# uber-research/UPSNet

Hardware: AMD Instinct MI355X
Metric: images/sec (whole node), UPSNet-50 1024x2048 (higher is better)
Workload: dtype f32

## Files before the change

include/upsnet_hip.h:

```cpp
#ifndef UPSNET_HIP_H
#define UPSNET_HIP_H

#include <stddef.h>
#include <stdint.h>

#ifdef __cplusplus
extern "C" {
#endif

const char *upsnet_last_error(void);
const char *upsnet_last_kernel_form(void);
int upsnet_abi_version(void);

int upsnet_zero_fill(void *stream, void *ptr, size_t bytes);


int upsnet_roi_align_forward(void *stream, const float *bottom_data, float spatial_scale, int num_rois,
                             int height, int width, int channels, int pooled_height, int pooled_width,
                             int sampling_ratio, const float *bottom_rois, float *top_data);

int upsnet_roi_align_forward_nhwc(void *stream, const float *feat_nhwc, int batch, int height, int width,
                                  int channels, float spatial_scale, const float *rois, int num_rois,
                                  int pooled_height, int pooled_width, int sampling_ratio, float *out_nhwc);

int upsnet_fpn_roi_align_forward(void *stream, const float *const feat_nhwc[4], const int feat_h[4],
                                 const int feat_w[4], const float spatial_scale[4], int channels,
                                 const float *rois, int num_rois, const int *num_rois_dev, int pooled_height,
                                 int pooled_width, int sampling_ratio, float *out_nhwc, int *levels_out);

int upsnet_fpn_roi_order(void *stream, const float *rois, int num_rois, const int *num_rois_dev, int image_height, int image_width,
                         int *order_out);
int upsnet_fpn_roi_align_forward_ordered(void *stream, const float *const feat_nhwc[4], const int feat_h[4], const int feat_w[4],
                                         const float spatial_scale[4], int channels, const float *rois, int num_rois, const int *num_rois_dev,
                                         int pooled_height, int pooled_width, int sampling_ratio, float *out_nhwc, int *levels_out,
                                         const int *order);

void upsnet_roi_tuning(int variant);
void upsnet_roi_geometry(int target_workgroups, int min_bins);


int upsnet_deform_im2col(void *stream, const float *data_im, const float *data_offset, int channels,
                         int height, int width, int ksize_h, int ksize_w, int pad_h, int pad_w, int stride_h,
                         int stride_w, int dilation_h, int dilation_w, int parallel_imgs, int deformable_group,
                         float *data_col);

int upsnet_mod_deform_im2col(void *stream, const float *data_im, const float *data_offset,
                             const float *data_mask, int batch_size, int channels, int height_im, int width_im,
                             int height_col, int width_col, int kernel_h, int kernel_w, int pad_h, int pad_w,
                             int stride_h, int stride_w, int dilation_h, int dilation_w, int deformable_group,
                             float *data_col);


int upsnet_roi_align_backward(void *stream, const float *top_diff, float spatial_scale, int batch_size, int num_rois,
                              int height, int width, int channels, int pooled_height, int pooled_width,
                              int sampling_ratio, const float *bottom_rois, float *bottom_diff);

int upsnet_deform_col2im(void *stream, const float *data_col, const float *data_offset, int channels, int height,
                         int width, int ksize_h, int ksize_w, int pad_h, int pad_w, int stride_h, int stride_w,
                         int dilation_h, int dilation_w, int parallel_imgs, int deformable_group, float *grad_im);

int upsnet_deform_col2im_coord(void *stream, const float *data_col, const float *data_im, const float *data_offset,
                               int channels, int height, int width, int ksize_h, int ksize_w, int pad_h, int pad_w,
                               int stride_h, int stride_w, int dilation_h, int dilation_w, int parallel_imgs,
                               int deformable_group, float *grad_offset);

int upsnet_mod_deform_col2im(void *stream, const float *data_col, const float *data_offset, const float *data_mask,
                             int batch_size, int channels, int height_im, int width_im, int height_col, int width_col,
                             int kernel_h, int kernel_w, int pad_h, int pad_w, int stride_h, int stride_w,
                             int dilation_h, int dilation_w, int deformable_group, float *grad_im);

int upsnet_mod_deform_col2im_coord(void *stream, const float *data_col, const float *data_im, const float *data_offset,
                                   const float *data_mask, int batch_size, int channels, int height_im, int width_im,
                                   int height_col, int width_col, int kernel_h, int kernel_w, int pad_h, int pad_w,
                                   int stride_h, int stride_w, int dilation_h, int dilation_w, int deformable_group,
                                   float *grad_offset, float *grad_mask);

int upsnet_deform_conv_forward_nhwc(void *stream, int nlev, const float *const x[], const float *const offset[],
                                    const float *const mask[], float *const out[], const int height[],
                                    const int width[], int cin, int cout, int kh, int kw, int pad_h, int pad_w,
                                    int stride_h, int stride_w, int dil_h, int dil_w, int deformable_group,
                                    const float *wpack, int ldw, const float *bias, int relu);

size_t upsnet_dcn_packed_weight_floats(int cout, int cin, int kh, int kw);
int upsnet_dcn_pack_weight(void *stream, const float *weight, int cout, int cin, int kh, int kw, float *wpack);
int upsnet_deform_conv_fused_nhwc(void *stream, int nlev, const float *const x[], const float *const offset[],
                                  const float *const mask[], float *const out[], const int height[], const int width[],
                                  int cin, int cout, int kh, int kw, int pad, int stride, int dil, const float *wpack,
                                  const float *bias, int relu);
size_t upsnet_deform_conv_fused_splitk_workspace_bytes(int height, int width, int cout, int kh, int kw, int pad, int stride, int dil,
                                                       int ksplit);
int upsnet_deform_conv_fused_nhwc_splitk(void *stream, const float *x, const float *offset, const float *mask, float *out, int height,
                                         int width, int cin, int cout, int kh, int kw, int pad, int stride, int dil,
                                         const float *wpack, const float *bias, int relu, int ksplit, void *workspace);
void upsnet_dcn_tuning(int variant);

size_t upsnet_dcn_packed_weight_bf16_elems(int cout, int cin, int kh, int kw);
int upsnet_dcn_pack_weight_bf16(void *stream, const float *weight, int cout, int cin, int kh, int kw, void *wpack);
int upsnet_deform_conv_fused_nhwc_bf16(void *stream, int nlev, const float *const x[], const float *const offset[],
                                       const float *const mask[], float *const out[], const int height[], const int width[], int cin,
                                       int cout, int kh, int kw, int pad, int stride, int dil, const void *wpack, const float *bias,
                                       int relu);


int upsnet_prep_image_u8(void *stream, const unsigned char *image_hwc, int height, int width, const double pixel_means[3],
                         double im_scale, int resized_h, int resized_w, int padded_h, int padded_w, int nhwc4, float *blob);

int upsnet_image_to_nhwc4(void *stream, const float *nchw, int batch, int channels, int height, int width, float *nhwc4);


int upsnet_conv2d_nhwc_f32_multiw(void *stream, int nseg, const float *const x[], float *const out[], const int batch[],
                                  const int height[], const int width[], int Cin, const float *const wpack[], int ldw, int Cout,
                                  int KH, int KW, int stride, int pad, int relu);

int upsnet_conv2d_nhwc_f32(void *stream, int nseg, const float *const x[], const float *const residual[],
                           float *const out[], const int batch[], const int height[], const int width[], int Cin,
                           const float *wpack, int ldw, const float *bias, int Cout, int KH, int KW, int stride, int pad,
                           int relu, int residual_up);

size_t upsnet_conv2d_splitk_workspace_bytes(int batch, int height, int width, int Cout, int KH, int KW, int stride, int pad, int ksplit);
int upsnet_conv2d_nhwc_f32_splitk(void *stream, const float *x, const float *residual, float *out, int batch, int height, int width,
                                  int Cin, const float *wpack, int ldw, const float *bias, int Cout, int KH, int KW, int stride,
                                  int pad, int relu, int ksplit, void *workspace);

int upsnet_conv2d_winograd_nhwc_f32(void *stream, int nseg, const float *const x[], const float *const residual[],
                                    float *const out[], const int batch[], const int height[], const int width[], int Cin,
                                    const float *wpack, int ldw, const float *bias, int Cout, int relu);

int upsnet_conv2d_winograd_nhwc_f32_splitk(void *stream, const float *x, const float *residual, float *out, int batch, int height,
                                           int width, int Cin, const float *wpack, int ldw, const float *bias, int Cout, int relu,
                                           int ksplit, void *workspace);
int upsnet_conv_pack_weight_winograd(void *stream, const float *weight, int cout, int cin, int ldw, float *wpack);

int upsnet_conv2d_winograd_nhwc_f32_tn32(void *stream, int nseg, const float *const x[], const float *const residual[],
                                         float *const out[], const int batch[], const int height[], const int width[], int Cin,
                                         const float *wpack, int ldw, const float *bias, int Cout, int relu);
int upsnet_conv_pack_weight_winograd_tn32(void *stream, const float *weight, int cout, int cin, int ldw, float *wpack);
int upsnet_conv2d_winograd_nhwc_f32_tail(void *stream, const float *x, float *out, int batch, int n_main, int height, int width, int Cin,
                                         const float *wpack, int ldw, const float *wpack32, int ldw32, const float *bias, int Cout, int relu);

int upsnet_conv2d_nhwc_bf16(void *stream, int nseg, const float *const x[], const float *const residual[], float *const out[],
                            const int batch[], const int height[], const int width[], int Cin, const void *wpack_hi,
                            const void *wpack_lo, int ldw, const float *bias, int Cout, int KH, int KW, int stride, int pad,
                            int relu);
int upsnet_conv_pack_weight_bf16(void *stream, const float *weight, int cout, int cin, int kh, int kw, int ldw, void *wpack_hi,
                                 void *wpack_lo);
int upsnet_bottleneck_proj_bf16(void *stream, const void *x, void *out, int batch, int height_in, int width_in, int cin, int cmid, int stride,
                                const void *w1, const void *w2, const void *w3d, const float *b1, const float *b2, const float *b3d);
int upsnet_conv_bf16_tuning(int enable, int tile_rows);
int upsnet_conv1x1_bf16_tuning(int enable);
int upsnet_stem_pool_pack_weight_f32(void *stream, const float *weight, int cin, float *wpack);
int upsnet_stem_pool_f32(void *stream, const float *x4, int batch, int height, int width, const float *wpack, const float *bias, float *out);
int upsnet_stem_pool_pack_weight_bf16(void *stream, const float *weight, int cin, void *wpack);
int upsnet_stem_pool_bf16(void *stream, const float *x4, int batch, int height, int width, const void *wpack, const float *bias, void *out);
int upsnet_deconv2x2_nhwc_bf16(void *stream, const void *x, int batch, int height, int width, int Cin, const void *wpack_hi, int ldw,
                               const float *bias, int Cout, int relu, void *out, int out_bf16);

int upsnet_bottleneck_bf16(void *stream, const void *x, void *out, int batch, int height, int width, int cmid, const void *w1,
                           const void *w2, const void *w3, const float *b1, const float *b2, const float *b3);

int upsnet_conv2d_stem_nhwc4_f32(void *stream, const float *x, int batch, int height, int width, const float *wpack,
                                 int ldw, const float *bias, int Cout, int KH, int KW, int stride, int pad, int relu,
                                 float *out);
int upsnet_conv_pack_weight_stem(void *stream, const float *weight, int cout, int cin, int kh, int kw, int ldw, float *wpack);

int upsnet_deconv2x2_nhwc_f32(void *stream, const float *x, int batch, int height, int width, int Cin, const float *wpack,
                              int ldw, const float *bias, int Cout, int relu, float *out);
int upsnet_deconv2x2_pack_weight(void *stream, const float *weight, int cin, int cout, int ldw, float *wpack);

int upsnet_deconv2x2_frag_nhwc_f32(void *stream, const float *x, float *out, int batch, int height, int width, int Cin,
                                   const float *wpack, const float *bias4, int Cout, int relu);

void upsnet_conv_tuning(int winograd_tiles, int force_tile);

int upsnet_conv_pack_weight(void *stream, const float *weight, int cout, int cin, int kh, int kw, int ldw, float *wpack);

int upsnet_conv1x1_frag_nhwc_f32(void *stream, const float *x, const float *residual, float *out, int batch, int height, int width,
                                 int Cin, const float *wpack, const float *bias, int Cout, int stride, int relu, int residual_up);
void upsnet_conv1x1_tuning(int bn);
int upsnet_conv1x1_siblings_nhwc_f32(void *stream, const float *x, float *out_a, float *out_b, int batch, int height, int width, int Cin,
                                     const float *wpack, const float *bias, int cout_a, int cout_b, int stride, int relu_a, int relu_b);
void upsnet_conv1x1_pair32_tuning(int waves);

int upsnet_conv2d_winograd36_nhwc_f32(void *stream, int nseg, const float *const x[], float *const out[], const int batch[],
                                      const int height[], const int width[], int Cin, const float *wpack, int ldw, const float *bias,
                                      int Cout, int relu);
int upsnet_conv_pack_weight_winograd36(void *stream, const float *weight, int cout, int cin, int ldw, float *wpack);
size_t upsnet_conv2d_winograd36_splitk_workspace_bytes(int batch, int height, int width, int Cout, int ksplit);
int upsnet_conv2d_winograd36_nhwc_f32_splitk(void *stream, const float *x, float *out, int batch, int height, int width, int Cin,
                                             const float *wpack, int ldw, const float *bias, int Cout, int relu, int ksplit, void *workspace);

size_t upsnet_conv1x1_ksw_packed_weight_floats(int cout, int cin);
int upsnet_conv1x1_ksw_pack_weight(void *stream, const float *weight, int cout, int cin, float *wpack);
int upsnet_conv1x1_ksw_nhwc_f32(void *stream, const float *x, const float *residual, float *out, int batch, int height, int width, int Cin,
                                const float *wpack, const float *bias, int Cout, int stride, int relu, int tile_pixels, int tile_channels,
                                int split_n);
void upsnet_conv1x1_ksw_tuning(int tile);

size_t upsnet_conv3x3_ksw_packed_weight_floats(int cin);
int upsnet_conv3x3_ksw_pack_weight(void *stream, const float *weight, int cout, int cin, float *wpack);
int upsnet_conv3x3_ksw_nhwc_f32(void *stream, const float *x, float *out, int batch, int height, int width, int Cin, const float *wpack,
                                const float *bias, int Cout, int relu);

size_t upsnet_conv1x1_splitk_workspace_bytes(int batch, int out_height, int out_width, int Cout, int ksplit);
int upsnet_conv1x1_frag_nhwc_f32_splitk(void *stream, const float *x, const float *residual, float *out, int batch, int height, int width,
                                        int Cin, const float *wpack, const float *bias, int Cout, int stride, int relu, int ksplit,
                                        void *workspace);

int upsnet_conv1x1_pair_nhwc_f32(void *stream, const float *x, const float *residual, float *out1, float *out2, long pixels, int C0,
                                 const float *w3pack, const float *bias3, int C1, const float *w1pack, const float *bias1, int C2);


int upsnet_nms_host(int *keep_out_host, int *num_out_host, const float *boxes_host, int boxes_num,
                    int boxes_dim, float nms_overlap_thresh, int device_id);

size_t upsnet_nms_workspace_bytes(int num_problems, int nmax);
int upsnet_nms_batched(void *stream, const float *boxes, const float *scores, const int *counts,
                       const uint8_t *pre_removed, int num_problems, int nmax, float thresh, int *keep_idx,
                       int *keep_cnt, void *workspace);

void upsnet_nms_tuning(int lds_staging);

int upsnet_cpu_nms_batched(void *stream, const float *boxes, const float *scores, const int *counts, int num_problems,
                           int nmax, double thresh, int *keep_idx, int *keep_cnt, void *workspace);

size_t upsnet_soft_nms_batched_workspace_bytes(int num_problems, int nmax);
int upsnet_soft_nms_batched(void *stream, float *boxes, int64_t *inds, const int *counts, int num_problems, int nmax,
                            float sigma, float Nt, float threshold, int method, int *n_out, void *workspace);

size_t upsnet_soft_nms_workspace_bytes(int n);
int upsnet_soft_nms(void *stream, float *boxes, int64_t *inds, int n, float sigma, float Nt, float threshold,
                    int method, int *n_out, void *workspace);


size_t upsnet_proposal_workspace_bytes(int nlev, const int *heights_host, const int *widths_host, int num_anchors,
                                       int pre_nms_top_n, int post_nms_top_n);
int upsnet_pyramid_proposals(void *stream, int nlev, const float *const cls_prob[], const float *const bbox_pred[],
                             const int *heights_host, const int *widths_host, const int *strides_host,
                             const float *anchors_host, int num_anchors, const float *im_info, int pre_nms_top_n,
                             int post_nms_top_n, float nms_thresh, float min_size, float *rois_out,
                             float *scores_out, int *num_out, void *workspace);

int upsnet_pyramid_proposals_strided(void *stream, int nlev, const float *const cls_prob[], const float *const bbox_pred[],
                                     const long *cls_chan_stride, const long *cls_pix_stride, const long *box_chan_stride,
                                     const long *box_pix_stride, const int *heights_host, const int *widths_host,
                                     const int *strides_host, const float *anchors_host, int num_anchors, const float *im_info,
                                     int pre_nms_top_n, int post_nms_top_n, float nms_thresh, float min_size, float *rois_out,
                                     float *scores_out, int *num_out, void *workspace);
int upsnet_pyramid_proposals_strided_ordered(void *stream, int nlev, const float *const cls_prob[], const float *const bbox_pred[],
                                     const long *cls_chan_stride, const long *cls_pix_stride, const long *box_chan_stride,
                                     const long *box_pix_stride, const int *heights_host, const int *widths_host,
                                     const int *strides_host, const float *anchors_host, int num_anchors, const float *im_info,
                                     int pre_nms_top_n, int post_nms_top_n, float nms_thresh, float min_size, float *rois_out,
                                     float *scores_out, int *num_out, void *workspace, int *roi_order_out);

int upsnet_pyramid_proposals_joint_strided(void *stream, int nlev, const float *const cls_prob[], const float *const bbox_pred[],
                                           const long *cls_chan_stride, const long *cls_pix_stride, const long *box_chan_stride,
                                           const long *box_pix_stride, const int *heights_host, const int *widths_host,
                                           const int *strides_host, const float *anchors_host, int num_anchors, const float *im_info,
                                           int pre_nms_top_n, int post_nms_top_n, float nms_thresh, float min_size, float *rois_out,
                                           float *scores_out, int *num_out, void *workspace);


int upsnet_mask_roi_capacity(int num_rois, int num_classes, int class_agnostic);
size_t upsnet_mask_roi_workspace_bytes(int num_rois, int num_classes, int class_agnostic);
int upsnet_mask_roi(void *stream, const float *rois, const float *bbox_delta, const float *cls_prob, int num_rois,
                    const int *num_rois_dev, int num_classes, const float *im_info, int class_agnostic,
                    float score_thresh, float nms_thresh, int max_det, const float reg_weights_host[4],
                    float *boxes_out, float *scores_out, int64_t *cls_out, int *src_out, int *num_out,
                    void *workspace);
int upsnet_mask_roi_ex(void *stream, const float *rois, const float *bbox_delta, const float *cls_prob, int num_rois,
                       const int *num_rois_dev, int num_classes, const float *im_info, int class_agnostic, int clip_boxes,
                       float score_thresh, float nms_thresh, int max_det, const float reg_weights_host[4],
                       float *boxes_out, float *scores_out, int64_t *cls_out, int *src_out, int *num_out,
                       void *workspace);

int upsnet_mask_roi_dedup(void *stream, const int *a_src, const int64_t *a_cls, const int *num_a, int cap_a, const int *b_src,
                          const int64_t *b_cls, const float *b_boxes, const int *num_b, int cap_b, int *map_out,
                          float *extra_boxes, int *num_extra);

int upsnet_mask_logit_gather(void *stream, const float *mask_logit, int n_rows, int num_classes, int hw, long stride_n,
                             long stride_c, long stride_e, const int *row, const int64_t *cls, int K, float *out);


size_t upsnet_mask_removal_workspace_bytes(int m, int num_thing_classes, int height, int width);
int upsnet_mask_removal(void *stream, const float *mask_rois, const float *cls_prob, const float *mask_logit,
                        const int64_t *cls_idx, int m, const int *m_dev, int mask_size, int num_thing_classes, int height, int width,
                        double fraction_threshold, int64_t *keep_inds, int *num_keep, int *real_keep,
                        void *workspace);

int upsnet_panoptic_tail_pack(void *stream, const int64_t *keep, const int *num_keep, int K, const int64_t *cls, const float *scores,
                              const int *det_num, const int *pan_num, const int *extra_num, int64_t *kept_cls, float *kept_scores,
                              int *counters);

int upsnet_mask_paste(void *stream, const float *mask_rois, const float *mask_logit, const int64_t *keep_inds,
                      const int *num_keep, const int *real_keep, int kmax, int mask_size, int height, int width,
                      float *mask_energy);

int upsnet_seg_term(void *stream, const float *fcn_output, int num_seg, int height, int width, const float *boxes,
                    const int64_t *cls, const int64_t *class_map, int k, float *seg_inst);

int upsnet_panoptic_fuse(void *stream, const float *fcn_output, int num_seg, int height, int width, int num_stuff,
                         const float *mask_rois, const float *mask_logit, const int64_t *cls_idx,
                         const int64_t *keep_inds, const int *num_keep, const int *real_keep, int kmax,
                         int mask_size, const int64_t *class_map, int enable_void, int64_t *pan_out,
                         int64_t *sem_out);

int upsnet_fcn_score_combine(void *stream, int nlev, const float *const part[], int num_seg, int height, int width,
                             const float *bias, float *score);

int upsnet_panoptic_fuse_up(void *stream, const float *fcn_score, int score_nhwc, int num_seg, int score_h, int score_w,
                            int scale, int num_stuff, const float *mask_rois, const float *mask_logit,
                            const int64_t *cls_idx, const int64_t *keep_inds, const int *num_keep, const int *real_keep,
                            int kmax, int mask_size, const int64_t *class_map, int64_t *pan_out, int64_t *sem_out);

int upsnet_panoptic_argmax(void *stream, const float *fcn_output, int num_seg, int height, int width, int num_stuff,
                           const float *seg_inst, const float *mask_energy, int k, int enable_void,
                           int64_t *pan_out);


size_t upsnet_unified_pan_workspace_bytes(void);
int upsnet_unified_pan_result(void *stream, const int64_t *pan, const int64_t *seg, const int64_t *cls_inds, int num_inst,
                              int height, int width, int id_last_stuff, int num_seg_classes, int stuff_area_limit,
                              void *workspace, unsigned char *pan_2ch);

size_t upsnet_combined_pan_workspace_bytes(int num_images, long total_pixels);
int upsnet_combined_pan_result(void *stream, int num_images, const int64_t *images, int max_height, int max_width, long total_pixels,
                               const int *cand, const int *segments, int id_last_stuff, int num_classes, int stuff_area_limit,
                               double fraction_threshold, void *workspace);

int upsnet_im_post_rle(void *stream, const float *pred_boxes, const float *mask_prob, const int64_t *cls_inds, int num_det,
                       int num_mask_channels, int mask_size, int im_height, int im_width, int cap, unsigned *transitions,
                       int *transition_count);

int upsnet_restore_label_maps(void *stream, const int64_t *sseg, const int64_t *pano, long src_stride, int src_height, int src_width,
                              const int *y_ofs, int out_height, const int *x_ofs, int out_width, unsigned char *out_sseg,
                              unsigned char *out_pano);


size_t upsnet_pq_workspace_bytes(int max_gt);
int upsnet_pq_accumulate(void *stream, const unsigned char *pred_2ch, const unsigned char *gt_rgb, int height, int width,
                         const int64_t *segments, int num_segments, const unsigned char *cat_known, int image_index, int max_gt,
                         void *workspace, int64_t *tp, int64_t *fp, int64_t *fn, double *iou, uint64_t *status);

int upsnet_confusion_accumulate(void *stream, const unsigned char *gt_label, const unsigned char *pred_label, long npix,
                                int class_num, int ignore_label, int64_t *confusion);


size_t upsnet_det_eval_image_workspace_bytes(int num_det, int num_rows, int num_gt, int height, int width, int segm);
int upsnet_det_eval_image(void *stream, int segm, int height, int width, int num_rows, int num_det, const double *det_xyxy,
                          const double *det_score, const int64_t *det_cls, const int *class_to_row, int num_classes,
                          const float *det_box_f32, const float *mask_prob, int num_mask_channels, int mask_size,
                          const int *det_trans, const int64_t *det_trans_off, int num_gt, const int *gt_row_off,
                          const double *gt_box, const double *gt_area, const int *gt_crowd, const int *gt_trans,
                          const int64_t *gt_trans_off, const int *gt_trans_dst, int num_gt_rle, const unsigned char *const *gt_u8,
                          const int *gt_u8_dst, int num_gt_u8, const int *rows_with_gt, int num_rows_with_gt,
                          const double *params, int image_index, void *workspace, double *rec_score, int *rec_img, int *rec_rk,
                          uint64_t *rec_match, uint64_t *rec_ign, int64_t *npig);

size_t upsnet_det_eval_accumulate_workspace_bytes(long num_records, int num_rows);
int upsnet_det_eval_accumulate(void *stream, long num_records, const double *rec_score, const int *rec_img, const int *rec_rk,
                               const uint64_t *rec_match, const uint64_t *rec_ign, const int *img_ord, int num_rows,
                               const int64_t *npig, const double *rec_thrs, void *workspace, double *precision, double *recall,
                               double *scores);

size_t upsnet_det_eval_boundary_image_workspace_bytes(int num_det, int num_rows, int num_gt, int height, int width);
int upsnet_det_eval_boundary_image(void *stream, int dilation, int height, int width, int num_rows, int num_det,
                                   const double *det_score, const int64_t *det_cls, const int *class_to_row, int num_classes,
                                   const float *det_box_f32, const float *mask_prob, int num_mask_channels, int mask_size,
                                   const int *det_trans, const int64_t *det_trans_off, int num_gt, const int *gt_row_off,
                                   const double *gt_area, const int *gt_crowd, const int *gt_trans,
                                   const int64_t *gt_trans_off, const int *gt_trans_dst, int num_gt_rle,
                                   const unsigned char *const *gt_u8, const int *gt_u8_dst, int num_gt_u8, const int *rows_with_gt,
                                   int num_rows_with_gt, const double *params, int image_index, void *workspace, double *rec_score,
                                   int *rec_img, int *rec_rk, uint64_t *rec_match, uint64_t *rec_ign, int64_t *npig);
int upsnet_boundary_dilation_fits(int height, int width, int dilation);

size_t upsnet_boundary_masks_workspace_bytes(int num_masks, int height, int width);
int upsnet_boundary_masks(void *stream, int dilation, int height, int width, int num_masks, const unsigned char *masks_u8,
                          const int *trans, const int64_t *trans_off, void *workspace, unsigned char *boundary_u8, int *boundary_area);

size_t upsnet_poly_raster_workspace_bytes(long total_vertices, long total_points);
int upsnet_poly_raster(void *stream, const double *vertices, const int *poly_off, const int *obj_off, const int *poly_off_dev,
                       const int *obj_off_dev, int num_poly, int num_obj, long total_points, int height, int width, void *workspace,
                       int *trans, int64_t *trans_off);


size_t upsnet_proposal_recall_workspace_bytes(int num_problems, long total_proposals);
int upsnet_proposal_recall(void *stream, int num_problems, const int64_t *problems, const float *proposals, const float *gt_boxes,
                           int max_gt, long total_proposals, void *workspace, float *out);


size_t upsnet_cs_inst_counts_ints(int num_preds);
size_t upsnet_cs_inst_workspace_bytes(int num_preds);
int upsnet_cs_inst_state_words(void);
int upsnet_cs_inst_image(void *stream, const uint16_t *gt_ids, int height, int width, int num_preds, const int *pred_cls,
                         const float *pred_scores, const int *trans, const int *trans_off, const unsigned char *masks, int walk_strided,
                         uint16_t *gt_t, const double *thresholds, int num_thr, int *counts, void *workspace, float *rec_score,
                         unsigned char *rec_cls, unsigned char *rec_code, int64_t *state);


size_t upsnet_cs_pixel_inst_ints(void);
int upsnet_cs_pixel_image(void *stream, const unsigned char *gt_labels, const uint16_t *gt_ids, const unsigned char *pred,
                          const unsigned char *lut, int height, int width, const double *avg_class_size, int64_t *conf, int *inst,
                          double *wsum, int *bad);


size_t upsnet_pan_format_workspace_bytes(void);
size_t upsnet_pan_format_table_ints(void);
int upsnet_pan_format(void *stream, const unsigned char *pred_2ch, int height, int width, const int *cat_table, void *workspace,
                      unsigned char *rgb, int *table);

int upsnet_pan_relabel(void *stream, const unsigned char *rgb, int height, int width, const int *table, int num_segments,
                       int image_index, unsigned char *out_2ch, int *counts, uint64_t *status);


size_t upsnet_gt_prepare_workspace_bytes(int seg_capacity);
int upsnet_gt_prepare(void *stream, const int *ids, const unsigned char *label_ids, int height, int width, const int *train_id,
                      const int *has_instances, const int *thing_row, int seg_capacity, int trans_capacity, void *workspace,
                      unsigned char *train_map, unsigned char *rgb, int *table, int *trans_off, int *trans, int *status);


int upsnet_vis_max_detections(void);
int upsnet_vis_max_label(void);
size_t upsnet_vis_workspace_bytes(int num_dets, int height, int width);
int upsnet_vis_font(unsigned char *cells);
int upsnet_vis_render(void *stream, const unsigned char *image, int height, int width, int num_dets, const float *boxes,
                      const unsigned char *colours, const unsigned char *labels, const int *label_len, const int *trans,
                      const int *trans_off, int num_trans, void *workspace, unsigned char *out);


int upsnet_group_norm_chunk_pixels(void);
size_t upsnet_group_norm_workspace_bytes(int nseg, const int batch[], const int height[], const int width[]);
int upsnet_group_norm_nhwc_f32(void *stream, int nseg, const float *const x[], float *const out[], const int batch[],
                               const int height[], const int width[], int C, const float *gamma, const float *beta, float eps,
                               int relu, const float *const residual[], const int res_height[], const int res_width[],
                               int residual_up, void *workspace);
int upsnet_group_norm_small_nhwc_f32(void *stream, const float *x, float *out, int batch, int height, int width, int C,
                                     const float *gamma, const float *beta, float eps, int relu);


int upsnet_cs_inst_expand(void *stream, const int *trans, const int *trans_off, int num_masks, int height, int width, int bits,
                          unsigned char *out);


int upsnet_tta_seg_merge(void *stream, int num_aug, const float *const maps[], const int map_h[], const int map_w[], const float q[],
                         const float resized_w[], const int flip[], int cell, int num_seg, int height, int width, float *out);

int upsnet_tta_roi_union(void *stream, int num_aug, const float *const rois[], const float *const delta[], const float *const prob[],
                         const int *const num_rois_dev[], const float r[], const float resized_w[], const int flip[], int capacity,
                         int delta_dim, int num_classes, float *rois_out, float *delta_out, float *prob_out, int *num_out);

int upsnet_tta_boxes_to_aug(void *stream, int num_aug, const float q[], const float resized_w[], const int flip[], const float *boxes,
                            int num_boxes, float *boxes_out);

int upsnet_tta_mask_merge(void *stream, int num_aug, const float *const logits[], const int flip[], int num_rois, int num_classes,
                          int mask_size, int nhwc, float *out);

#ifdef __cplusplus
}
#endif
#endif
```

upsnet_amd/_lib.py:

```python
import ctypes
import os

import torch

_HERE = os.path.dirname(os.path.abspath(__file__))
LIB_PATH = os.environ.get("UPSNET_LIB_PATH") or os.path.join(_HERE, "csrc", "libupsnet_hip.so")

c_int, c_float, c_double, c_void_p, c_size_t, c_long = ctypes.c_int, ctypes.c_float, ctypes.c_double, ctypes.c_void_p, ctypes.c_size_t, ctypes.c_long
P = c_void_p

_SIGNATURES = {
    "upsnet_last_error": (ctypes.c_char_p, []),
    "upsnet_last_kernel_form": (ctypes.c_char_p, []),
    "upsnet_abi_version": (c_int, []),
    "upsnet_zero_fill": (c_int, [P, P, c_size_t]),
    "upsnet_roi_align_forward": (c_int, [P, P, c_float, c_int, c_int, c_int, c_int, c_int, c_int, c_int, P, P]),
    "upsnet_roi_align_forward_nhwc": (c_int, [P, P, c_int, c_int, c_int, c_int, c_float, P, c_int, c_int, c_int, c_int, P]),
    "upsnet_fpn_roi_align_forward": (c_int, [P, P, P, P, P, c_int, P, c_int, P, c_int, c_int, c_int, P, P]),
    "upsnet_fpn_roi_order": (c_int, [P, P, c_int, P, c_int, c_int, P]),
    "upsnet_fpn_roi_align_forward_ordered": (c_int, [P, P, P, P, P, c_int, P, c_int, P, c_int, c_int, c_int, P, P, P]),
    "upsnet_roi_tuning": (None, [c_int]),
    "upsnet_roi_geometry": (None, [c_int, c_int]),
    "upsnet_deform_im2col": (c_int, [P, P, P] + [c_int] * 13 + [P]),
    "upsnet_mod_deform_im2col": (c_int, [P, P, P, P] + [c_int] * 15 + [P]),
    "upsnet_roi_align_backward": (c_int, [P, P, c_float] + [c_int] * 8 + [P, P]),
    "upsnet_deform_col2im": (c_int, [P, P, P] + [c_int] * 13 + [P]),
    "upsnet_deform_col2im_coord": (c_int, [P, P, P, P] + [c_int] * 13 + [P]),
    "upsnet_mod_deform_col2im": (c_int, [P, P, P, P] + [c_int] * 15 + [P]),
    "upsnet_mod_deform_col2im_coord": (c_int, [P, P, P, P, P] + [c_int] * 15 + [P, P]),
    "upsnet_deform_conv_forward_nhwc": (c_int, [P, c_int, P, P, P, P, P, P] + [c_int] * 11 + [P, c_int, P, c_int]),
    "upsnet_dcn_packed_weight_floats": (c_size_t, [c_int, c_int, c_int, c_int]),
    "upsnet_dcn_pack_weight": (c_int, [P, P, c_int, c_int, c_int, c_int, P]),
    "upsnet_deform_conv_fused_nhwc": (c_int, [P, c_int, P, P, P, P, P, P] + [c_int] * 7 + [P, P, c_int]),
    "upsnet_deform_conv_fused_splitk_workspace_bytes": (c_size_t, [c_int] * 9),
    "upsnet_deform_conv_fused_nhwc_splitk": (c_int, [P, P, P, P, P] + [c_int] * 9 + [P, P, c_int, c_int, P]),
    "upsnet_dcn_tuning": (None, [c_int]),
    "upsnet_dcn_packed_weight_bf16_elems": (c_size_t, [c_int, c_int, c_int, c_int]),
    "upsnet_dcn_pack_weight_bf16": (c_int, [P, P, c_int, c_int, c_int, c_int, P]),
    "upsnet_deform_conv_fused_nhwc_bf16": (c_int, [P, c_int, P, P, P, P, P, P] + [c_int] * 7 + [P, P, c_int]),
    "upsnet_conv1x1_frag_nhwc_f32": (c_int, [P, P, P, P, c_int, c_int, c_int, c_int, P, P, c_int, c_int, c_int, c_int]),
    "upsnet_conv1x1_tuning": (None, [c_int]),
    "upsnet_conv1x1_siblings_nhwc_f32": (c_int, [P, P, P, P, c_int, c_int, c_int, c_int, P, P, c_int, c_int, c_int, c_int, c_int]),
    "upsnet_conv1x1_pair32_tuning": (None, [c_int]),
    "upsnet_conv1x1_splitk_workspace_bytes": (ctypes.c_size_t, [c_int, c_int, c_int, c_int, c_int]),
    "upsnet_conv1x1_frag_nhwc_f32_splitk": (c_int, [P, P, P, P, c_int, c_int, c_int, c_int, P, P, c_int, c_int, c_int, c_int, P]),
    "upsnet_conv1x1_ksw_packed_weight_floats": (ctypes.c_size_t, [c_int, c_int]),
    "upsnet_conv1x1_ksw_pack_weight": (c_int, [P, P, c_int, c_int, P]),
    "upsnet_conv1x1_ksw_nhwc_f32": (c_int, [P, P, P, P, c_int, c_int, c_int, c_int, P, P, c_int, c_int, c_int, c_int, c_int, c_int]),
    "upsnet_conv1x1_ksw_tuning": (None, [c_int]),
    "upsnet_conv3x3_ksw_packed_weight_floats": (ctypes.c_size_t, [c_int]),
    "upsnet_conv3x3_ksw_pack_weight": (c_int, [P, P, c_int, c_int, P]),
    "upsnet_conv3x3_ksw_nhwc_f32": (c_int, [P, P, P, c_int, c_int, c_int, c_int, P, P, c_int, c_int]),
    "upsnet_conv2d_winograd36_splitk_workspace_bytes": (ctypes.c_size_t, [c_int, c_int, c_int, c_int, c_int]),
    "upsnet_conv2d_winograd36_nhwc_f32_splitk": (c_int, [P, P, P, c_int, c_int, c_int, c_int, P, c_int, P, c_int, c_int, c_int, P]),
    "upsnet_conv1x1_pair_nhwc_f32": (c_int, [P, P, P, P, P, c_long, c_int, P, P, c_int, P, P, c_int]),
    "upsnet_conv2d_nhwc_f32": (c_int, [P, c_int, P, P, P, P, P, P, c_int, P, c_int, P, c_int, c_int, c_int, c_int, c_int, c_int, c_int]),
    "upsnet_conv2d_nhwc_f32_multiw": (c_int, [P, c_int, P, P, P, P, P, c_int, P, c_int, c_int, c_int, c_int, c_int, c_int, c_int]),
    "upsnet_conv_tuning": (None, [c_int, c_int]),
    "upsnet_conv_pack_weight": (c_int, [P, P, c_int, c_int, c_int, c_int, c_int, P]),
    "upsnet_nms_host": (c_int, [P, P, P, c_int, c_int, c_float, c_int]),
    "upsnet_nms_workspace_bytes": (c_size_t, [c_int, c_int]),
    "upsnet_nms_batched": (c_int, [P, P, P, P, P, c_int, c_int, c_float, P, P, P]),
    "upsnet_nms_tuning": (None, [c_int]),
    "upsnet_cpu_nms_batched": (c_int, [P, P, P, P, c_int, c_int, c_double, P, P, P]),
    "upsnet_soft_nms_batched_workspace_bytes": (c_size_t, [c_int, c_int]),
    "upsnet_soft_nms_batched": (c_int, [P, P, P, P, c_int, c_int, c_float, c_float, c_float, c_int, P, P]),
    "upsnet_soft_nms_workspace_bytes": (c_size_t, [c_int]),
    "upsnet_soft_nms": (c_int, [P, P, P, c_int, c_float, c_float, c_float, c_int, P, P]),
    "upsnet_proposal_workspace_bytes": (c_size_t, [c_int, P, P, c_int, c_int, c_int]),
    "upsnet_pyramid_proposals_strided": (c_int, [P, c_int, P, P, P, P, P, P, P, P, P, P, c_int, P, c_int, c_int, c_float, c_float, P, P, P, P]),
    "upsnet_pyramid_proposals_strided_ordered": (c_int, [P, c_int, P, P, P, P, P, P, P, P, P, P, c_int, P, c_int, c_int, c_float, c_float, P, P, P, P, P]),
    "upsnet_pyramid_proposals_joint_strided": (c_int, [P, c_int, P, P, P, P, P, P, P, P, P, P, c_int, P, c_int, c_int, c_float, c_float, P, P, P, P]),
    "upsnet_pyramid_proposals": (c_int, [P, c_int, P, P, P, P, P, P, c_int, P, c_int, c_int, c_float, c_float, P, P, P, P]),
    "upsnet_mask_roi_capacity": (c_int, [c_int, c_int, c_int]),
    "upsnet_mask_roi_workspace_bytes": (c_size_t, [c_int, c_int, c_int]),
    "upsnet_mask_roi": (c_int, [P, P, P, P, c_int, P, c_int, P, c_int, c_float, c_float, c_int, P, P, P, P, P, P, P]),
    "upsnet_mask_roi_ex": (c_int, [P, P, P, P, c_int, P, c_int, P, c_int, c_int, c_float, c_float, c_int, P, P, P, P, P, P, P]),
    "upsnet_mask_logit_gather": (c_int, [P, P, c_int, c_int, c_int, c_long, c_long, c_long, P, P, c_int, P]),
    "upsnet_mask_removal_workspace_bytes": (c_size_t, [c_int, c_int, c_int, c_int]),
    "upsnet_mask_removal": (c_int, [P, P, P, P, P, c_int, P, c_int, c_int, c_int, c_int, c_double, P, P, P, P]),
    "upsnet_panoptic_tail_pack": (c_int, [P, P, P, c_int, P, P, P, P, P, P, P, P]),
    "upsnet_mask_paste": (c_int, [P, P, P, P, P, P, c_int, c_int, c_int, c_int, P]),
    "upsnet_seg_term": (c_int, [P, P, c_int, c_int, c_int, P, P, P, c_int, P]),
    "upsnet_panoptic_fuse": (c_int, [P, P, c_int, c_int, c_int, c_int, P, P, P, P, P, P, c_int, c_int, P, c_int, P, P]),
    "upsnet_panoptic_fuse_up": (c_int, [P, P, c_int, c_int, c_int, c_int, c_int, c_int, P, P, P, P, P, P, c_int, c_int, P, P, P]),
    "upsnet_conv2d_stem_nhwc4_f32": (c_int, [P, P, c_int, c_int, c_int, P, c_int, P, c_int, c_int, c_int, c_int, c_int, c_int, P]),
    "upsnet_conv_pack_weight_stem": (c_int, [P, P, c_int, c_int, c_int, c_int, c_int, P]),
    "upsnet_deconv2x2_nhwc_f32": (c_int, [P, P, c_int, c_int, c_int, c_int, P, c_int, P, c_int, c_int, P]),
    "upsnet_deconv2x2_pack_weight": (c_int, [P, P, c_int, c_int, c_int, P]),
    "upsnet_deconv2x2_frag_nhwc_f32": (c_int, [P, P, P, c_int, c_int, c_int, c_int, P, P, c_int, c_int]),
    "upsnet_prep_image_u8": (c_int, [P, P, c_int, c_int, P, c_double, c_int, c_int, c_int, c_int, c_int, P]),
    "upsnet_image_to_nhwc4": (c_int, [P, P, c_int, c_int, c_int, c_int, P]),
    "upsnet_unified_pan_workspace_bytes": (c_size_t, []),
    "upsnet_unified_pan_result": (c_int, [P, P, P, P, c_int, c_int, c_int, c_int, c_int, c_int, P, P]),
    "upsnet_combined_pan_workspace_bytes": (c_size_t, [c_int, c_long]),
    "upsnet_combined_pan_result": (c_int, [P, c_int, P, c_int, c_int, c_long, P, P, c_int, c_int, c_int, c_double, P]),
    "upsnet_mask_roi_dedup": (c_int, [P, P, P, P, c_int, P, P, P, P, c_int, P, P, P]),
    "upsnet_conv2d_winograd_nhwc_f32": (c_int, [P, c_int, P, P, P, P, P, P, c_int, P, c_int, P, c_int, c_int]),
    "upsnet_conv2d_winograd_nhwc_f32_splitk": (c_int, [P, P, P, P, c_int, c_int, c_int, c_int, P, c_int, P, c_int, c_int, c_int, P]),
    "upsnet_conv_pack_weight_winograd": (c_int, [P, P, c_int, c_int, c_int, P]),
    "upsnet_conv_pack_weight_winograd_tn32": (c_int, [P, P, c_int, c_int, c_int, P]),
    "upsnet_conv2d_winograd_nhwc_f32_tn32": (c_int, [P, c_int, P, P, P, P, P, P, c_int, P, c_int, P, c_int, c_int]),
    "upsnet_conv2d_winograd_nhwc_f32_tail": (c_int, [P, P, P, c_int, c_int, c_int, c_int, c_int, P, c_int, P, c_int, P, c_int, c_int]),
    "upsnet_conv2d_winograd36_nhwc_f32": (c_int, [P, c_int, P, P, P, P, P, c_int, P, c_int, P, c_int, c_int]),
    "upsnet_conv_pack_weight_winograd36": (c_int, [P, P, c_int, c_int, c_int, P]),
    "upsnet_conv2d_nhwc_bf16": (c_int, [P, c_int, P, P, P, P, P, P, c_int, P, P, c_int, P, c_int, c_int, c_int, c_int, c_int, c_int]),
    "upsnet_bottleneck_proj_bf16": (c_int, [P, P, P, c_int, c_int, c_int, c_int, c_int, c_int, P, P, P, P, P, P]),
    "upsnet_conv_bf16_tuning": (c_int, [c_int, c_int]),
    "upsnet_conv1x1_bf16_tuning": (c_int, [c_int]),
    "upsnet_stem_pool_pack_weight_f32": (c_int, [P, P, c_int, P]),
    "upsnet_stem_pool_f32": (c_int, [P, P, c_int, c_int, c_int, P, P, P]),
    "upsnet_stem_pool_pack_weight_bf16": (c_int, [P, P, c_int, P]),
    "upsnet_stem_pool_bf16": (c_int, [P, P, c_int, c_int, c_int, P, P, P]),
    "upsnet_deconv2x2_nhwc_bf16": (c_int, [P, P, c_int, c_int, c_int, c_int, P, c_int, P, c_int, c_int, P, c_int]),
    "upsnet_bottleneck_bf16": (c_int, [P, P, P, c_int, c_int, c_int, c_int, P, P, P, P, P, P]),
    "upsnet_conv_pack_weight_bf16": (c_int, [P, P, c_int, c_int, c_int, c_int, c_int, P, P]),
    "upsnet_conv2d_splitk_workspace_bytes": (c_size_t, [c_int, c_int, c_int, c_int, c_int, c_int, c_int, c_int, c_int]),
    "upsnet_conv2d_nhwc_f32_splitk": (c_int, [P, P, P, P, c_int, c_int, c_int, c_int, P, c_int, P, c_int, c_int, c_int, c_int, c_int, c_int, c_int, P]),
    "upsnet_im_post_rle": (c_int, [P, P, P, P, c_int, c_int, c_int, c_int, c_int, c_int, P, P]),
    "upsnet_fcn_score_combine": (c_int, [P, c_int, P, c_int, c_int, c_int, P, P]),
    "upsnet_panoptic_argmax": (c_int, [P, P, c_int, c_int, c_int, c_int, P, P, c_int, c_int, P]),
    "upsnet_pq_workspace_bytes": (c_size_t, [c_int]),
    "upsnet_pq_accumulate": (c_int, [P, P, P, c_int, c_int, P, c_int, P, c_int, c_int, P, P, P, P, P, P]),
    "upsnet_restore_label_maps": (c_int, [P, P, P, c_long, c_int, c_int, P, c_int, P, c_int, P, P]),
    "upsnet_confusion_accumulate": (c_int, [P, P, P, c_long, c_int, c_int, P]),
    "upsnet_det_eval_image_workspace_bytes": (c_size_t, [c_int] * 6),
    "upsnet_det_eval_image": (c_int, [P, c_int, c_int, c_int, c_int, c_int, P, P, P, P, c_int, P, P, c_int, c_int, P, P, c_int, P, P, P, P,
                                      P, P, P, c_int, P, P, c_int, P, c_int, P, c_int, P, P, P, P, P, P, P]),
    "upsnet_det_eval_accumulate_workspace_bytes": (c_size_t, [c_long, c_int]),
    "upsnet_det_eval_accumulate": (c_int, [P, c_long, P, P, P, P, P, P, c_int, P, P, P, P, P, P]),
    "upsnet_det_eval_boundary_image_workspace_bytes": (c_size_t, [c_int] * 5),
    "upsnet_det_eval_boundary_image": (c_int, [P, c_int, c_int, c_int, c_int, c_int, P, P, P, c_int, P, P, c_int, c_int, P, P, c_int, P, P, P,
                                               P, P, P, c_int, P, P, c_int, P, c_int, P, c_int, P, P, P, P, P, P, P]),
    "upsnet_boundary_dilation_fits": (c_int, [c_int, c_int, c_int]),
    "upsnet_boundary_masks_workspace_bytes": (c_size_t, [c_int, c_int, c_int]),
    "upsnet_boundary_masks": (c_int, [P, c_int, c_int, c_int, c_int, P, P, P, P, P, P]),
    "upsnet_poly_raster_workspace_bytes": (c_size_t, [c_long, c_long]),
    "upsnet_poly_raster": (c_int, [P, P, P, P, P, P, c_int, c_int, c_long, c_int, c_int, P, P, P]),
    "upsnet_proposal_recall_workspace_bytes": (c_size_t, [c_int, c_long]),
    "upsnet_proposal_recall": (c_int, [P, c_int, P, P, P, c_int, c_long, P, P]),
    "upsnet_cs_inst_counts_ints": (c_size_t, [c_int]),
    "upsnet_cs_inst_workspace_bytes": (c_size_t, [c_int]),
    "upsnet_cs_inst_state_words": (c_int, []),
    "upsnet_cs_inst_image": (c_int, [P, P, c_int, c_int, c_int, P, P, P, P, P, c_int, P, P, c_int, P, P, P, P, P, P]),
    "upsnet_cs_pixel_inst_ints": (c_size_t, []),
    "upsnet_cs_pixel_image": (c_int, [P, P, P, P, P, c_int, c_int, P, P, P, P, P]),
    "upsnet_pan_format_workspace_bytes": (c_size_t, []),
    "upsnet_pan_format_table_ints": (c_size_t, []),
    "upsnet_pan_format": (c_int, [P, P, c_int, c_int, P, P, P, P]),
    "upsnet_pan_relabel": (c_int, [P, P, c_int, c_int, P, c_int, c_int, P, P, P]),
    "upsnet_gt_prepare_workspace_bytes": (c_size_t, [c_int]),
    "upsnet_gt_prepare": (c_int, [P, P, P, c_int, c_int, P, P, P, c_int, c_int, P, P, P, P, P, P, P]),
    "upsnet_vis_max_detections": (c_int, []),
    "upsnet_vis_max_label": (c_int, []),
    "upsnet_vis_workspace_bytes": (c_size_t, [c_int, c_int, c_int]),
    "upsnet_vis_font": (c_int, [P]),
    "upsnet_vis_render": (c_int, [P, P, c_int, c_int, c_int, P, P, P, P, P, P, c_int, P, P]),
    "upsnet_group_norm_chunk_pixels": (c_int, []),
    "upsnet_group_norm_workspace_bytes": (c_size_t, [c_int, P, P, P]),
    "upsnet_group_norm_nhwc_f32": (c_int, [P, c_int, P, P, P, P, P, c_int, P, P, c_float, c_int, P, P, P, c_int, P]),
    "upsnet_group_norm_small_nhwc_f32": (c_int, [P, P, P, c_int, c_int, c_int, c_int, P, P, c_float, c_int]),
    "upsnet_cs_inst_expand": (c_int, [P, P, P, c_int, c_int, c_int, c_int, P]),
    "upsnet_tta_seg_merge": (c_int, [P, c_int, P, P, P, P, P, P, c_int, c_int, c_int, c_int, P]),
    "upsnet_tta_roi_union": (c_int, [P, c_int, P, P, P, P, P, P, P, c_int, c_int, c_int, P, P, P, P]),
    "upsnet_tta_boxes_to_aug": (c_int, [P, c_int, P, P, P, P, c_int, P]),
    "upsnet_tta_mask_merge": (c_int, [P, c_int, P, P, c_int, c_int, c_int, c_int, P]),
}

_lib = None


def exported_symbols():
    return sorted(_SIGNATURES)


def lib():
    global _lib
    if _lib is None:
        if not os.path.exists(LIB_PATH):
            raise RuntimeError("upsnet_amd: %s is missing -- build it with `python -m upsnet_amd.build` "
                               "(there is no CPU fallback)" % LIB_PATH)
        l = ctypes.CDLL(LIB_PATH)
        for name, (res, args) in _SIGNATURES.items():
            fn = getattr(l, name)
            fn.restype = res
            fn.argtypes = args
        _lib = l
    return _lib


def check(rc, what):
    if rc != 0:
        raise RuntimeError("upsnet_amd.%s failed: %s" % (what, lib().upsnet_last_error().decode()))


def ptr(t):
    return None if t is None else c_void_p(t.data_ptr())


def stream():
    return c_void_p(torch.cuda.current_stream().cuda_stream)


def require_cuda(*tensors):
    for t in tensors:
        if t is not None and not t.is_cuda:
            raise Exception("not implemented")


def f32c(t):
    if t.dtype != torch.float32:
        t = t.float()
    return t.contiguous()


def nhwc(t):
    return t.contiguous(memory_format=torch.channels_last)


def int_array(vals):
    return (c_int * len(vals))(*[int(v) for v in vals])


def float_array(vals):
    return (c_float * len(vals))(*[float(v) for v in vals])


def ptr_array(tensors):
    return (c_void_p * len(tensors))(*[None if t is None else t.data_ptr() for t in tensors])
```

upsnet_amd/csrc/conv_params.h:

```cpp
#pragma once
#include "common.h"

#define CV_BM 128
#define CV_BK 32
#define CV_LDA (CV_BM + 1)
#define CV_MAXSEG 5

typedef float floatx16 __attribute__((ext_vector_type(16)));

struct ConvSeg {
    const float *x, *res, *off, *mask;
    const float *w;
    float *out;
    int N, H, W, Ho, Wo;
    int OH, OW;
    int tile_start;
    long M;
};

struct ConvParams {
    ConvSeg seg[CV_MAXSEG];
    const float *w, *bias;
    int nseg, Cin, Cout, ldw, KH, KW, stride, pad, dil, relu;
    int res_up;
    int m_tiles, n_tiles;
    int ksplit;
    float *partial;
    long m_total;
    int io;
    int sib_split, sib_relu;
    float *sib_out;
};

static inline int conv_fill(ConvParams &p, const char *who, int nseg, const float *const x[], const float *const res[],
                     const float *const off[], const float *const mask[], float *const out[], const int batch[],
                     const int height[], const int width[], int Cin, int Cout, const float *wpack, int ldw, const float *bias,
                     int KH, int KW, int stride, int pad, int dil, int relu)
{
    UPS_REQUIRE(nseg >= 1 && nseg <= CV_MAXSEG, "%s: 1..%d feature maps per launch (got %d)", who, CV_MAXSEG, nseg);
    UPS_REQUIRE(x && out && height && width && wpack, "%s: null pointer", who);
    UPS_REQUIRE(Cin > 0 && Cin % CV_BK == 0, "%s: Cin must be a multiple of 32 (got %d)", who, Cin);
    UPS_REQUIRE(Cout > 0 && ldw % 32 == 0 && ldw >= Cout, "%s: ldw must be Cout rounded up to 32 (got %d for Cout=%d)", who, ldw, Cout);
    UPS_REQUIRE(KH >= 1 && KW >= 1 && KH * KW <= 49 && stride >= 1 && pad >= 0 && dil >= 1, "%s: bad kernel/stride/pad/dilation", who);
    UPS_REQUIRE((long)KH * KW * Cin * ldw < (1L << 30), "%s: packed weight exceeds 4 GiB", who);
    p.w = wpack; p.bias = bias; p.nseg = nseg; p.Cin = Cin; p.Cout = Cout; p.ldw = ldw; p.KH = KH; p.KW = KW;
    p.stride = stride; p.pad = pad; p.dil = dil; p.relu = relu; p.res_up = 0;
    p.ksplit = 1; p.partial = nullptr; p.m_total = 0; p.io = 0; p.sib_split = 0; p.sib_relu = 0; p.sib_out = nullptr;
    int tiles = 0;
    for (int i = 0; i < CV_MAXSEG; ++i) {
        ConvSeg &s = p.seg[i];
        if (i < nseg) {
            const int nb = batch ? batch[i] : 1;
            UPS_REQUIRE(x[i] && out[i] && nb > 0 && height[i] > 0 && width[i] > 0, "%s: bad feature map %d", who, i);
            s.x = x[i]; s.out = out[i]; s.res = res ? res[i] : nullptr; s.off = off ? off[i] : nullptr; s.mask = mask ? mask[i] : nullptr;
            s.w = nullptr;
            s.N = nb; s.H = height[i]; s.W = width[i];
            s.OH = s.OW = 0;
            s.Ho = (height[i] + 2 * pad - (dil * (KH - 1) + 1)) / stride + 1;
            s.Wo = (width[i] + 2 * pad - (dil * (KW - 1) + 1)) / stride + 1;
            UPS_REQUIRE(s.Ho > 0 && s.Wo > 0, "%s: empty output for feature map %d", who, i);
            UPS_REQUIRE((long)nb * height[i] * width[i] * Cin < (1L << 30), "%s: feature map %d exceeds 4 GiB (32-bit byte offsets); split the batch", who, i);
            s.M = (long)nb * s.Ho * s.Wo;
            UPS_REQUIRE(s.M * Cout < (1L << 29), "%s: output %d exceeds 2 GiB (32-bit byte offsets in the epilogue); split the batch", who, i);
            s.tile_start = tiles;
            tiles += (int)((s.M + 127) / 128);
        } else {
            s.x = s.res = s.off = s.mask = nullptr; s.w = nullptr; s.out = nullptr;
            s.N = s.H = s.W = s.Ho = s.Wo = s.OH = s.OW = 0; s.M = 0; s.tile_start = 0x7fffffff;
        }
    }
    p.m_tiles = tiles;
    return 0;
}


int conv_splitk_reduce(hipStream_t st, const float *partial, int ksplit, long m_total, long M, int Cout, const float *bias, const float *res,
                       int relu, float *out);
```

upsnet_amd/csrc/conv_wino36.hip:

```cpp
#include <cstdlib>
#include <type_traits>
#include "conv_params.h"
#include "upsnet_hip.h"

#define W36_TM 32
#define W36_TN 64
#define W36_PTS 36
#define W36_VBUF (W36_PTS * 4 * W36_TM * 16)
#define W36_BSTEP (2 * W36_TN * 16)
#define W36_STEPS (2 * W36_PTS)
#define W36_XCH (16 * W36_PTS * 64 * 4)
#define W36_RING 3

typedef unsigned w36_uintx4 __attribute__((ext_vector_type(4)));

#define W36_BT(D0, D1, D2, D3, D4, D5)                                                                               \
    {                                                                                                                \
        const float a0_ = D0, a1_ = D1, a2_ = D2, a3_ = D3, a4_ = D4, a5_ = D5;                                       \
        const float e1_ = __builtin_fmaf(-2.25f, a2_, a4_), o1_ = __builtin_fmaf(-2.25f, a1_, a3_);                   \
        const float e3_ = __builtin_fmaf(-0.5625f, a2_, a4_), o3_ = __builtin_fmaf(-0.5625f, a1_, a3_);               \
        D0 = __builtin_fmaf(1.265625f, a0_, __builtin_fmaf(-2.8125f, a2_, a4_));                                     \
        D1 = __builtin_fmaf(0.75f, o1_, e1_);                                                                        \
        D2 = __builtin_fmaf(-0.75f, o1_, e1_);                                                                       \
        D3 = __builtin_fmaf(1.5f, o3_, e3_);                                                                         \
        D4 = __builtin_fmaf(-1.5f, o3_, e3_);                                                                        \
        D5 = __builtin_fmaf(1.265625f, a1_, __builtin_fmaf(-2.8125f, a3_, a5_));                                     \
    }
#define W36_AT(M0, M1, M2, M3, M4, M5, Y0, Y1, Y2, Y3)                                                               \
    {                                                                                                                \
        const float s1_ = (M1) + (M2), d1_ = (M1) - (M2), s2_ = (M3) + (M4), d2_ = (M3) - (M4);                      \
        Y0 = ((M0) + s1_) + s2_;                                                                                     \
        Y1 = __builtin_fmaf(1.5f, d2_, 0.75f * d1_);                                                                 \
        Y2 = __builtin_fmaf(2.25f, s2_, 0.5625f * s1_);                                                              \
        Y3 = __builtin_fmaf(3.375f, d2_, __builtin_fmaf(0.421875f, d1_, (M5)));                                      \
    }

template <bool SK>
__global__ void __launch_bounds__(512, 1) conv_wino36_f32_kernel(const ConvParams p)
{
    extern __shared__ __attribute__((aligned(16))) unsigned char smem_raw[];
    const int tid = threadIdx.x, lane = tid & 63;
    const int wave = __builtin_amdgcn_readfirstlane(tid >> 6);
    const int cb = wave >> 2, pg = wave & 3;
    const int lhalf = lane >> 5, l32 = lane & 31;
    int m_t, n_t, kz = 0;
    {
        const int nt = p.n_tiles;
        const int per = (p.m_tiles + 7) >> 3;
        int bid = (int)blockIdx.x;
        if constexpr (SK) { const int base_grid = 8 * per * nt; kz = bid / base_grid; bid -= kz * base_grid; }
        const int q = bid >> 3;
        n_t = q % nt;
        const int local = q / nt;
        m_t = (bid & 7) * per + local;
        if (local >= per || m_t >= p.m_tiles) return;
    }
    int si = 0;
#pragma unroll
    for (int q = 1; q < CV_MAXSEG; ++q) if (q < p.nseg && m_t >= p.seg[q].tile_start) si = q;
    const ConvSeg sg = p.seg[si];
    const long p0 = (long)(m_t - sg.tile_start) * W36_TM;
    const int nslabs_all = p.Cin >> 4;
    const int s_first = SK ? (kz * nslabs_all) / p.ksplit : 0;
    const int nslabs = SK ? ((kz + 1) * nslabs_all) / p.ksplit - s_first : nslabs_all;
    const long HoWo = (long)sg.Ho * sg.Wo;

    const int ltile = tid >> 4, lch = tid & 15;
    int hrow0, wcol0;
    int hlo, hhi;
    unsigned tbase, nrmask = 0, ncmask = 0;
    bool lane_fix;
    {
        const long pp = p0 + ltile;
        const bool tile_ok = pp < sg.M;
        const long ppc = tile_ok ? pp : sg.M - 1;
        const int n = (int)(ppc / HoWo);
        const int rem = (int)(ppc - (long)n * HoWo);
        const int ty = rem / sg.Wo, tx = rem - ty * sg.Wo;
        const int h0 = 4 * ty - 1;
        hlo = n * sg.H; hhi = tile_ok ? hlo + sg.H : hlo;
        hrow0 = hlo + h0;
        wcol0 = 4 * tx - 1;
#pragma unroll
        for (int r = 0; r < 6; ++r) nrmask |= (h0 + r >= 0 && h0 + r < sg.H) ? 0u : (1u << r);
#pragma unroll
        for (int c = 0; c < 6; ++c) ncmask |= (wcol0 + c >= 0 && wcol0 + c < sg.W) ? 0u : (1u << c);
        lane_fix = tile_ok && (nrmask | ncmask) != 0;
        tbase = (unsigned)(hrow0 * sg.W + wcol0) * (4u * (unsigned)p.Cin) + 4u * (unsigned)lch;
    }
    const bool fix = __builtin_amdgcn_ballot_w64(lane_fix) != 0ull;
    bool risky;
    {
        const long plast = min(p0 + (long)W36_TM, sg.M) - 1;
        const long nl = plast / HoWo;
        const long tyl = (plast - nl * HoWo) / sg.Wo;
        risky = (nl * sg.H + 4 * tyl + 4) * (long)sg.W + 4L * sg.Wo >= (long)sg.N * sg.H * sg.W;
    }
    const unsigned cin4 = 4u * (unsigned)p.Cin;
    const unsigned rowpitch = (unsigned)sg.W * cin4;
    const unsigned cin4_s = __builtin_amdgcn_readfirstlane(cin4);
    const unsigned rowpitch_s = __builtin_amdgcn_readfirstlane((unsigned)sg.W) * cin4_s;
    const unsigned cbase = (unsigned)wcol0 * cin4 + 4u * (unsigned)lch;
#define W36_ROWOFF(R) (((unsigned)min(max(hrow0 + (R), hlo), max(hhi - 1, hlo)) * rowpitch) | ((hrow0 + (R) >= hlo && hrow0 + (R) < hhi) ? 0u : 0x80000000u))
    const size_t xaddr = reinterpret_cast<size_t>(sg.x);
    const unsigned xlo = __builtin_amdgcn_readfirstlane((unsigned)xaddr), xhi = __builtin_amdgcn_readfirstlane((unsigned)(xaddr >> 32));
    const unsigned xbytes = __builtin_amdgcn_readfirstlane((unsigned)(sg.N * sg.H * sg.W) * 4u * (unsigned)p.Cin - (SK ? (unsigned)s_first * 64u : 0u));
    const char *xbase = reinterpret_cast<const char *>(((size_t)xhi << 32) | xlo) + (SK ? (size_t)s_first * 64 : 0);
#define W36_SWZ(Q) ((((Q) & 1) << 2) | (((Q) >> 1) << 1))
    const unsigned st_base = (unsigned)((((lch >> 2) * W36_TM + (ltile ^ W36_SWZ(lch >> 2))) * 16) + (lch & 3) * 4);
    constexpr unsigned XI_PITCH = 4 * W36_TM * 16;
    const unsigned fr_base0 = (unsigned)((lhalf * W36_TM + (l32 ^ W36_SWZ(lhalf))) * 16) + (unsigned)pg * 9u * XI_PITCH;
    const unsigned fr_base1 = (unsigned)(((2 + lhalf) * W36_TM + (l32 ^ W36_SWZ(2 + lhalf))) * 16) + (unsigned)pg * 9u * XI_PITCH;
    const size_t waddr = reinterpret_cast<size_t>(p.w) + ((size_t)n_t * (size_t)nslabs_all + (size_t)s_first) * (W36_STEPS * W36_BSTEP);
    const unsigned wlo = __builtin_amdgcn_readfirstlane((unsigned)waddr), whi = __builtin_amdgcn_readfirstlane((unsigned)(waddr >> 32));
    const __amdgpu_buffer_rsrc_t wrsrc = __builtin_amdgcn_make_buffer_rsrc(reinterpret_cast<void *>(((size_t)whi << 32) | wlo), 0,
                                                                            nslabs * (int)(W36_STEPS * W36_BSTEP), 0x00020000);
    const unsigned b_lane = (unsigned)(lhalf * (W36_TN * 16) + (32 * cb + l32) * 16);
    const int gmax = nslabs * W36_STEPS - 1;

    floatx16 acc[9];
#pragma unroll
    for (int i = 0; i < 9; ++i)
#pragma unroll
        for (int r = 0; r < 16; ++r) acc[i][r] = 0.f;

    float ld[36];
    float4 breg[W36_RING];

#define W36_LOADROW_FAST(R, RS) { unsigned so_ = (unsigned)((R) ? (R) - 1 : 0) * rowpitch_s; asm volatile("" : "+s"(so_));              \
        ld[6 * (R)] = __uint_as_float(__builtin_amdgcn_raw_buffer_load_b32(RS, (R) ? tbase + rowpitch_s : tbase, so_, 0));               \
        _Pragma("unroll") for (int c_ = 1; c_ < 6; ++c_) ld[6 * (R) + c_] = __uint_as_float(__builtin_amdgcn_raw_buffer_load_b32(       \
            RS, ((R) ? tbase + rowpitch_s : tbase) + cin4_s, so_ + (unsigned)(c_ - 1) * cin4_s, 0)); }
#define W36_LOADROW_SAFE(R, RS) { unsigned cb_ = cbase; asm volatile("" : "+v"(cb_)); const unsigned rb_ = W36_ROWOFF(R) + cb_; _Pragma("unroll") for (int c_ = 0; c_ < 6; ++c_) \
        ld[6 * (R) + c_] = __uint_as_float(__builtin_amdgcn_raw_buffer_load_b32(RS, (rb_ + (unsigned)c_ * cin4) | ((ncmask << (30 - c_)) & 0x40000000u), 0, 0)); }
#define W36_FIXROW(R) if (fix) { asm volatile("" ::: "memory"); const unsigned bad_ = ((nrmask >> (R)) & 1u) ? 0x3fu : ncmask;           \
        _Pragma("unroll") for (int c_ = 0; c_ < 6; ++c_) ld[6 * (R) + c_] = ((bad_ >> c_) & 1u) ? 0.f : ld[6 * (R) + c_]; }
#define W36_ROWPASS(R) W36_BT(ld[6 * (R) + 0], ld[6 * (R) + 1], ld[6 * (R) + 2], ld[6 * (R) + 3], ld[6 * (R) + 4], ld[6 * (R) + 5])
#define W36_COLSTASH(J, SB)                                                                                           \
    {                                                                                                                 \
        float c0_ = ld[0 + (J)], c1_ = ld[6 + (J)], c2_ = ld[12 + (J)], c3_ = ld[18 + (J)], c4_ = ld[24 + (J)], c5_ = ld[30 + (J)]; \
        W36_BT(c0_, c1_, c2_, c3_, c4_, c5_)                                                                          \
        *reinterpret_cast<float *>(smem_raw + (SB) + (0 * 6 + (J)) * XI_PITCH) = c0_;                                 \
        *reinterpret_cast<float *>(smem_raw + (SB) + (1 * 6 + (J)) * XI_PITCH) = c1_;                                 \
        *reinterpret_cast<float *>(smem_raw + (SB) + (2 * 6 + (J)) * XI_PITCH) = c2_;                                 \
        *reinterpret_cast<float *>(smem_raw + (SB) + (3 * 6 + (J)) * XI_PITCH) = c3_;                                 \
        *reinterpret_cast<float *>(smem_raw + (SB) + (4 * 6 + (J)) * XI_PITCH) = c4_;                                 \
        *reinterpret_cast<float *>(smem_raw + (SB) + (5 * 6 + (J)) * XI_PITCH) = c5_;                                 \
    }
#define W36_BLOAD(SLOT, G) { const w36_uintx4 v_ = __builtin_amdgcn_raw_buffer_load_b128(wrsrc, b_lane, (unsigned)min((G), gmax) * W36_BSTEP, 0); \
        breg[SLOT] = make_float4(__uint_as_float(v_.x), __uint_as_float(v_.y), __uint_as_float(v_.z), __uint_as_float(v_.w)); }

#pragma unroll
    for (int u = 0; u < W36_RING; ++u) W36_BLOAD(u, 18 * pg + u)
    {
        const __amdgpu_buffer_rsrc_t xr = __builtin_amdgcn_make_buffer_rsrc(const_cast<char *>(xbase), 0, xbytes, 0x00020000);
#pragma unroll
        for (int r = 0; r < 6; ++r) { W36_LOADROW_SAFE(r, xr) }
#pragma unroll
        for (int r = 0; r < 6; ++r) { W36_ROWPASS(r) }
#pragma unroll
        for (int j = 0; j < 6; ++j) { W36_COLSTASH(j, st_base) }
    }
    __syncthreads();
    float4 afr = *reinterpret_cast<const float4 *>(smem_raw + fr_base0);

    auto slab_loop = [&](auto fast_tag) __attribute__((always_inline)) {
    constexpr bool FAST = decltype(fast_tag)::value;
    for (int s = 0; s < nslabs; ++s) {
        const int sn = min(s + 1, nslabs - 1);
        const __amdgpu_buffer_rsrc_t xr = __builtin_amdgcn_make_buffer_rsrc(const_cast<char *>(xbase) + (size_t)sn * 64, 0, xbytes - (unsigned)sn * 64u, 0x00020000);
        const unsigned cur = (s & 1) ? W36_VBUF : 0u, nxt = W36_VBUF - cur;
        const unsigned sb = nxt + st_base;
        const int g0 = s * W36_STEPS + 18 * pg;
#pragma unroll
        for (int u = 0; u < 18; ++u) {
            if (u < 6) { if constexpr (FAST) { W36_LOADROW_FAST(u, xr) } else { W36_LOADROW_SAFE(u, xr) } }
            float4 afn;
            if (u < 17) afn = *reinterpret_cast<const float4 *>(smem_raw + cur + (((u + 1) & 1) ? fr_base1 : fr_base0) + (unsigned)((u + 1) >> 1) * XI_PITCH);
            else afn = *reinterpret_cast<const float4 *>(smem_raw + nxt + fr_base0);
            if (u == 6) { if constexpr (FAST) { W36_FIXROW(0) } W36_ROWPASS(0) }
            if (u == 7) { if constexpr (FAST) { W36_FIXROW(1) } W36_ROWPASS(1) }
            if (u == 8) { if constexpr (FAST) { W36_FIXROW(2) } W36_ROWPASS(2) }
            if (u == 9) { if constexpr (FAST) { W36_FIXROW(3) } W36_ROWPASS(3) }
            if (u == 10) { if constexpr (FAST) { W36_FIXROW(4) } W36_ROWPASS(4) }
            if (u == 11) { if constexpr (FAST) { W36_FIXROW(5) } W36_ROWPASS(5) W36_COLSTASH(0, sb) }
            if (u == 12) { W36_COLSTASH(1, sb) }
            if (u == 13) { W36_COLSTASH(2, sb) }
            if (u == 14) { W36_COLSTASH(3, sb) }
            if (u == 15) { W36_COLSTASH(4, sb) }
            if (u == 16) { W36_COLSTASH(5, sb) }
            const float4 bf = breg[u % W36_RING];
            acc[u >> 1] = __builtin_amdgcn_mfma_f32_32x32x2f32(afr.x, bf.x, acc[u >> 1], 0, 0, 0);
            acc[u >> 1] = __builtin_amdgcn_mfma_f32_32x32x2f32(afr.y, bf.y, acc[u >> 1], 0, 0, 0);
            acc[u >> 1] = __builtin_amdgcn_mfma_f32_32x32x2f32(afr.z, bf.z, acc[u >> 1], 0, 0, 0);
            acc[u >> 1] = __builtin_amdgcn_mfma_f32_32x32x2f32(afr.w, bf.w, acc[u >> 1], 0, 0, 0);
            W36_BLOAD(u % W36_RING, (u + W36_RING < 18 ? g0 : g0 + W36_STEPS - 18) + u + W36_RING)
            if (u == 16) __syncthreads();
            afr = afn;
            __builtin_amdgcn_sched_barrier(0);
        }
    }
    };
    if (risky) slab_loop(std::false_type{}); else slab_loop(std::true_type{});
#undef W36_LOADROW_FAST
#undef W36_LOADROW_SAFE
#undef W36_ROWOFF
#undef W36_FIXROW
#undef W36_ROWPASS
#undef W36_COLSTASH
#undef W36_BLOAD

    const unsigned crow = (unsigned)p.Cout * 4u;
    const size_t oaddr_ = reinterpret_cast<size_t>(SK ? p.partial + (size_t)kz * (size_t)p.m_total * (size_t)p.Cout : sg.out);
    const unsigned obytes_ = __builtin_amdgcn_readfirstlane((unsigned)((long)sg.N * sg.OH * sg.OW) * crow);
    const __amdgpu_buffer_rsrc_t orsrc = __builtin_amdgcn_make_buffer_rsrc(
        reinterpret_cast<void *>(((size_t)(unsigned)__builtin_amdgcn_readfirstlane((unsigned)(oaddr_ >> 32)) << 32) | (unsigned)__builtin_amdgcn_readfirstlane((unsigned)oaddr_)),
        0, (int)obytes_, 0x00020000);
    float *xch = reinterpret_cast<float *>(smem_raw);
#pragma unroll 1
    for (int bb = 0; bb < 2; ++bb) {
        __syncthreads();
        if (cb == bb) {
#pragma unroll
            for (int u = 0; u < 9; ++u)
#pragma unroll
                for (int r = 0; r < 16; ++r) xch[(r * W36_PTS + 9 * pg + u) * 64 + lane] = acc[u][r];
        }
        __syncthreads();
        const int co_ch = n_t * W36_TN + 32 * bb + l32;
        const bool co_ok = co_ch < p.Cout;
        const float bv = (p.bias != nullptr && co_ok) ? p.bias[co_ch] : 0.f;
#pragma unroll 1
        for (int rr = 0; rr < 2; ++rr) {
            const int r = 2 * wave + rr;
            const long pp = p0 + 8 * (r >> 2) + 4 * lhalf + (r & 3);
            float m[36];
#pragma unroll
            for (int x = 0; x < 36; ++x) m[x] = xch[(r * W36_PTS + x) * 64 + lane];
            if (!(co_ok && pp < sg.M)) continue;
            const int n = (int)(pp / HoWo);
            const int rem = (int)(pp - (long)n * HoWo);
            const int ty = rem / sg.Wo, tx = rem - ty * sg.Wo;
            float t[6][4];
#pragma unroll
            for (int i = 0; i < 6; ++i) W36_AT(m[6 * i + 0], m[6 * i + 1], m[6 * i + 2], m[6 * i + 3], m[6 * i + 4], m[6 * i + 5], t[i][0], t[i][1], t[i][2], t[i][3])
#pragma unroll
            for (int c = 0; c < 4; ++c) {
                float y[4];
                W36_AT(t[0][c], t[1][c], t[2][c], t[3][c], t[4][c], t[5][c], y[0], y[1], y[2], y[3])
                const int ox = 4 * tx + c;
#pragma unroll
                for (int a = 0; a < 4; ++a) {
                    const int oy = 4 * ty + a;
                    float v = y[a];
                    if constexpr (!SK) { v = v + bv; if (p.relu) v = fmaxf(v, 0.f); }
                    const unsigned off = (oy < sg.OH && ox < sg.OW) ? (unsigned)((n * sg.OH + oy) * sg.OW + ox) * crow + 4u * (unsigned)co_ch : 0x80000000u;
                    __builtin_amdgcn_raw_buffer_store_b32(__float_as_uint(v), orsrc, off, 0, 0);
                }
            }
        }
    }
}

static int w36_fill(ConvParams &p, const char *who, int nseg, const float *const x[], float *const out[], const int batch[], const int height[],
                    const int width[], int Cin, int Cout, const float *wpack, int ldw, const float *bias, int relu)
{
    UPS_REQUIRE(Cin > 0 && Cin % 32 == 0 && ldw % W36_TN == 0, "%s: Cin %% 32 == 0 and ldw %% 64 == 0 (got %d, %d)", who, Cin, ldw);
    int rc = conv_fill(p, who, nseg, x, nullptr, nullptr, nullptr, out, batch, height, width, Cin, Cout, wpack, ldw, bias, 3, 3, 1, 1, 1, relu);
    if (rc) return rc;
    UPS_REQUIRE((long)W36_PTS * Cin * ldw < (1L << 29), "%s: packed weight exceeds 2 GiB", who);
    int tiles = 0;
    for (int i = 0; i < nseg; ++i) {
        ConvSeg &s = p.seg[i];
        s.OH = s.Ho; s.OW = s.Wo;
        s.Ho = (s.OH + 3) / 4; s.Wo = (s.OW + 3) / 4;
        s.M = (long)s.N * s.Ho * s.Wo;
        UPS_REQUIRE((long)s.N * s.H * s.W * Cin < (1L << 28), "%s: feature map %d exceeds 1 GiB; split the batch", who, i);
        UPS_REQUIRE((long)s.N * s.OH * s.OW * Cout < (1L << 29), "%s: output %d exceeds 2 GiB; split the batch", who, i);
        s.tile_start = tiles;
        tiles += (int)((s.M + W36_TM - 1) / W36_TM);
    }
    p.m_tiles = tiles;
    p.n_tiles = ldw / W36_TN;
    return 0;
}

extern "C" int upsnet_conv2d_winograd36_nhwc_f32(void *stream, int nseg, const float *const x[], float *const out[], const int batch[],
                                                 const int height[], const int width[], int Cin, const float *wpack, int ldw, const float *bias,
                                                 int Cout, int relu)
{
    ConvParams p;
    int rc = w36_fill(p, "conv2d_winograd36_nhwc_f32", nseg, x, out, batch, height, width, Cin, Cout, wpack, ldw, bias, relu);
    if (rc) return rc;
    static std::atomic<unsigned long long> attr_dev{0};
    UPS_ONCE_PER_DEVICE(attr_dev, UPS_CHECK_HIP(hipFuncSetAttribute(reinterpret_cast<const void *>(&conv_wino36_f32_kernel<false>), hipFuncAttributeMaxDynamicSharedMemorySize, W36_XCH)));
    const int grid = 8 * ((p.m_tiles + 7) / 8) * p.n_tiles;
    hipLaunchKernelGGL(conv_wino36_f32_kernel<false>, dim3(grid), dim3(512), W36_XCH, (hipStream_t)stream, p);
    UPS_CHECK_LAUNCH("conv_wino36_f32_kernel");
    ups_set_form("wino36<%d,%d>", W36_TM, W36_TN);
    return 0;
}

extern "C" size_t upsnet_conv2d_winograd36_splitk_workspace_bytes(int batch, int height, int width, int Cout, int ksplit)
{
    return (size_t)ksplit * (size_t)batch * height * width * Cout * sizeof(float);
}

extern "C" int upsnet_conv2d_winograd36_nhwc_f32_splitk(void *stream, const float *x, float *out, int batch, int height, int width, int Cin,
                                                        const float *wpack, int ldw, const float *bias, int Cout, int relu, int ksplit,
                                                        void *workspace)
{
    const float *xs[1] = {x};
    float *os[1] = {out};
    const int nb[1] = {batch}, hh[1] = {height}, ww[1] = {width};
    ConvParams p;
    int rc = w36_fill(p, "conv2d_winograd36_nhwc_f32_splitk", 1, xs, os, nb, hh, ww, Cin, Cout, wpack, ldw, bias, relu);
    if (rc) return rc;
    UPS_REQUIRE(workspace && ksplit >= 2 && ksplit <= 8 && Cin / 16 >= ksplit, "conv2d_winograd36_nhwc_f32_splitk: ksplit 2..8, <= Cin / 16, and a workspace");
    p.ksplit = ksplit;
    p.partial = (float *)workspace;
    p.m_total = (long)batch * height * width;
    UPS_REQUIRE(p.m_total * Cout < (1L << 29), "conv2d_winograd36_nhwc_f32_splitk: output exceeds 2 GiB; split the batch");
    static std::atomic<unsigned long long> attr_dev{0};
    UPS_ONCE_PER_DEVICE(attr_dev, UPS_CHECK_HIP(hipFuncSetAttribute(reinterpret_cast<const void *>(&conv_wino36_f32_kernel<true>), hipFuncAttributeMaxDynamicSharedMemorySize, W36_XCH)));
    const int grid = 8 * ((p.m_tiles + 7) / 8) * p.n_tiles * ksplit;
    hipLaunchKernelGGL(conv_wino36_f32_kernel<true>, dim3(grid), dim3(512), W36_XCH, (hipStream_t)stream, p);
    UPS_CHECK_LAUNCH("conv_wino36_f32_kernel<splitk>");
    ups_set_form("wino36<%d,%d> splitk%d", W36_TM, W36_TN, ksplit);
    return conv_splitk_reduce((hipStream_t)stream, p.partial, ksplit, p.m_total, p.m_total, Cout, bias, nullptr, relu, out);
}

__global__ void conv_pack_weight_wino36_kernel(const float *__restrict__ w, int cout, int cin, int ldw, float *__restrict__ wp)
{
    const long total = (long)ldw * cin;
    const int nslabs = cin >> 4;
    const double G[6][3] = {{64.0 / 81, 0.0, 0.0}, {-128.0 / 243, -32.0 / 81, -8.0 / 27}, {-128.0 / 243, 32.0 / 81, -8.0 / 27},
                            {32.0 / 243, 16.0 / 81, 8.0 / 27}, {32.0 / 243, -16.0 / 81, 8.0 / 27}, {0.0, 0.0, 1.0}};
    for (long idx = (long)blockIdx.x * blockDim.x + threadIdx.x; idx < total; idx += (long)blockDim.x * gridDim.x) {
        const int co = idx % ldw, c = idx / ldw;
        double g[3][3], t[6][3];
#pragma unroll
        for (int a = 0; a < 3; ++a)
#pragma unroll
            for (int b = 0; b < 3; ++b) g[a][b] = co < cout ? (double)w[(((long)co * cin + c) * 3 + a) * 3 + b] : 0.0;
#pragma unroll
        for (int i = 0; i < 6; ++i)
#pragma unroll
            for (int b = 0; b < 3; ++b) t[i][b] = G[i][0] * g[0][b] + G[i][1] * g[1][b] + G[i][2] * g[2][b];
        const long blk = ((long)(co / W36_TN) * nslabs + (c >> 4)) * W36_PTS;
        const int q = (c & 15) >> 2, ci = c & 3, cl = co % W36_TN;
#pragma unroll
        for (int i = 0; i < 6; ++i)
#pragma unroll
            for (int j = 0; j < 6; ++j) {
                const double u = t[i][0] * G[j][0] + t[i][1] * G[j][1] + t[i][2] * G[j][2];
                wp[(((blk + i * 6 + j) * 4 + q) * W36_TN + cl) * 4 + ci] = (float)u;
            }
    }
}

extern "C" int upsnet_conv_pack_weight_winograd36(void *stream, const float *weight, int cout, int cin, int ldw, float *wpack)
{
    UPS_REQUIRE(weight && wpack && cout > 0 && cin > 0 && ldw >= cout, "conv_pack_weight_winograd36: bad args");
    UPS_REQUIRE(cin % 16 == 0 && ldw % W36_TN == 0, "conv_pack_weight_winograd36: Cin %% 16 must be 0 and ldw a multiple of 64");
    const long total = (long)ldw * cin;
    int blocks = (int)((total + 255) / 256);
    if (blocks > 65535) blocks = 65535;
    hipLaunchKernelGGL(conv_pack_weight_wino36_kernel, dim3(blocks), dim3(256), 0, (hipStream_t)stream, weight, cout, cin, ldw, wpack);
    UPS_CHECK_LAUNCH("conv_pack_weight_wino36_kernel");
    return 0;
}
```

upsnet_amd/knobs.py:

```python
import os
import re

_ROOT = os.path.dirname(os.path.abspath(__file__))
_NAME = re.compile(r'UPSNET_[A-Z0-9_]+')

REGISTRY = {
    'UPSNET_ALLOW_LIBRARY_CONV': ('0', 'models/hipconv.py', 'a convolution no hand-written kernel covers runs on the library instead of raising'),
    'UPSNET_BF16_ACT': ('1', 'models/hipconv.py', 'bf16 mode: bf16 activations between the layers (0: fp32 activations)'),
    'UPSNET_BF16_BLOCK': ('1', 'models/hipconv.py', 'bf16 mode: one-launch bottlenecks (0: three launches)'),
    'UPSNET_BF16_BLOCK_MIN_TILES': ('128', 'models/hipconv.py', 'bf16 mode: fewest tiles for the one-launch bottleneck'),
    'UPSNET_BF16_HALO': ('1', 'csrc/conv_bf16.hip', 'bf16 3x3 layers on the haloed-patch kernel (0: general kernel)'),
    'UPSNET_BF16_MIN_WG': ('192', 'models/hipconv.py', 'bf16 mode: fewest workgroups for a bf16 layer'),
    'UPSNET_BF16_MIN_WG_WREG': ('16', 'models/hipconv.py', 'bf16 mode: fewest workgroups for the weights-from-L2 3x3 kernel'),
    'UPSNET_BF16_NARROW_BELOW': ('384', 'csrc/conv_bf16.hip', 'bf16 general kernel: 128 x 64 tiles below this many workgroups'),
    'UPSNET_BF16_PROJ': ('1', 'models/hipconv.py', 'bf16 mode: projection bottlenecks as one launch'),
    'UPSNET_BF16_STEM': ('1', 'models/hipconv.py', 'bf16 mode: fused stem + pool kernel'),
    'UPSNET_BF16_WREG': ('1', 'csrc/conv3x3_wreg_bf16.hip', 'bf16 3x3 layers on the weights-from-L2 kernel'),
    'UPSNET_BF16_WREG1': ('1', 'csrc/conv1x1_wreg_bf16.hip', 'bf16 1x1 layers on the no-LDS kernel where it wins'),
    'UPSNET_BF16_WREG_TH': ('auto', 'csrc/conv3x3_wreg_bf16.hip', 'tile rows of the weights-from-L2 3x3 kernel'),
    'UPSNET_CONV1X1': ('1', 'models/hipconv.py', '1x1 layers on the lean GEMM kernel (0: implicit-GEMM kernel)'),
    'UPSNET_CONV1X1_BALANCE': ('0', 'models/hipconv.py', 'split-K tail for unevenly tiled 1x1 layers'),
    'UPSNET_CONV1X1_MIN_WG': ('256', 'models/hipconv.py', 'fewest workgroups for the lean 1x1 kernel'),
    'UPSNET_CONV1X1_KSW': ('1', 'models/hipconv.py', 'small-tile (16x16x4 fragment) 1x1 kernel for maps the 64-pixel tiles do not fill evenly'),
    'UPSNET_CONV1X1_KSW_MAX_FILL': ('0.75', 'models/hipconv.py', 'use it when the last round of 64-pixel workgroups is less than this full'),
    'UPSNET_CONV3X3_KSW': ('1', 'models/hipconv.py', 'small-tile 3x3 kernel for <= 32-channel layers (offset predictors) on small maps'),
    'UPSNET_CONV1X1_PAIR': ('1', 'models/hipconv.py', 'conv3 + next conv1 in one launch'),
    'UPSNET_CONV1X1_PAIR32_WAVES': ('8', 'ops.py', 'waves per workgroup of the res4 pair kernel'),
    'UPSNET_CONV1X1_PAIR_MIN_TILES': ('1024', 'models/hipconv.py', 'fewest tiles for the res2 pair kernel'),
    'UPSNET_CONV1X1_PAIR_RES3': ('1', 'models/hipconv.py', 'pair kernel on res3'),
    'UPSNET_CONV1X1_PAIR_RES4': ('1', 'models/hipconv.py', 'pair kernel on res4'),
    'UPSNET_CONV1X1_SIBLINGS': ('1', 'models/hipconv.py', 'conv1 + projection shortcut in one launch'),
    'UPSNET_CONV_PRECISION': ('fp32', 'models/hipconv.py', 'fp32 | bf16 | bf16x3 (bench.py --conv-precision)'),
    'UPSNET_DCN_BF16': ('1', 'ops.py', 'bf16 mode: fused deformable convolution on the bf16 cores'),
    'UPSNET_DCN_KERNEL': ('frag', 'ops.py', 'generation of the fused deformable kernel'),
    'UPSNET_DCN_SMALL_GRID': ('0', 'csrc/deform_fused.hip', 'small-grid variant threshold of the fused deformable kernel'),
    'UPSNET_DCN_SPLITK': ('1', 'ops.py', 'split-K for the offset predictors of small maps'),
    'UPSNET_DCN_VARIANT': ('5', 'csrc/deform_fused.hip', 'schedule variant of the fused deformable kernel'),
    'UPSNET_DECONV_FRAG': ('1', 'models/hipconv.py', 'transposed convolution on the lean GEMM kernel'),
    'UPSNET_DIST_BACKEND': ('nccl', 'upsnet_end2end_test.py', 'torch.distributed backend of the harness (gloo when ranks share a GPU)'),
    'UPSNET_EARLY_MASK': ('1', 'models/resnet_upsnet.py', 'mask head on the side stream as soon as the detections exist'),
    'UPSNET_FC_RELU': ('1', 'models/rcnn.py', 'ReLU of fc6 / fc7 in the library GEMM epilogue (0: separate elementwise launch)'),
    'UPSNET_GRAPH': ('1', 'models/resnet_upsnet.py', 'whole forward as one HIP graph'),
    'UPSNET_GRAPH_ALIAS': ('1', 'models/resnet_upsnet.py', 'outputs are views into the graph buffers (0: copies)'),
    'UPSNET_GRAPH_OWN_STREAM': ('0', 'models/resnet_upsnet.py', 'capture / replay on an own stream with one instance'),
    'UPSNET_GRAPH_SLOTS': ('2', 'models/resnet_upsnet.py', 'graph instances per input shape'),
    'UPSNET_HIP_MEMSET': ('0', 'csrc/fill.hip', 'zero scratch with hipMemsetAsync instead of a kernel'),
    'UPSNET_LIB_PATH': ('', '_lib.py', 'path of libupsnet_hip.so (same-box A/B of two builds)'),
    'UPSNET_NMS_LDS': ('0', 'csrc/nms.hip', 'stage the suppression mask in LDS'),
    'UPSNET_NMS_SCAN16': ('1', 'csrc/nms.hip', 'unrolled scan for <= 1024 boxes'),
    'UPSNET_OVERLAP': ('1', 'models/resnet_upsnet.py', 'semantic branch on a side stream'),
    'UPSNET_PIN': ('1', 'upsnet_end2end_test.py', 'pin each rank to its CPU slice'),
    'UPSNET_ROI_KERNEL': ('auto', 'csrc/roi_align.hip', 'ROIAlign kernel variant 0..4; auto = 3 (corner-sharing) for >= 100 bins per ROI, else 0 -- so '
                                                        '"0" is NOT the default; upsnet_roi_tuning(v >= 0) overrides the variable, (v < 0) returns to it'),
    'UPSNET_ROI_XCD_ORDER': ('1', 'ops.py', 'deal the ROIs of the box head\'s ROIAlign launch to the XCDs by image neighbourhood (table written by prop_merge_kernel)'),
    'UPSNET_ROI_XCD_ORDER_MIN': ('512', 'ops.py', 'only for launches with at least this many ROIs'),
    'UPSNET_ROI_XCD_ORDER_STANDALONE': ('0', 'ops.py', 'build the table with a launch of its own for ROI sets that do not come from pyramid_proposals'),
    'UPSNET_ROI_PER_BIN': ('0', 'csrc/roi_align.hip', 'one wave per (roi, bin) (older decomposition)'),
    'UPSNET_SHARE_GPU': ('0', 'upsnet_end2end_test.py', 'let N ranks share one GPU (functional runs of the N > 1 path)'),
    'UPSNET_SPLITK': ('1', 'models/hipconv.py', 'split-K forms for small maps'),
    'UPSNET_STEM_POOL': ('1', 'models/hipconv.py', 'fused stem + pool kernel (0: stem kernel + library pool)'),
    'UPSNET_WINO36': ('1', 'models/hipconv.py', 'largest 3x3 / stride 1 layers on the Winograd F(4x4,3x3) kernel'),
    'UPSNET_WINO36_SPLITK': ('0', 'models/hipconv.py', 'res3 / res4 conv2 and FPN P4 on the split-K F(4x4) form (3-5 us per launch; more rounding error)'),
    'UPSNET_WINO36_PREFIX': ('0', 'models/hipconv.py', 'multi-map F(4x4) launches keep only the leading maps that fill whole rounds of workgroups (measured: no gain)'),
    'UPSNET_WINO36_ROI': ('1', 'models/hipconv.py', 'mask head (ROI batches) on the Winograd F(4x4,3x3) kernel (0: F(2x2) with the half-size tail)'),
    'UPSNET_WINO36_MIN_FILL': ('0.65', 'models/hipconv.py', 'F(4x4,3x3) only if its last round of workgroups is at least this full'),
    'UPSNET_WINOGRAD': ('1', 'models/hipconv.py', '3x3 / stride 1 layers on the Winograd kernel'),
    'UPSNET_WINOGRAD_MIN_WG': ('128', 'models/hipconv.py', 'fewest workgroups for the Winograd kernel'),
    'UPSNET_WINO_TAIL_FUSED': ('1', 'models/hipconv.py', 'mask-head tail inside the main launch (0: two launches)'),
    'UPSNET_WINO_TAIL_SPLIT': ('1', 'models/hipconv.py', 'mask-head tail on half-size workgroups'),
    'UPSNET_WINO_TM64_MIN': ('768', 'models/hipconv.py', '64-tile Winograd workgroups above this many'),
}


def known():
    return set(REGISTRY)


def scan_sources():
    names = set()
    files = [os.path.join(os.path.dirname(_ROOT), 'bench.py')]
    for d, _, fs in os.walk(_ROOT):
        files += [os.path.join(d, f) for f in fs if f.endswith(('.py', '.hip', '.cpp', '.h')) and f != 'knobs.py']
    for f in files:
        try:
            with open(f, errors='ignore') as fh:
                names.update(_NAME.findall(fh.read()))
        except OSError:
            pass
    return names


def active(env=None):
    env = os.environ if env is None else env
    return {k: env[k] for k in sorted(env) if k.startswith('UPSNET_')}


def check(env=None):
    act = active(env)
    unknown = sorted(set(act) - known())
    if unknown:
        raise ValueError('unknown UPSNET_* environment variable(s) %s -- no source file reads them (typo?)' % ', '.join(unknown))
    return act
```

upsnet_amd/models/hipconv.py:

```python
import os

import torch
import torch.nn as nn
import torch.nn.functional as F

from .. import group_norm, ops

ENABLED = True
ALLOW_LIBRARY = os.environ.get('UPSNET_ALLOW_LIBRARY_CONV', '0') == '1'
FALLBACKS = []
TRACE = None


def _library(m, x, why):
    if x.is_cuda:
        FALLBACKS.append((repr(m), why))
        if not ALLOW_LIBRARY:
            raise RuntimeError('upsnet_amd.hipconv: %r on a CUDA tensor %s is not covered by the hand-written kernels (%s); set '
                               'UPSNET_ALLOW_LIBRARY_CONV=1 to run it on the library convolution' % (m, tuple(x.shape), why))


def _trace(kind, **kw):
    if TRACE is not None:
        kw['kind'] = kind
# ... 24 lines not shown

def _plan(m):
    return _pack(m, 'direct', ops.pack_conv_weight)


def _conv1x1_plan(m):
    return _pack(m, 'c1x1', ops.pack_conv1x1_weight)


def _use_conv1x1(m, x, always=False):
    if not (CONV1X1 and tuple(m.kernel_size) == (1, 1) and tuple(m.padding) == (0, 0) and m.stride[0] in (1, 2) and
            m.in_channels % 32 == 0 and m.out_channels >= 32):
        return False
    if always:
        return True
    st = m.stride[0]
    pix = x.shape[0] * ((x.shape[2] - 1) // st + 1) * ((x.shape[3] - 1) // st + 1)
    return -(-pix // 64) * -(-m.out_channels // 64) >= CONV1X1_MIN_WG


BALANCE = os.environ.get('UPSNET_CONV1X1_BALANCE', '0') == '1'
_BAL_OVERHEAD_US = 6.0
_BAL_STEP_US = 0.49
_CUS = {}


def _cus(device):
    if device.index not in _CUS:
        _CUS[device.index] = torch.cuda.get_device_properties(device).multi_processor_count
    return _CUS[device.index]


def _c1_bn(m_tiles, cout):
    return 128 if (cout > 64 and m_tiles * -(-cout // 128) >= 512) else 64


def _c1_walk_us(m_tiles, cin, cout):
    bn = _c1_bn(m_tiles, cout)
    return m_tiles * -(-cout // bn), (cin // 32) * (2 if bn == 128 else 1) * _BAL_STEP_US


def _c1_best_split(wgs, walk_us, nsl, cus):
    best, best_t = 1, -(-wgs // cus) * walk_us
    for ks in range(2, min(16, nsl // 2) + 1):
        if -(-nsl // ks) * (ks - 1) >= nsl:
            continue
        t = -(-wgs * ks // cus) * (walk_us / ks) + _BAL_OVERHEAD_US
        if t < best_t - 1.0:
            best, best_t = ks, t
    return best, best_t


def _c1_balance(m, x, cus=None):
    st = m.stride[0]
    M = x.shape[0] * ((x.shape[2] - 1) // st + 1) * ((x.shape[3] - 1) // st + 1)
    if not BALANCE or st != 1:
        return M, 1
    cus = cus or _cus(x.device)
    cin, cout, nsl = m.in_channels, m.out_channels, m.in_channels // 32
    m_tiles = -(-M // 64)
    wgs, walk = _c1_walk_us(m_tiles, cin, cout)
    plain = -(-wgs // cus) * walk
    if wgs % cus == 0 or wgs >= 8 * cus:
        return M, 1
    nt = wgs // m_tiles
    main_tiles = (wgs // cus) * cus // nt
    main_t = 0.0
    if main_tiles > 0:
        mw, mwalk = _c1_walk_us(main_tiles, cin, cout)
        main_t = -(-mw // cus) * mwalk
    tw, twalk = _c1_walk_us(m_tiles - main_tiles, cin, cout)
    ks, tail_t = _c1_best_split(tw, twalk, nsl, cus)
    if ks == 1 or main_t + tail_t + (_BAL_OVERHEAD_US if main_tiles else 0.0) >= plain - 1.0:
        return M, 1
    return main_tiles * 64, ks


def _conv1x1_balanced(m, x, relu, residual):
    rows_main, ks = _c1_balance(m, x)
    wp = _conv1x1_plan(m)
    if ks == 1:
        return ops.conv1x1_frag(x, wp, m.bias, m.out_channels, 1, relu=relu, residual=residual), 'conv1x1'
    x = ops.nhwc(x.float())
    N, C, H, W = x.shape
    M, co = N * H * W, m.out_channels
    out = ops._nhwc_out(N, co, H, W, x.device)
    slab = lambda t, c: t.permute(0, 2, 3, 1).reshape(M, c)
    img = lambda rows, c: rows.view(1, 1, rows.shape[0], c).permute(0, 3, 1, 2)
    xr, orow = slab(x, C), slab(out, co)
    rr = None if residual is None else slab(ops.nhwc(residual.float()), co)
    if rows_main:
        ops.conv1x1_frag(img(xr[:rows_main], C), wp, m.bias, co, 1, relu=relu, residual=None if rr is None else img(rr[:rows_main], co),
                         out=img(orow[:rows_main], co))
    ops.conv1x1_frag(img(xr[rows_main:], C), wp, m.bias, co, 1, relu=relu, residual=None if rr is None else img(rr[rows_main:], co),
                     out=img(orow[rows_main:], co), ksplit=ks)
    return out, 'conv1x1 %s splitk%d' % ('main + tail' if rows_main else 'all', ks)


KSW = os.environ.get('UPSNET_CONV1X1_KSW', '1') != '0'
KSW_MAX_FILL = float(os.environ.get('UPSNET_CONV1X1_KSW_MAX_FILL', '0.75'))
KSW_TILE = (16, 64)


def _ksw_plan(m):
    return _pack(m, 'ksw', ops.pack_conv1x1_ksw_weight)


def _use_ksw(m, x, cus=None):
    if not (KSW and PRECISION == 'fp32' and x.dtype == torch.float32 and tuple(m.kernel_size) == (1, 1) and tuple(m.padding) == (0, 0) and
            m.stride[0] in (1, 2) and m.in_channels % 16 == 0 and m.out_channels % 4 == 0 and m.in_channels >= 256 and
            m.in_channels >= 2 * m.out_channels):
        return False
    st = m.stride[0]
    pix = x.shape[0] * ((x.shape[2] - 1) // st + 1) * ((x.shape[3] - 1) // st + 1)
    m_tiles = -(-pix // 64)
    wgs = m_tiles * -(-m.out_channels // _c1_bn(m_tiles, m.out_channels))
    cus = cus or _cus(x.device)
    return wgs < KSW_MAX_FILL * -(-wgs // cus) * cus


KSW3 = os.environ.get('UPSNET_CONV3X3_KSW', '1') != '0'


def _ksw3_plan(m):
    return _pack(m, 'ksw3', ops.pack_conv3x3_ksw_weight)


def _use_ksw3(m, x):
    return (KSW3 and PRECISION == 'fp32' and x.dtype == torch.float32 and tuple(m.kernel_size) == (3, 3) and tuple(m.stride) == (1, 1) and
            tuple(m.padding) == (1, 1) and tuple(m.dilation) == (1, 1) and m.out_channels <= 32 and m.in_channels % 16 == 0)


PAIR = os.environ.get('UPSNET_CONV1X1_PAIR', '1') != '0'
PAIR_MIN_TILES = int(os.environ.get('UPSNET_CONV1X1_PAIR_MIN_TILES', '1024'))


PAIR_RES3 = os.environ.get('UPSNET_CONV1X1_PAIR_RES3', '1') != '0'
PAIR_RES4 = os.environ.get('UPSNET_CONV1X1_PAIR_RES4', '1') != '0'


def use_pair(m3, m1, x, residual):
    if not (PAIR and CONV1X1 and PRECISION == 'fp32' and supported(m3, x) and residual is not None and isinstance(m1, nn.Conv2d)):
        return False
    ok = lambda m: (tuple(m.kernel_size) == (1, 1) and tuple(m.stride) == (1, 1) and tuple(m.padding) == (0, 0) and m.groups == 1)
    if not (ok(m3) and ok(m1) and m3.out_channels % 128 == 0 and m1.in_channels == m3.out_channels):
        return False
    tiles = x.shape[0] * x.shape[2] * x.shape[3] // 64
    if m3.in_channels == 64 and m1.out_channels == 64:
        return tiles >= PAIR_MIN_TILES
    if PAIR_RES3 and m3.in_channels == 128 and m1.out_channels == 128:
        return tiles >= PAIR_MIN_TILES // 2
    if PAIR_RES4 and m3.in_channels == 256 and m1.out_channels == 256:
        return 2 * tiles >= PAIR_MIN_TILES // 4
    return False


def conv_pair(m3, m1, x, residual):
    out1, out2 = ops.conv1x1_pair(x, residual, _conv1x1_plan(m3), m3.bias, m3.out_channels, _conv1x1_plan(m1), m1.bias, m1.out_channels)
    _trace('conv', module=m3, x=x, out=out1, relu=True, residual=residual, residual_up=False, form='pair(conv3)')
    _trace('conv', module=m1, x=out1, out=out2, relu=True, residual=None, residual_up=False, form='pair(conv1)')
    return out1, out2


SIBLINGS = os.environ.get('UPSNET_CONV1X1_SIBLINGS', '1') != '0'


def use_siblings(ma, mb, x):
    if not (SIBLINGS and CONV1X1 and PRECISION == 'fp32' and isinstance(ma, nn.Conv2d) and isinstance(mb, nn.Conv2d) and supported(ma, x) and
            supported(mb, x) and x.dtype == torch.float32):
        return False
    ok = lambda m: tuple(m.kernel_size) == (1, 1) and tuple(m.padding) == (0, 0) and m.groups == 1 and m.stride[0] in (1, 2)
    if not (_use_conv1x1(ma, x) and _use_conv1x1(mb, x)):
        return False
    return (ok(ma) and ok(mb) and ma.stride == mb.stride and ma.in_channels == mb.in_channels and ma.in_channels % 32 == 0 and
            ma.out_channels % 32 == 0 and (ma.bias is None) == (mb.bias is None))


def conv_siblings(ma, mb, x, relu_a=True, relu_b=False):
    wp, b = ops.cached_pack(ma, 'siblings', (ma.weight, ma.bias, mb.weight, mb.bias), lambda: (
        ops.pack_conv1x1_weight(torch.cat([ma.weight.detach(), mb.weight.detach()], 0)),
        None if ma.bias is None else torch.cat([ma.bias.detach(), mb.bias.detach()], 0).contiguous()))
    ya, yb = ops.conv1x1_siblings(x, wp, b, ma.out_channels, mb.out_channels, ma.stride[0], relu_a=relu_a, relu_b=relu_b)
    _trace('conv', module=ma, x=x, out=ya, relu=relu_a, residual=None, residual_up=False, form='conv1x1 siblings(a)')
    _trace('conv', module=mb, x=x, out=yb, relu=relu_b, residual=None, residual_up=False, form='conv1x1 siblings(b)')
    return ya, yb


def supported(m, x):
    return (ENABLED and isinstance(m, nn.Conv2d) and x.is_cuda and
            (x.dtype == torch.float32 or (x.dtype == torch.bfloat16 and PRECISION == 'bf16')) and
            ops.conv_supported(m.in_channels, m.kernel_size[0], m.kernel_size[1], m.groups, m.dilation) and
            m.stride[0] == m.stride[1] and m.padding[0] == m.padding[1] and m.padding_mode == 'zeros')


BF16_MIN_WG = int(os.environ.get('UPSNET_BF16_MIN_WG', '192'))
BF16_MIN_WG_WREG = int(os.environ.get('UPSNET_BF16_MIN_WG_WREG', '16'))


def _use_bf16(m, xs, always=False):
    if PRECISION == 'fp32' or m.kernel_size[0] * m.kernel_size[1] > 9 or m.out_channels < 64:
        return False
    if always or xs[0].dtype == torch.bfloat16:
        return True
    k, st, pd, dl = m.kernel_size[0], m.stride[0], m.padding[0], m.dilation[0]
    wgs = 0
    for x in xs:
        ho, wo = (x.shape[2] + 2 * pd - (dl * (k - 1) + 1)) // st + 1, (x.shape[3] + 2 * pd - (dl * (k - 1) + 1)) // st + 1
        wgs += -(-(x.shape[0] * ho * wo) // 128)
    small_ok = PRECISION == 'bf16' and k == 3 and st == 1 and dl == 1 and m.out_channels % 256 == 0
    return wgs * -(-m.out_channels // 128) >= (BF16_MIN_WG_WREG if small_ok else BF16_MIN_WG)


def _bf16_form():
    return PRECISION if TRACE is None else '%s %s' % (PRECISION, ops.last_kernel_form())


def _bf16_plan(m):
    return _pack(m, 'bf16', lambda w: ops.pack_conv_weight_bf16(w, split=(PRECISION == 'bf16x3')), PRECISION)


BF16_BLOCK = os.environ.get('UPSNET_BF16_BLOCK', '1') != '0'
BF16_BLOCK_MIN_TILES = int(os.environ.get('UPSNET_BF16_BLOCK_MIN_TILES', '128'))
BF16_PROJ = os.environ.get('UPSNET_BF16_PROJ', '1') != '0'


def use_block(blk, x):
    if not (ENABLED and BF16_BLOCK and PRECISION == 'bf16' and BF16_ACT and x.is_cuda and x.dtype == torch.bfloat16 and not blk.deformable):
        return False
    c1, c2, c3 = blk.conv1, blk.conv2, blk.conv3
    cm, cin, st = c1.out_channels, c1.in_channels, c1.stride[0]
    plain = lambda m, k, p, s=1: (tuple(m.kernel_size) == (k, k) and tuple(m.stride) == (s, s) and tuple(m.padding) == (p, p) and
                                  tuple(m.dilation) == (1, 1) and m.groups == 1)
    if not (plain(c2, 3, 1) and plain(c3, 1, 0) and c2.in_channels == cm and c2.out_channels == cm and c3.in_channels == cm and
            c3.out_channels == 4 * cm):
        return False
    ho, wo = (x.shape[2] - 1) // st + 1, (x.shape[3] - 1) // st + 1
    th, tw = {64: (8, 16), 128: (8, 8)}.get(cm, (4, 8))
    if x.shape[0] * -(-ho // th) * -(-wo // tw) < BF16_BLOCK_MIN_TILES or x.shape[0] * ho * wo * 4 * cm >= (1 << 30):
        return False
    if blk.downsample is None:
        return cm in (64, 128, 256, 512) and plain(c1, 1, 0) and cin == 4 * cm
    pr = blk.downsample[0]
    return (BF16_PROJ and isinstance(pr, nn.Conv2d) and len(blk.downsample) == 2 and isinstance(blk.downsample[1], nn.Identity) and
            st in (1, 2) and plain(c1, 1, 0, st) and plain(pr, 1, 0, st) and pr.in_channels == cin and pr.out_channels == 4 * cm and
            (cm, cin) in ((64, 64), (128, 256), (256, 512)))


def block(blk, x):
    ms = (blk.conv1, blk.conv2, blk.conv3) + (() if blk.downsample is None else (blk.downsample[0],))
    pack = ops.pack_bottleneck_bf16 if blk.downsample is None else ops.pack_bottleneck_proj_bf16
    p = ops.cached_pack(blk.conv1, 'block16', [t for m in ms for t in (m.weight, m.bias)], lambda: pack(*(m.weight for m in ms), *(m.bias for m in ms)))
    if blk.downsample is None:
        y = ops.bottleneck_bf16(x, p)
    else:
        y = ops.bottleneck_proj_bf16(x, p, blk.conv1.stride[0])
    _trace('block', module=blk, x=x, out=y, form='bottleneck_bf16' if blk.downsample is None else 'bottleneck_proj_bf16')
    return y


def _winograd_plan(m, tn32=False):
    return _pack(m, 'wino32' if tn32 else 'wino', lambda w: ops.pack_winograd_weight(w, tn32=tn32))


WINO_TAIL_SPLIT = os.environ.get('UPSNET_WINO_TAIL_SPLIT', '1') != '0'


def _wino_tail_split(m, x):
    if not WINO_TAIL_SPLIT or x.shape[0] < 2 or m.out_channels % 64:
        return 0
    cus = _cus(x.device)
    n, tiles, nt = x.shape[0], ((x.shape[2] + 1) // 2) * ((x.shape[3] + 1) // 2), m.out_channels // 64
    slots = 2 * cus
    wgs = -(-(n * tiles) // 32) * nt
    if wgs <= slots or _wino_tm(m, [x]) != 32:
        return 0
    n_main = ((wgs // slots) * slots // nt) * 32 // tiles
    fit = (cus // (m.out_channels // 32)) * 32 // tiles
    n_main = min(n_main, n - fit) if n - fit > 0 else n_main
    tail = n - n_main
    if n_main <= 0 or tail <= 0 or -(-(tail * tiles) // 32) * (m.out_channels // 32) > cus:
        return 0
    return n_main


WINO_TAIL_FUSED = os.environ.get('UPSNET_WINO_TAIL_FUSED', '1') != '0'


def _wino_split_launch(m, x, n_main, relu):
    wp, ldw = _winograd_plan(m)
    if WINO_TAIL_FUSED:
        wp32, ldw32 = _winograd_plan(m, tn32=True)
        return ops.conv2d_winograd_tail(x, wp, ldw, wp32, ldw32, m.bias, m.out_channels, n_main, relu=relu)
    out = ops._nhwc_out(x.shape[0], m.out_channels, x.shape[2], x.shape[3], x.device)
    ops.conv2d_winograd_multi([x[:n_main]], wp, ldw, m.bias, m.out_channels, relu=relu, outs=[out[:n_main]])
    wp32, ldw32 = _winograd_plan(m, tn32=True)
    ops.conv2d_winograd_multi([x[n_main:]], wp32, ldw32, m.bias, m.out_channels, relu=relu, outs=[out[n_main:]], tn32=True)
    return out


def _winograd36_plan(m):
    return _pack(m, 'wino36', ops.pack_winograd36_weight)


def _winograd36_shape_ok(m):
    return (tuple(m.kernel_size) == (3, 3) and tuple(m.stride) == (1, 1) and tuple(m.padding) == (1, 1) and tuple(m.dilation) == (1, 1) and
            m.in_channels % 32 == 0 and m.out_channels % 64 == 0)


def _use_winograd36(m, xs):
    if not (WINO36 and WINOGRAD and _winograd36_shape_ok(m) and all(x.dtype == torch.float32 for x in xs)):
        return False
    cus = _cus(xs[0].device)
    wgs = sum(-(-(x.shape[0] * ((x.shape[2] + 3) // 4) * ((x.shape[3] + 3) // 4)) // 32) for x in xs) * (m.out_channels // 64)
    if cus // 2 <= wgs < cus and m.in_channels >= 256:
        return True
    return wgs >= cus and wgs >= WINO36_MIN_FILL * (-(-wgs // cus)) * cus


WINO36_PREFIX = os.environ.get('UPSNET_WINO36_PREFIX', '0') != '0'


def _wino36_round_prefix(m, xs):
    n = len(xs)
    if not WINO36_PREFIX or n < 2:
        return n
    cus = _cus(xs[0].device)
    per = [-(-(x.shape[0] * ((x.shape[2] + 3) // 4) * ((x.shape[3] + 3) // 4)) // 32) * (m.out_channels // 64) for x in xs]
    fill = lambda w: w / float(-(-w // cus) * cus)
    last = sum(per) % cus
    if last == 0 or last >= cus // 2:
        return n
    for k in range(n - 1, 0, -1):
        w = sum(per[:k])
        if w >= cus and fill(w) >= 0.95:
            return k
    return n


def _wino36_ksplit(m, x):
    if not (WINO36 and WINOGRAD and _winograd36_shape_ok(m) and x.dtype == torch.float32):
        return 1
    cus = _cus(x.device)
    wgs = -(-(x.shape[0] * ((x.shape[2] + 3) // 4) * ((x.shape[3] + 3) // 4)) // 32) * (m.out_channels // 64)
    if wgs >= cus or wgs < cus // 4 or (wgs >= cus // 2 and m.in_channels >= 256):
        return 1
    ks = min(cus // wgs, (m.in_channels // 16) // 4, 8)
    return ks if ks >= 2 else 1


def _use_winograd(m, xs, always=False):
    if not (WINOGRAD and tuple(m.kernel_size) == (3, 3) and tuple(m.stride) == (1, 1) and tuple(m.padding) == (1, 1) and
            tuple(m.dilation) == (1, 1) and m.in_channels % 16 == 0):
        return False
    if always:
        return True
    return _wino_workgroups(m, xs, _wino_tm(m, xs)) * _wino_ksplit(m, xs) >= WINOGRAD_MIN_WORKGROUPS


def _wino_workgroups(m, xs, tm=64):
    tiles = sum(-(-(x.shape[0] * ((x.shape[2] + 1) // 2) * ((x.shape[3] + 1) // 2)) // tm) for x in xs)
    return tiles * (1 if m.out_channels <= 32 else -(-m.out_channels // 64))


def _wino_tm(m, xs):
    return 64 if m.out_channels > 32 and _wino_workgroups(m, xs, 64) > WINO_TM64_MIN else 32


def _wino_ksplit(m, xs):
    if not SPLITK or len(xs) != 1 or m.out_channels % 4 or _wino_tm(m, xs) == 64:
        return 1
    wgs, slabs = _wino_workgroups(m, xs, 32), m.in_channels // 16
    if wgs >= 256:
        return 1
    k = 1
    while k < 8 and wgs * (k + 1) <= 512 and slabs // (k + 1) >= 4:
        k += 1
    return k


def _ksplit(m, x, ldw):
    if not SPLITK:
        return 1
    k, st, pd = m.kernel_size[0], m.stride[0], m.padding[0]
    pix = x.shape[0] * ((x.shape[2] + 2 * pd - k) // st + 1) * ((x.shape[3] + 2 * pd - k) // st + 1)
    slabs = k * k * m.in_channels // 32
    if ldw == 32:
        blocks, ks = -(-pix // 128), 1
        while ks < 8 and blocks * (ks + 1) <= 384 and slabs // (ks + 1) >= 6:
            ks += 1
        while ks > 1 and -(-slabs // ks) * (ks - 1) >= slabs:
            ks -= 1
        return ks
    if ldw % 64 or m.out_channels % 4:
        return 1
    blocks = -(-pix // 64) * (ldw // 64)
    if blocks <= 128 and slabs >= 32:
        return 4
    if blocks <= 256 and slabs >= 128:
        return 3
    return 1


def conv(m, x, relu=False, residual=None, residual_up=False, winograd=True, pin=False, out_dtype=None):
    if x.dtype == torch.bfloat16 and not (supported(m, x) and _use_bf16(m, [x])):
        x = x.float()
    if residual is not None and residual.dtype == torch.bfloat16 and not (supported(m, x) and _use_bf16(m, [x], always=pin or winograd == 'always')):
        residual = residual.float()
    y, form = _conv(m, x, relu, residual, residual_up, winograd, pin or winograd == 'always', out_dtype)
    _trace('conv', module=m, x=x, out=y, relu=relu, residual=residual, residual_up=residual_up, form=form)
    return y


def _conv(m, x, relu=False, residual=None, residual_up=False, winograd=True, pin=False, out_dtype=None):
    if supported(m, x):
        if (not residual_up or tuple(m.kernel_size) == (1, 1)) and _use_bf16(m, [x], always=pin):
            hi, lo, ldw = _bf16_plan(m)
            od = out_dtype if (out_dtype == torch.bfloat16 and lo is None) else torch.float32
            return ops.conv2d_nhwc_bf16_multi([x], hi, lo, ldw, m.bias, m.out_channels, m.kernel_size[0], m.stride[0], m.padding[0],
                                              relu=relu, residuals=None if residual is None else [residual],
                                              residual_up=residual_up, out_dtype=od)[0], _bf16_form()
        if winograd is True and not pin and residual is None and WINO36_SPLITK and _wino36_ksplit(m, x) > 1:
            wp, ldw = _winograd36_plan(m)
            ks = _wino36_ksplit(m, x)
            return ops.conv2d_winograd36_splitk(x, wp, ldw, m.bias, m.out_channels, ks, relu=relu), 'winograd36 splitk%d' % ks
        if winograd is True and not pin and residual is None and _use_winograd36(m, [x]):
            wp, ldw = _winograd36_plan(m)
            return ops.conv2d_winograd36_multi([x], wp, ldw, m.bias, m.out_channels, relu=relu)[0], 'winograd36'
        if (winograd == 'always' and WINO36 and WINO36_ROI and residual is None and x.dtype == torch.float32 and _winograd36_shape_ok(m) and
                x.shape[2] * x.shape[3] <= 1024):
            wp, ldw = _winograd36_plan(m)
            return ops.conv2d_winograd36_multi([x], wp, ldw, m.bias, m.out_channels, relu=relu)[0], 'winograd36 roi'
        if winograd and not residual_up and _use_winograd(m, [x], always=(winograd == 'always')):
            wp, ldw = _winograd_plan(m)
            ks = 1 if winograd == 'always' else _wino_ksplit(m, [x])
            if ks > 1:
                return ops.conv2d_winograd_splitk(x, wp, ldw, m.bias, m.out_channels, ks, relu=relu, residual=residual), 'winograd splitk%d' % ks
            n_main = _wino_tail_split(m, x) if (residual is None and x.dtype == torch.float32) else 0
            if n_main:
                return _wino_split_launch(m, x, n_main, relu), 'winograd tm32 + tail tn32'
            return ops.conv2d_winograd_multi([x], wp, ldw, m.bias, m.out_channels, relu=relu,
                                             residuals=None if residual is None else [residual])[0], 'winograd tm%d' % _wino_tm(m, [x])
        if not pin and residual is None and _use_ksw3(m, x):
            return ops.conv3x3_ksw(x, _ksw3_plan(m), m.bias, m.out_channels, relu=relu), 'conv3x3 ksw 16x32'
        if not pin and not residual_up and _use_ksw(m, x):
            return ops.conv1x1_ksw(x, _ksw_plan(m), m.bias, m.out_channels, KSW_TILE, stride=m.stride[0], relu=relu,
                                   residual=residual), 'conv1x1 ksw %dx%d' % KSW_TILE
        if _use_conv1x1(m, x, always=pin):
            if not pin and not residual_up and m.stride[0] == 1:
                return _conv1x1_balanced(m, x, relu, residual)
            return ops.conv1x1_frag(x, _conv1x1_plan(m), m.bias, m.out_channels, m.stride[0], relu=relu, residual=residual,
                                    residual_up=residual_up), 'conv1x1'
        wp, ldw = _plan(m)
        ks = 1 if (residual_up or pin) else _ksplit(m, x, ldw)
        if ks > 1:
            return ops.conv2d_nhwc_splitk(x, wp, ldw, m.bias, m.out_channels, m.kernel_size[0], m.stride[0], m.padding[0], ks,
                                          relu=relu, residual=residual), 'igemm splitk%d' % ks
        return ops.conv2d_nhwc(x, wp, ldw, m.bias, m.out_channels, m.kernel_size[0], m.stride[0], m.padding[0],
                               relu=relu, residual=residual, residual_up=residual_up), 'igemm'
    _library(m, x, 'hipconv.supported() is false')
    y = m(x)
    if residual is not None:
        y = y + (F.interpolate(residual, scale_factor=2, mode='nearest') if residual_up else residual)
    return (F.relu(y, inplace=True) if relu else y), 'library'


def conv_multi(m, xs, relu=False):
    xs = list(xs)
    if len(xs) <= 5 and all(supported(m, x) for x in xs):
        if _use_bf16(m, xs):
            hi, lo, ldw = _bf16_plan(m)
            ys, form = ops.conv2d_nhwc_bf16_multi(xs, hi, lo, ldw, m.bias, m.out_channels, m.kernel_size[0], m.stride[0], m.padding[0], relu=relu), _bf16_form()
        elif _use_winograd36(m, xs):
            wp, ldw = _winograd36_plan(m)
            k = _wino36_round_prefix(m, xs)
            if k < len(xs):
                ys = ops.conv2d_winograd36_multi(xs[:k], wp, ldw, m.bias, m.out_channels, relu=relu)
                for x, y in zip(xs[:k], ys):
                    _trace('conv', module=m, x=x, out=y, relu=relu, residual=None, residual_up=False, form='winograd36 multi')
                return ys + conv_multi(m, xs[k:], relu=relu)
            ys, form = ops.conv2d_winograd36_multi(xs, wp, ldw, m.bias, m.out_channels, relu=relu), 'winograd36 multi'
        elif _use_winograd(m, xs):
            wp, ldw = _winograd_plan(m)
            ys, form = ops.conv2d_winograd_multi(xs, wp, ldw, m.bias, m.out_channels, relu=relu), 'winograd tm%d multi' % _wino_tm(m, xs)
        else:
            wp, ldw = _plan(m)
            ys, form = ops.conv2d_nhwc_multi(xs, wp, ldw, m.bias, m.out_channels, m.kernel_size[0], m.stride[0], m.padding[0], relu=relu), 'igemm multi'
        for x, y in zip(xs, ys):
            _trace('conv', module=m, x=x, out=y, relu=relu, residual=None, residual_up=False, form=form)
        return ys
    return [conv(m, x, relu=relu) for x in xs]


def stem_supported(m, x):
    return (ENABLED and isinstance(m, nn.Conv2d) and x.is_cuda and x.dtype == torch.float32 and m.in_channels <= 4 and
            m.kernel_size[1] <= 8 and m.groups == 1 and tuple(m.dilation) == (1, 1) and m.stride[0] == m.stride[1] and
            m.padding[0] == m.padding[1] and m.padding_mode == 'zeros')


def conv_stem(m, x, relu=False):
    if not stem_supported(m, x):
        _library(m, x, 'hipconv.stem_supported() is false')
        y = m(x[:, :m.in_channels] if x.shape[1] != m.in_channels else x)
        return F.relu(y, inplace=True) if relu else y
    wp, ldw = _pack(m, 'stem', ops.pack_stem_weight)
    is_nhwc4 = x.shape[1] == 4 and x.is_contiguous(memory_format=torch.channels_last)
    x4 = x if is_nhwc4 else ops.image_to_nhwc4(x)
    y = ops.conv2d_stem(x4, wp, ldw, m.bias, m.out_channels, m.kernel_size[0], m.kernel_size[1], m.stride[0], m.padding[0], relu=relu)
    _trace('conv', module=m, x=x4[:, :m.in_channels], out=y, relu=relu, residual=None, residual_up=False, form='stem')
    return y


STEM_POOL = os.environ.get('UPSNET_STEM_POOL', '1') != '0'
BF16_STEM = os.environ.get('UPSNET_BF16_STEM', '1') != '0'


def _stem_geometry(m, x):
    return (ENABLED and stem_supported(m, x) and m.out_channels == 64 and m.in_channels <= 3 and tuple(m.kernel_size) == (7, 7) and
            tuple(m.stride) == (2, 2) and tuple(m.padding) == (3, 3))


def use_stem_pool(m, x):
    if not _stem_geometry(m, x):
        return None
    if PRECISION == 'bf16' and BF16_ACT and BF16_STEM:
        return 'bf16'
    return 'f32' if STEM_POOL else None


def stem_pool(m, x):
    kind = use_stem_pool(m, x)
    wp = _pack(m, 'stem_pool_' + kind, ops.pack_stem_pool_weight_bf16 if kind == 'bf16' else ops.pack_stem_pool_weight_f32)
    is_nhwc4 = x.shape[1] == 4 and x.is_contiguous(memory_format=torch.channels_last)
    x4 = x if is_nhwc4 else ops.image_to_nhwc4(x)
    y = ops.stem_pool_bf16(x4, wp, m.bias) if kind == 'bf16' else ops.stem_pool_f32(x4, wp, m.bias)
    _trace('stem_pool', module=m, x=x4[:, :m.in_channels], out=y, form='stem + pool bf16' if kind == 'bf16' else 'stem + pool')
    return y


DECONV_FRAG = os.environ.get('UPSNET_DECONV_FRAG', '1') != '0'


def deconv2x2(m, x, relu=False):
    geom = (ENABLED and isinstance(m, nn.ConvTranspose2d) and x.is_cuda and tuple(m.kernel_size) == (2, 2) and
            tuple(m.stride) == (2, 2) and tuple(m.padding) == (0, 0) and tuple(m.output_padding) == (0, 0) and m.groups == 1 and
            tuple(m.dilation) == (1, 1) and m.in_channels % 32 == 0)
    if geom and x.dtype == torch.bfloat16 and PRECISION == 'bf16' and m.in_channels % 64 == 0 and m.out_channels % 32 == 0:
        whi, ldw = _pack(m, 'deconv16', ops.pack_deconv2x2_weight_bf16)
        y = ops.deconv2x2_bf16(x, whi, ldw, m.bias, m.out_channels, relu=relu)
        _trace('deconv', module=m, x=x, out=y, relu=relu, form='deconv2x2 bf16')
        return y
    if x.dtype == torch.bfloat16:
        x = x.float()
    ok = geom and x.dtype == torch.float32
    if not ok:
        _library(m, x, 'not a 2x2 / stride-2 transposed convolution with Cin % 32 == 0')
        y = m(x)
        return F.relu(y, inplace=True) if relu else y
    if DECONV_FRAG and m.out_channels % 32 == 0:
        wp, bias4 = _pack(m, 'deconv_frag', lambda w: ops.pack_deconv2x2_weight_frag(w, m.bias))
        y = ops.deconv2x2_frag(x, wp, bias4, m.out_channels, relu=relu)
        _trace('deconv', module=m, x=x, out=y, relu=relu, form='deconv2x2 frag')
        return y
    wp, ldw = _pack(m, 'deconv', ops.pack_deconv2x2_weight)
    y = ops.deconv2x2(x, wp, ldw, m.bias, m.out_channels, relu=relu)
    _trace('deconv', module=m, x=x, out=y, relu=relu, form='deconv2x2')
    return y


def dcn(m, x, offset, relu=False):
    if (ENABLED and x.is_cuda and x.shape[0] == 1 and not torch.is_grad_enabled() and
            ops.fused_dcn_supported(m.in_channels, m.out_channels, m.deformable_groups, m.groups, m.padding, m.stride, m.dilation)):
        return ops.deform_conv_fused([x], [offset], ops.cached_dcn_pack(m.weight), m.bias, m.in_channels, m.out_channels, m.kernel_size,
                                     m.stride, m.padding, m.dilation, relu=relu)[0]
    y = m(x, offset)
    return torch.relu_(y) if relu else y


def head_norm(with_norm):
    assert with_norm in ['batch_norm', 'group_norm', 'none']
    if with_norm == 'batch_norm':
        raise NotImplementedError(
            "with_norm='batch_norm': the reference takes this layer from upsnet/operators/modules/distbatchnorm.py (a synchronised "
            "BatchNorm2d imported only under Horovod + syncbn), which is not part of its tree -- there is no BatchNorm2d to reproduce; "
            "use 'group_norm' or 'none'")
    return None if with_norm == 'none' else (lambda num_channels: nn.GroupNorm(32, num_channels))


def norm_supported(gn, x):
    return (ENABLED and isinstance(gn, nn.GroupNorm) and gn.affine and x.is_cuda and x.dim() in (2, 4) and x.shape[1] == gn.num_channels and
            group_norm.supported(gn.num_channels, gn.num_groups))


def _norm_library(gn, x, relu, residual, residual_up):
    _library(gn, x, 'hipconv.norm_supported() is false')
    y = gn(x)
    if residual is not None:
        y = y + (F.interpolate(residual, scale_factor=2, mode='nearest') if residual_up else residual)
    return F.relu(y, inplace=True) if relu else y


def norm(gn, x, relu=False, residual=None, residual_up=False):
    if norm_supported(gn, x):
        if x.dim() == 2 or (residual is None and x.shape[2] * x.shape[3] <= group_norm.chunk_pixels()):
            y = group_norm.group_norm_small(x, gn.weight, gn.bias, gn.eps, relu=relu)
            form = 'gn rows' if x.dim() == 2 or x.shape[2] * x.shape[3] == 1 else 'gn small'
        else:
            y, form = group_norm.group_norm(x, gn.weight, gn.bias, gn.eps, relu=relu, residual=residual, residual_up=residual_up), 'gn'
    else:
        y, form = _norm_library(gn, x, relu, residual, residual_up), 'library'
    _trace('gn', module=gn, x=x, out=y, relu=relu, residual=residual, residual_up=residual_up, form=form)
    return y


def norm_multi(gn, xs, relu=False):
    xs = list(xs)
    if 1 <= len(xs) <= group_norm.MAX_MAPS and all(x.dim() == 4 and norm_supported(gn, x) for x in xs):
        ys = group_norm.group_norm_multi(xs, gn.weight, gn.bias, gn.eps, relu=relu)
        for x, y in zip(xs, ys):
            _trace('gn', module=gn, x=x, out=y, relu=relu, residual=None, residual_up=False, form='gn multi')
        return ys
    return [norm(gn, x, relu=relu) for x in xs]


def clear_cache(model=None):
    if model is not None:
        for m in model.modules():
            m.__dict__.pop('_hip_plans', None)
            for p in m.parameters(recurse=False):
                p.__dict__.pop('_hip_plans', None)


def conv_multi_cat(ms, xs, return_flat=False):
    xs = list(xs)
    m0 = ms[0]
    same = all(isinstance(m, nn.Conv2d) and m.kernel_size == m0.kernel_size and m.stride == m0.stride and m.padding == m0.padding and
               m.dilation == m0.dilation and m.in_channels == m0.in_channels and (m.bias is None) == (m0.bias is None) for m in ms)
    couts = [m.out_channels for m in ms]
    if (not same or any(_use_bf16(m, xs) for m in ms) or xs[0].dtype != torch.float32 or len(xs) > 5 or
            not all(supported(m0, x) for x in xs) or
            (sum(couts) + 31) // 32 != 1 or _use_winograd(m0, xs)):
        res = [conv_multi(m, xs) for m in ms]
        return (res, None, None) if return_flat else res
    (wp, ldw), b = ops.cached_pack(m0, 'cat', [t for m in ms for t in (m.weight, m.bias)], lambda: (
        ops.pack_conv_weight(torch.cat([m.weight.detach() for m in ms], 0)),
        None if m0.bias is None else torch.cat([m.bias.detach() for m in ms], 0)))
    outs = ops.conv2d_nhwc_multi(xs, wp, ldw, b, sum(couts), m0.kernel_size[0], m0.stride[0], m0.padding[0], relu=False)
    res, c0 = [], 0
    for m, c in zip(ms, couts):
        res.append([o[:, c0:c0 + c] for o in outs])
        for x, y in zip(xs, res[-1]):
            _trace('conv', module=m, x=x, out=y, relu=False, residual=None, residual_up=False, form='igemm multi cat')
        c0 += c
    if return_flat:
        return res, getattr(outs[0], '_ups_flat', None), outs
    return res
```

upsnet_amd/ops.py:

```python
import os

import numpy as np
import torch

from . import _lib
from ._lib import check, f32c, float_array, int_array, lib, nhwc, ptr, ptr_array, require_cuda, stream


PROFILE = {'enabled': False, 'events': []}


def _prof_begin():
    if not PROFILE['enabled']:
        return None
    ev0 = torch.cuda.Event(enable_timing=True)
    ev0.record()
    return ev0


def _prof_end(ev0, kind, flops, nbytes, label=None):
    ev1 = torch.cuda.Event(enable_timing=True)
    ev1.record()
    PROFILE['events'].append((kind, ev0, ev1, flops, nbytes) if label is None else (kind, ev0, ev1, flops, nbytes, label))

# ... 1020 lines not shown
    check(lib().upsnet_unified_pan_result(stream(), ptr(pan), ptr(seg), ptr(cls_inds) if cls_inds.numel() else None, int(cls_inds.numel()),
                                          H, W, int(id_last_stuff), int(num_seg_classes), int(stuff_area_limit), ptr(ws), ptr(out)),
          "unified_pan_result")
    return out


COMBINED_PAN_CHUNK_IMAGES = 256
COMBINED_PAN_CHUNK_PIXELS = 1 << 28
_SEG_BLOCK = 4096


def _combined_seg_u8(seg, dev):
    if isinstance(seg, torch.Tensor):
        t = seg
    else:
        a = np.asarray(seg)
        if a.ndim == 2 and a.dtype != np.uint8 and a.size:
            if not np.issubdtype(a.dtype, np.integer) or int(a.min()) < 0 or int(a.max()) > 255:
                raise ValueError("combined_pan_result: semantic labels must be integers in 0..255")
            a = a.astype(np.uint8)
        t = torch.from_numpy(np.ascontiguousarray(a))
    if t.dim() != 2:
        raise ValueError("combined_pan_result: semantic maps must be [H,W], got %s" % (tuple(t.shape),))
    if t.dtype != torch.uint8 and (t.dtype.is_floating_point or t.dtype.is_complex or t.dtype == torch.bool):
        raise ValueError("combined_pan_result: semantic maps must be uint8 or int64, got %s" % t.dtype)
    return t.to(dev)


def combined_pan_result(segs, boxes, masks, id_last_stuff, score_threshold=0.6, fraction_threshold=0.7, stuff_area_limit=4 * 64 * 64):
    from .dataset.rle import _segmented_cumsum, decode_rle_strings
    n = len(segs)
    if len(boxes) != len(masks):
        raise ValueError("combined_pan_result: %d classes of boxes, %d of masks" % (len(boxes), len(masks)))
    num_classes = len(boxes)
    if num_classes < 2 or id_last_stuff < 0 or id_last_stuff + num_classes - 1 >= 255:
        raise ValueError("combined_pan_result: %d classes after id_last_stuff %d do not fit the uint8 labels" % (num_classes, id_last_stuff))
    for c in range(1, num_classes):
        if len(boxes[c]) != n or len(masks[c]) != n:
            raise ValueError("combined_pan_result: class %d has boxes for %d and masks for %d of %d images" % (c, len(boxes[c]), len(masks[c]), n))
    if n == 0:
        return []
    dev = next((s.device for s in segs if isinstance(s, torch.Tensor) and s.is_cuda), None) or torch.device('cuda', torch.cuda.current_device())
    seg_t = [_combined_seg_u8(s, dev) for s in segs]
    wide = [t for t in seg_t if t.dtype != torch.uint8 and t.numel()]
    if wide:
        r = torch.stack([torch.stack([t.min(), t.max()]).to(torch.int64) for t in wide]).cpu()
        if int(r[:, 0].min()) < 0 or int(r[:, 1].max()) > 255:
            raise ValueError("combined_pan_result: semantic labels must be integers in 0..255")
    seg_t = [t.to(torch.uint8).contiguous() for t in seg_t]
    thr = float(score_threshold)
    strings, cls_of, npix_of, img_ncand = [], [], [], []
    for i, t in enumerate(seg_t):
        H, W = int(t.shape[0]), int(t.shape[1])
        if H * W > (1 << 24):
            raise ValueError("combined_pan_result: image %d has %d x %d pixels; the pixel counts are exact only up to 2^24" % (i, H, W))
        sc, cl, rl = [], [], []
        for c in range(1, num_classes):
            b, m = boxes[c][i], masks[c][i]
            b = np.asarray(b)
            nb = b.shape[0] if b.size else 0
            if nb != len(m):
                raise ValueError("combined_pan_result: image %d class %d: %d boxes, %d masks" % (i, c, nb, len(m)))
            if nb:
                if b.ndim != 2 or b.shape[1] < 5:
                    raise ValueError("combined_pan_result: image %d class %d: boxes must be [n,5], got %s" % (i, c, b.shape))
                sc.append(b[:, 4].astype(np.float64))
                cl.append(np.full(nb, c, np.int32))
                rl.extend(m)
        for r in rl:
            if not isinstance(r, dict) or [int(v) for v in r.get('size', ())] != [H, W]:
                raise ValueError("combined_pan_result: image %d: mask size %s differs from the semantic map's %s" %
                                 (i, r.get('size') if isinstance(r, dict) else type(r), [H, W]))
        if sc:
            s = np.concatenate(sc)
            order = np.argsort(s, kind='stable')[::-1]
            order = order[~(s[order] < thr)]
            cls = np.concatenate(cl)[order]
            per = np.bincount(cls, minlength=num_classes)
            if per.max(initial=0) > 255:
                raise ValueError("combined_pan_result: image %d class %d has %d candidates at or above the score threshold; the "
                                 "instance ids are uint8" % (i, int(per.argmax()), int(per.max())))
            for k in order:
                cnt = rl[k]['counts']
                if not isinstance(cnt, (str, bytes)):
                    raise ValueError("combined_pan_result: image %d: RLE counts must be a compressed string" % i)
                strings.append(cnt)
            cls_of.append(cls)
        npix_of.append(np.full(len(order) if sc else 0, H * W, np.int64))
        img_ncand.append(len(order) if sc else 0)
    cls_all = np.concatenate(cls_of) if cls_of else np.zeros(0, np.int32)
    npix_all = np.concatenate(npix_of)
    counts, off = decode_rle_strings(strings)
    ncodes = np.diff(off)
    str_of = np.repeat(np.arange(len(strings)), ncodes)
    if counts.size and counts.min() < 0:
        raise ValueError("combined_pan_result: negative RLE count (string %d)" % int(str_of[np.argmax(counts < 0)]))
    total = np.bincount(str_of, weights=counts.astype(np.float64), minlength=len(strings))
    bad = np.flatnonzero(total != npix_all)
    if bad.size:
        raise ValueError("combined_pan_result: RLE counts of candidate %d sum to %d, not H * W = %d" %
                         (int(bad[0]), int(total[bad[0]]), int(npix_all[bad[0]])))
    first = np.zeros(counts.size, bool)
    first[off[:-1][ncodes > 0]] = True
    pos = _segmented_cumsum(counts, first) if counts.size else counts
    j = np.arange(counts.size) - np.repeat(off[:-1], ncodes)
    odd = np.flatnonzero(((j & 1) == 1) & (counts > 0))
    run_b = pos[odd]
    run_a = run_b - counts[odd]
    run_str = str_of[odd]
    area = np.bincount(run_str, weights=(run_b - run_a).astype(np.float64), minlength=len(strings)).astype(np.int64)
    blk_a, blk_b = run_a // _SEG_BLOCK, (run_b - 1) // _SEG_BLOCK
    nseg = blk_b - blk_a + 1
    run_idx = np.repeat(np.arange(run_a.size), nseg)
    blk = blk_a[run_idx] + (np.arange(run_idx.size) - np.repeat(np.cumsum(nseg) - nseg, nseg))
    seg_a = np.maximum(run_a[run_idx], blk * _SEG_BLOCK)
    seg_b = np.minimum(run_b[run_idx], (blk + 1) * _SEG_BLOCK)
    seg_str = run_str[run_idx]
    seg_cnt = np.bincount(seg_str, minlength=len(strings))
    keep = area > 0
    cand_img = np.repeat(np.arange(n), img_ncand)
    out = [torch.empty((int(t.shape[0]), int(t.shape[1]), 3), dtype=torch.uint8, device=dev) for t in seg_t]
    live = [i for i in range(n) if seg_t[i].numel()]
    chunks, cur, cur_pix = [], [], 0
    for i in live:
        p = seg_t[i].numel()
        if cur and (len(cur) >= COMBINED_PAN_CHUNK_IMAGES or cur_pix + p > COMBINED_PAN_CHUNK_PIXELS):
            chunks.append(cur)
            cur, cur_pix = [], 0
        cur.append(i)
        cur_pix += p
    if cur:
        chunks.append(cur)
    for ch in chunks:
        in_chunk = keep & np.isin(cand_img, ch)
        sel = np.flatnonzero(in_chunk)
        cbeg = np.concatenate([[0], np.cumsum(np.bincount(np.searchsorted(ch, cand_img[sel]), minlength=len(ch)))])
        segs_sel = np.flatnonzero(in_chunk[seg_str])
        c_seg_end = np.cumsum(seg_cnt[sel])
        cand = np.stack([cls_all[sel], area[sel], c_seg_end - seg_cnt[sel], c_seg_end], 1).astype(np.int32) if sel.size else None
        segs_np = np.stack([seg_a[segs_sel], seg_b[segs_sel]], 1).astype(np.int32) if segs_sel.size else None
        hw = np.array([[int(seg_t[i].shape[0]), int(seg_t[i].shape[1])] for i in ch], np.int64)
        npx = hw[:, 0] * hw[:, 1]
        img = np.zeros((len(ch), 8), np.int64)
        img[:, 0:2] = hw
        img[:, 2] = [seg_t[i].data_ptr() for i in ch]
        img[:, 3] = [out[i].data_ptr() for i in ch]
        img[:, 4], img[:, 5] = cbeg[:-1], cbeg[1:]
        img[:, 6] = np.concatenate([[0], np.cumsum((npx + 63) // 64)[:-1]])
        img[:, 7] = np.concatenate([[0], np.cumsum(npx)[:-1]])
        total_pix = int(npx.sum())
        img_d = torch.from_numpy(img).to(dev)
        cand_d = torch.from_numpy(cand).to(dev) if cand is not None else None
        segs_d = torch.from_numpy(segs_np).to(dev) if segs_np is not None else None
        ws = torch.empty((int(lib().upsnet_combined_pan_workspace_bytes(len(ch), total_pix)),), dtype=torch.uint8, device=dev)
        check(lib().upsnet_combined_pan_result(stream(), len(ch), ptr(img_d), int(hw[:, 0].max()), int(hw[:, 1].max()), total_pix,
                                               ptr(cand_d), ptr(segs_d), int(id_last_stuff), num_classes, int(stuff_area_limit),
                                               float(fraction_threshold), ptr(ws)), "combined_pan_result")
    return out


def pq_workspace(max_gt, device):
    nbytes = int(lib().upsnet_pq_workspace_bytes(int(max_gt)))
    if nbytes == 0:
        raise ValueError("pq_workspace: max_gt %d outside 0..4096" % max_gt)
    return torch.zeros((nbytes,), dtype=torch.uint8, device=device)


def pq_accumulate(pred_2ch, gt_rgb, segments, cat_known, image_index, max_gt, workspace, tp, fp, fn, iou, status):
    require_cuda(pred_2ch, gt_rgb, segments, cat_known, workspace, tp, fp, fn, iou, status)
    if pred_2ch.dtype != torch.uint8 or gt_rgb.dtype != torch.uint8 or pred_2ch.dim() != 3 or pred_2ch.shape[2] != 3 \
            or tuple(pred_2ch.shape) != tuple(gt_rgb.shape):
        raise ValueError("pq_accumulate: pred_2ch %s %s and gt_rgb %s %s must both be uint8 [H,W,3]"
                         % (tuple(pred_2ch.shape), pred_2ch.dtype, tuple(gt_rgb.shape), gt_rgb.dtype))
    if segments.dtype != torch.int64 or segments.dim() != 2 or segments.shape[1] != 4:
        raise ValueError("pq_accumulate: segments must be int64 [n,4]")
    for t, dt, n in ((cat_known, torch.uint8, 256), (tp, torch.int64, 256), (fp, torch.int64, 256), (fn, torch.int64, 256),
                     (iou, torch.float64, 256), (status, torch.int64, 1)):
        if t.dtype != dt or t.numel() != n or not t.is_contiguous():
            raise ValueError("pq_accumulate: accumulator / table of %d %s expected, got %s %s" % (n, dt, tuple(t.shape), t.dtype))
    pred_2ch, gt_rgb, segments = pred_2ch.contiguous(), gt_rgb.contiguous(), segments.contiguous()
    H, W = pred_2ch.shape[:2]
    check(lib().upsnet_pq_accumulate(stream(), ptr(pred_2ch), ptr(gt_rgb), H, W, ptr(segments) if segments.numel() else None,
                                     int(segments.shape[0]), ptr(cat_known), int(image_index), int(max_gt), ptr(workspace), ptr(tp), ptr(fp),
                                     ptr(fn), ptr(iou), ptr(status)), "pq_accumulate")


def confusion_accumulate(gt_label, pred_label, class_num, ignore_label, confusion):
    require_cuda(gt_label, pred_label, confusion)
    if gt_label.dtype != torch.uint8 or pred_label.dtype != torch.uint8 or gt_label.shape != pred_label.shape:
        raise ValueError("confusion_accumulate: gt %s %s and pred %s %s must both be uint8 of one shape"
                         % (tuple(gt_label.shape), gt_label.dtype, tuple(pred_label.shape), pred_label.dtype))
    if confusion.dtype != torch.int64 or tuple(confusion.shape) != (class_num, class_num) or not confusion.is_contiguous():
        raise ValueError("confusion_accumulate: confusion must be a contiguous int64 [%d,%d] tensor" % (class_num, class_num))
    gt_label, pred_label = gt_label.contiguous(), pred_label.contiguous()
    check(lib().upsnet_confusion_accumulate(stream(), ptr(gt_label), ptr(pred_label), int(gt_label.numel()), int(class_num),
                                            int(ignore_label), ptr(confusion)), "confusion_accumulate")
    return confusion


def mask_roi_dedup(a_src, a_cls, a_num, b_src, b_cls, b_boxes, b_num):
    require_cuda(a_src, b_src, b_boxes)
    cap_a, cap_b = a_src.shape[0], b_src.shape[0]
    dev = b_boxes.device
    mp = torch.empty((cap_b,), dtype=torch.int32, device=dev)
    extra = torch.empty((cap_b, 5), dtype=torch.float32, device=dev)
    n_extra = torch.empty((1,), dtype=torch.int32, device=dev)
    check(lib().upsnet_mask_roi_dedup(stream(), ptr(a_src), ptr(a_cls), ptr(a_num), cap_a, ptr(b_src), ptr(b_cls), ptr(f32c(b_boxes)),
                                      ptr(b_num), cap_b, ptr(mp), ptr(extra), ptr(n_extra)), "mask_roi_dedup")
    return mp, extra, n_extra


def pack_winograd_weight(weight, tn32=False):
    require_cuda(weight)
    weight = f32c(weight)
    Cout, Cin, kh, kw = weight.shape
    if (kh, kw) != (3, 3):
        raise RuntimeError("pack_winograd_weight: kernel must be 3x3")
    if tn32:
        ldw = (Cout + 31) // 32 * 32
        wp = torch.empty((16 * Cin, ldw), dtype=torch.float32, device=weight.device)
        check(lib().upsnet_conv_pack_weight_winograd_tn32(stream(), ptr(weight), Cout, Cin, ldw, ptr(wp)), "conv_pack_weight_winograd_tn32")
        return wp, ldw
    ldw = 32 if Cout <= 32 else (Cout + 63) // 64 * 64
    wp = torch.empty((16 * Cin, ldw), dtype=torch.float32, device=weight.device)
    check(lib().upsnet_conv_pack_weight_winograd(stream(), ptr(weight), Cout, Cin, ldw, ptr(wp)), "conv_pack_weight_winograd")
    return wp, ldw


def conv2d_winograd_splitk(x, wpack, ldw, bias, cout, ksplit, relu=False, residual=None):
    require_cuda(x, wpack)
    x = nhwc(x.float())
    N, C, H, W = x.shape
    out = _nhwc_out(N, cout, H, W, x.device)
    res = None
    if residual is not None:
        res = nhwc(residual.float())
        if tuple(res.shape) != tuple(out.shape):
            raise RuntimeError("conv2d_winograd_splitk: residual shape %s != %s" % (tuple(res.shape), tuple(out.shape)))
    ws = _ws(lib().upsnet_conv2d_splitk_workspace_bytes(N, H, W, int(cout), 3, 3, 1, 1, int(ksplit)), x.device)
    ev0 = _prof_begin()
    check(lib().upsnet_conv2d_winograd_nhwc_f32_splitk(stream(), ptr(x), ptr(res), ptr(out), N, H, W, C, ptr(wpack), int(ldw),
                                                       ptr(None if bias is None else f32c(bias)), int(cout), int(bool(relu)), int(ksplit),
                                                       ptr(ws)), "conv2d_winograd_nhwc_f32_splitk")
    if ev0 is not None:
        npix = N * H * W
        _prof_end(ev0, 'conv', 2.0 * cout * C * 9 * npix, 4.0 * (C * npix + cout * npix * (2 if res is not None else 1) + cout * C * 9),
                  "winograd split-K x%d 3x3/1 %d->%d %s" % (ksplit, C, cout, (N, H, W)))
    return out


def conv2d_winograd_tail(x, wpack, ldw, wpack32, ldw32, bias, cout, n_main, relu=False):
    require_cuda(wpack, wpack32, x)
    x = nhwc(x.float())
    N, C, H, W = x.shape
    out = _nhwc_out(N, cout, H, W, x.device)
    ev0 = _prof_begin()
    check(lib().upsnet_conv2d_winograd_nhwc_f32_tail(stream(), ptr(x), ptr(out), int(N), int(n_main), int(H), int(W), int(C), ptr(wpack), int(ldw),
                                                     ptr(wpack32), int(ldw32), ptr(None if bias is None else f32c(bias)), int(cout),
                                                     int(bool(relu))), "conv2d_winograd_nhwc_f32_tail")
    if ev0 is not None:
        npix = N * H * W
        _prof_end(ev0, 'conv', 2.0 * cout * C * 9 * npix, 4.0 * (C * npix + cout * npix + cout * C * 9),
                  "winograd 3x3/1 %d->%d [%s] tail %d" % (C, cout, (N, H, W), N - n_main))
    return out


def conv2d_winograd_multi(xs, wpack, ldw, bias, cout, relu=False, residuals=None, outs=None, tn32=False):
    require_cuda(wpack, *xs)
    assert 1 <= len(xs) <= 5
    xs = [nhwc(x.float()) for x in xs]
    cin = xs[0].shape[1]
    given, outs, ress = outs, [], None
    for i, x in enumerate(xs):
        N, C, H, W = x.shape
        if C != cin:
            raise RuntimeError("conv2d_winograd_multi: channel mismatch")
        if given is not None:
            o = given[i]
            if tuple(o.shape) != (N, cout, H, W) or o.dtype != torch.float32 or not o.permute(0, 2, 3, 1).is_contiguous():
                raise RuntimeError("conv2d_winograd_multi: outs[%d] must be a channels_last fp32 [%d,%d,%d,%d]" % (i, N, cout, H, W))
            outs.append(o)
        else:
            outs.append(_nhwc_out(N, cout, H, W, x.device))
    if residuals is not None:
        ress = [nhwc(r.float()) for r in residuals]
        for r, o in zip(ress, outs):
            if tuple(r.shape) != tuple(o.shape):
                raise RuntimeError("conv2d_winograd: residual shape %s != %s" % (tuple(r.shape), tuple(o.shape)))
    ev0 = _prof_begin()
    fn = lib().upsnet_conv2d_winograd_nhwc_f32_tn32 if tn32 else lib().upsnet_conv2d_winograd_nhwc_f32
    check(fn(stream(), len(xs), ptr_array(xs), ptr_array(ress) if ress is not None else None,
             ptr_array(outs), int_array([x.shape[0] for x in xs]), int_array([x.shape[2] for x in xs]),
             int_array([x.shape[3] for x in xs]), int(cin), ptr(wpack), int(ldw),
             ptr(None if bias is None else f32c(bias)), int(cout), int(bool(relu))),
          "conv2d_winograd_nhwc_f32")
    if ev0 is not None:
        npix = sum(o.shape[0] * o.shape[2] * o.shape[3] for o in outs)
        _prof_end(ev0, 'conv', 2.0 * cout * cin * 9 * npix, 4.0 * (cin * npix + cout * npix * (2 if ress is not None else 1) + cout * cin * 9),
                  "winograd 3x3/1 %d->%d %s%s%s" % (cin, cout, [tuple(x.shape[0:1] + x.shape[2:]) for x in xs],
                                                    " +res" if ress is not None else "", " tn32" if tn32 else ""))
    return outs


def pack_winograd36_weight(weight):
    require_cuda(weight)
    weight = f32c(weight)
    Cout, Cin, kh, kw = weight.shape
    if (kh, kw) != (3, 3) or Cin % 32:
        raise RuntimeError("pack_winograd36_weight: 3x3 kernel and Cin %% 32 == 0")
    ldw = (Cout + 63) // 64 * 64
    wp = torch.empty((36 * Cin, ldw), dtype=torch.float32, device=weight.device)
    check(lib().upsnet_conv_pack_weight_winograd36(stream(), ptr(weight), Cout, Cin, ldw, ptr(wp)), "conv_pack_weight_winograd36")
    return wp, ldw


def conv2d_winograd36_multi(xs, wpack, ldw, bias, cout, relu=False, outs=None):
    require_cuda(wpack, *xs)
    assert 1 <= len(xs) <= 5
    xs = [nhwc(x.float()) for x in xs]
    cin = xs[0].shape[1]
    given, outs = outs, []
    for i, x in enumerate(xs):
        N, C, H, W = x.shape
        if C != cin:
            raise RuntimeError("conv2d_winograd36_multi: channel mismatch")
        if given is not None:
            o = given[i]
            if tuple(o.shape) != (N, cout, H, W) or o.dtype != torch.float32 or not o.permute(0, 2, 3, 1).is_contiguous():
                raise RuntimeError("conv2d_winograd36_multi: outs[%d] must be a channels_last fp32 [%d,%d,%d,%d]" % (i, N, cout, H, W))
            outs.append(o)
        else:
            outs.append(_nhwc_out(N, cout, H, W, x.device))
    ev0 = _prof_begin()
    check(lib().upsnet_conv2d_winograd36_nhwc_f32(stream(), len(xs), ptr_array(xs), ptr_array(outs), int_array([x.shape[0] for x in xs]),
                                                  int_array([x.shape[2] for x in xs]), int_array([x.shape[3] for x in xs]), int(cin), ptr(wpack),
                                                  int(ldw), ptr(None if bias is None else f32c(bias)), int(cout), int(bool(relu))),
          "conv2d_winograd36_nhwc_f32")
    if ev0 is not None:
        npix = sum(o.shape[0] * o.shape[2] * o.shape[3] for o in outs)
        _prof_end(ev0, 'conv', 2.0 * cout * cin * 9 * npix, 4.0 * (cin * npix + cout * npix + cout * cin * 9),
                  "winograd36 3x3/1 %d->%d %s" % (cin, cout, [tuple(x.shape[0:1] + x.shape[2:]) for x in xs]))
    return outs


def conv2d_winograd36_splitk(x, wpack, ldw, bias, cout, ksplit, relu=False):
    require_cuda(wpack, x)
    x = nhwc(x.float())
    N, cin, H, W = x.shape
    out = _nhwc_out(N, cout, H, W, x.device)
    ws = _ws(lib().upsnet_conv2d_winograd36_splitk_workspace_bytes(N, H, W, int(cout), int(ksplit)), x.device)
    ev0 = _prof_begin()
    check(lib().upsnet_conv2d_winograd36_nhwc_f32_splitk(stream(), ptr(x), ptr(out), N, H, W, int(cin), ptr(wpack), int(ldw),
                                                         ptr(None if bias is None else f32c(bias)), int(cout), int(bool(relu)), int(ksplit), ptr(ws)),
          "conv2d_winograd36_nhwc_f32_splitk")
    if ev0 is not None:
        npix = N * H * W
        _prof_end(ev0, 'conv', 2.0 * cout * cin * 9 * npix, 4.0 * (cin * npix + cout * npix + cout * cin * 9),
                  "winograd36 split-K x%d 3x3/1 %d->%d %s" % (ksplit, cin, cout, (N, H, W)))
    return out


def pack_conv_weight_bf16(weight, split=True):
    require_cuda(weight)
    weight = f32c(weight)
    Cout, Cin, kh, kw = weight.shape
    ldw = (Cout + 127) // 128 * 128
    shape = (kh * kw * Cin // 32, ldw, 32)
    hi = torch.empty(shape, dtype=torch.bfloat16, device=weight.device)
    lo = torch.empty(shape, dtype=torch.bfloat16, device=weight.device) if split else None
    check(lib().upsnet_conv_pack_weight_bf16(stream(), ptr(weight), Cout, Cin, kh, kw, ldw, ptr(hi), ptr(lo)), "conv_pack_weight_bf16")
    return hi, lo, ldw


def conv2d_nhwc_bf16_multi(xs, whi, wlo, ldw, bias, cout, ksize, stride, pad, relu=False, residuals=None, residual_up=False,
                           out_dtype=torch.float32):
    require_cuda(whi, *xs)
    assert 1 <= len(xs) <= 5
    in16 = xs[0].dtype == torch.bfloat16
    out16 = out_dtype == torch.bfloat16
    if (in16 or out16) and wlo is not None:
        raise RuntimeError("conv2d_nhwc_bf16_multi: bf16 tensors only in the plain bf16 mode")
    xs = [nhwc(x if (in16 and x.dtype == torch.bfloat16) else x.float()) for x in xs]
    if in16 and any(x.dtype != torch.bfloat16 for x in xs):
        raise RuntimeError("conv2d_nhwc_bf16_multi: mixed input dtypes in one launch")
    cin = xs[0].shape[1]
    outs, ress = [], None
    for x in xs:
        N, C, H, W = x.shape
        if C != cin:
            raise RuntimeError("conv2d_nhwc_bf16_multi: channel mismatch")
        Ho, Wo = (H + 2 * pad - ksize) // stride + 1, (W + 2 * pad - ksize) // stride + 1
        outs.append(torch.empty((N, Ho, Wo, cout), dtype=torch.bfloat16, device=x.device).permute(0, 3, 1, 2) if out16
                    else _nhwc_out(N, cout, Ho, Wo, x.device))
    res16 = False
    if residuals is not None:
        res16 = residuals[0].dtype == torch.bfloat16 and wlo is None
        ress = [nhwc(r if (res16 and r.dtype == torch.bfloat16) else r.float()) for r in residuals]
        if res16 and any(r.dtype != torch.bfloat16 for r in ress):
            raise RuntimeError("conv2d_nhwc_bf16_multi: mixed residual dtypes in one launch")
        for r, o in zip(ress, outs):
            want = (o.shape[0], o.shape[1], o.shape[2] // 2, o.shape[3] // 2) if residual_up else tuple(o.shape)
            if tuple(r.shape) != want:
                raise RuntimeError("conv2d_nhwc_bf16: residual shape %s != %s" % (tuple(r.shape), want))
    ev0 = _prof_begin()
    check(lib().upsnet_conv2d_nhwc_bf16(stream(), len(xs), ptr_array(xs), ptr_array(ress) if ress is not None else None, ptr_array(outs),
                                        int_array([x.shape[0] for x in xs]), int_array([x.shape[2] for x in xs]),
                                        int_array([x.shape[3] for x in xs]), int(cin), ptr(whi), ptr(wlo), int(ldw),
                                        ptr(None if bias is None else f32c(bias)), int(cout), int(ksize), int(ksize), int(stride), int(pad),
                                        int(bool(relu)) | (2 if (residual_up and ress is not None) else 0) | (4 if in16 else 0) |
                                        (8 if out16 else 0) | (16 if res16 else 0)), "conv2d_nhwc_bf16")
    if ev0 is not None:
        npix = sum(o.shape[0] * o.shape[2] * o.shape[3] for o in outs)
        nin = sum(x.shape[0] * x.shape[2] * x.shape[3] for x in xs)
        _prof_end(ev0, 'conv_bf16', 2.0 * cout * cin * ksize * ksize * npix,
                  (2.0 if in16 else 4.0) * cin * nin + (2.0 if out16 else 4.0) * cout * npix +
                  ((2.0 if res16 else 4.0) * cout * npix * (0.25 if residual_up else 1.0) if ress is not None else 0.0) +
                  2.0 * cout * cin * ksize * ksize)
    return outs


def _bf16_fragments(w2d):
    cout, k = w2d.shape
    return w2d.to(torch.bfloat16).view(cout // 32, 32, k // 16, 2, 8).permute(0, 2, 3, 1, 4).contiguous()


def pack_bottleneck_bf16(w1, w2, w3, b1, b2, b3):
    require_cuda(w1, w2, w3)
    cm, c = w1.shape[0], w1.shape[1]
    if not (c == 4 * cm and tuple(w2.shape) == (cm, cm, 3, 3) and tuple(w3.shape) == (c, cm, 1, 1) and cm in (64, 128, 256, 512)):
        raise RuntimeError("pack_bottleneck_bf16: not an identity bottleneck of width 64/128/256/512")
    zeros = lambda n: torch.zeros(n, dtype=torch.float32, device=w1.device)
    return (_bf16_fragments(w1.detach().float().reshape(cm, c)),
            _bf16_fragments(w2.detach().float().permute(0, 2, 3, 1).reshape(cm, 9 * cm)),
            _bf16_fragments(w3.detach().float().reshape(c, cm)),
            zeros(cm) if b1 is None else f32c(b1.detach()), zeros(cm) if b2 is None else f32c(b2.detach()),
            zeros(c) if b3 is None else f32c(b3.detach()), cm)


def pack_bottleneck_proj_bf16(w1, w2, w3, wd, b1, b2, b3, bd):
    require_cuda(w1, w2, w3, wd)
    cm, cin = w1.shape[0], w1.shape[1]
    c = 4 * cm
    if not (tuple(w2.shape) == (cm, cm, 3, 3) and tuple(w3.shape) == (c, cm, 1, 1) and tuple(wd.shape) == (c, cin, 1, 1) and
            (cm, cin) in ((64, 64), (128, 256), (256, 512))):
        raise RuntimeError("pack_bottleneck_proj_bf16: not the first bottleneck of res2 / res3 / res4")
    z = lambda b, n: torch.zeros(n, dtype=torch.float32, device=w1.device) if b is None else f32c(b.detach())
    w3d = torch.cat([w3.detach().float().reshape(c, cm), wd.detach().float().reshape(c, cin)], 1)
    return (_bf16_fragments(w1.detach().float().reshape(cm, cin)),
            _bf16_fragments(w2.detach().float().permute(0, 2, 3, 1).reshape(cm, 9 * cm)),
            _bf16_fragments(w3d), z(b1, cm), z(b2, cm), (z(b3, c) + z(bd, c)).contiguous(), cm, cin)


def bottleneck_proj_bf16(x, pack, stride):
    w1, w2, w3d, b1, b2, b3d, cm, cin = pack
    require_cuda(x, w1)
    if x.dtype != torch.bfloat16 or x.shape[1] != cin:
        raise RuntimeError("bottleneck_proj_bf16: expects a bf16 map of %d channels" % cin)
    x = nhwc(x)
    N, C, H, W = x.shape
    Ho, Wo = (H - 1) // stride + 1, (W - 1) // stride + 1
    out = torch.empty((N, Ho, Wo, 4 * cm), dtype=torch.bfloat16, device=x.device).permute(0, 3, 1, 2)
    ev0 = _prof_begin()
    check(lib().upsnet_bottleneck_proj_bf16(stream(), ptr(x), ptr(out), N, H, W, int(cin), int(cm), int(stride), ptr(w1), ptr(w2), ptr(w3d),
                                            ptr(b1), ptr(b2), ptr(b3d)), "bottleneck_proj_bf16")
    if ev0 is not None:
        k = cm * cin + 9 * cm * cm + 4 * cm * (cm + cin)
        _prof_end(ev0, 'bottleneck_bf16', 2.0 * k * N * Ho * Wo, 2.0 * C * N * Ho * Wo + 2.0 * 4 * cm * N * Ho * Wo + 2.0 * k)
    return out


def bottleneck_bf16(x, pack):
    w1, w2, w3, b1, b2, b3, cm = pack
    require_cuda(x, w1)
    if x.dtype != torch.bfloat16 or x.shape[1] != 4 * cm:
        raise RuntimeError("bottleneck_bf16: expects a bf16 map of %d channels" % (4 * cm))
    x = nhwc(x)
    N, C, H, W = x.shape
    out = torch.empty((N, H, W, C), dtype=torch.bfloat16, device=x.device).permute(0, 3, 1, 2)
    ev0 = _prof_begin()
    check(lib().upsnet_bottleneck_bf16(stream(), ptr(x), ptr(out), N, H, W, cm, ptr(w1), ptr(w2), ptr(w3), ptr(b1), ptr(b2), ptr(b3)),
          "bottleneck_bf16")
    if ev0 is not None:
        _prof_end(ev0, 'bottleneck_bf16', 2.0 * 17 * cm * cm * N * H * W, 2.0 * 2 * C * N * H * W + 2.0 * 17 * cm * cm)
    return out


def conv2d_nhwc_splitk(x, wpack, ldw, bias, cout, ksize, stride, pad, ksplit, relu=False, residual=None):
    require_cuda(x, wpack)
    x = nhwc(x.float())
    N, C, H, W = x.shape
    Ho, Wo = (H + 2 * pad - ksize) // stride + 1, (W + 2 * pad - ksize) // stride + 1
    out = _nhwc_out(N, cout, Ho, Wo, x.device)
    res = None
    if residual is not None:
        res = nhwc(residual.float())
        if tuple(res.shape) != tuple(out.shape):
            raise RuntimeError("conv2d_nhwc_splitk: residual shape %s != %s" % (tuple(res.shape), tuple(out.shape)))
    ws = _ws(lib().upsnet_conv2d_splitk_workspace_bytes(N, H, W, int(cout), int(ksize), int(ksize), int(stride), int(pad), int(ksplit)), x.device)
    ev0 = _prof_begin()
    check(lib().upsnet_conv2d_nhwc_f32_splitk(stream(), ptr(x), ptr(res), ptr(out), N, H, W, C, ptr(wpack), int(ldw),
                                              ptr(None if bias is None else f32c(bias)), int(cout), int(ksize), int(ksize), int(stride),
                                              int(pad), int(bool(relu)), int(ksplit), ptr(ws)), "conv2d_nhwc_f32_splitk")
    if ev0 is not None:
        npix = N * Ho * Wo
        _prof_end(ev0, 'conv', 2.0 * cout * C * ksize * ksize * npix,
                  4.0 * (C * N * H * W + cout * npix * (2 if res is not None else 1) + cout * C * ksize * ksize),
                  "split-K x%d %dx%d/%d %d->%d %s" % (ksplit, ksize, ksize, stride, C, cout, (N, H, W)))
    return out


PROPOSAL_RECALL_MAX_GT = 4096


def proposal_recall_workspace_bytes(num_problems, total_proposals):
    return int(lib().upsnet_proposal_recall_workspace_bytes(int(num_problems), int(total_proposals)))


def proposal_recall(problems, proposals, gt_boxes, max_gt, total_proposals, workspace, out):
    require_cuda(problems, proposals, gt_boxes, workspace, out)
    if problems.dtype != torch.int64 or problems.dim() != 2 or problems.shape[1] != 6 or not problems.is_contiguous():
        raise ValueError("proposal_recall: problems must be a contiguous int64 [n, 6] table, got %s %s" % (problems.dtype, tuple(problems.shape)))
    for name, b in (('proposals', proposals), ('gt_boxes', gt_boxes)):
        if b.dtype != torch.float32 or b.dim() != 2 or b.shape[1] != 4 or not b.is_contiguous():
            raise ValueError("proposal_recall: %s must be contiguous float32 [., 4], got %s %s" % (name, b.dtype, tuple(b.shape)))
    if not 0 <= int(max_gt) <= PROPOSAL_RECALL_MAX_GT:
        raise ValueError("proposal_recall: %d GT boxes in a problem (at most %d)" % (int(max_gt), PROPOSAL_RECALL_MAX_GT))
    n = int(problems.shape[0])
    if workspace.numel() * workspace.element_size() < proposal_recall_workspace_bytes(n, total_proposals):
        raise ValueError("proposal_recall: workspace of %d bytes, %d needed" % (workspace.numel() * workspace.element_size(),
                                                                             proposal_recall_workspace_bytes(n, total_proposals)))
    if out.dtype != torch.float32 or not out.is_contiguous():
        raise ValueError("proposal_recall: out must be contiguous float32")
    check(lib().upsnet_proposal_recall(stream(), n, ptr(problems), ptr(proposals), ptr(gt_boxes), int(max_gt), int(total_proposals),
                                       ptr(workspace), ptr(out)), "proposal_recall")
    return out


def gt_prepare_workspace(device, seg_capacity=4096):
    from .dataset import gt_prepare as impl
    return impl.gt_prepare_workspace(device, seg_capacity)


def gt_prepare_launch(ids, tables, label_ids=None, seg_capacity=4096, trans_capacity=None, workspace=None):
    from .dataset import gt_prepare as impl
    return impl.gt_prepare_launch(ids, tables, label_ids, seg_capacity, trans_capacity, workspace)


def gt_prepare(ids, tables, label_ids=None, seg_capacity=4096, trans_capacity=None, workspace=None):
    from .dataset import gt_prepare as impl
    return impl.gt_prepare(ids, tables, label_ids, seg_capacity, trans_capacity, workspace)


def panoptic_semantic(rgb, segments_info):
    from .dataset import gt_prepare as impl
    return impl.panoptic_semantic(rgb, segments_info)


TTA_MAX_AUG = 8


def tta_seg_merge(maps, q, resized_w, flip, cell):
    from . import tta as impl
    return impl.seg_merge(maps, q, resized_w, flip, cell)


def tta_roi_union(rois, delta, prob, num_rois_dev, r, resized_w, flip):
    from . import tta as impl
    return impl.roi_union(rois, delta, prob, num_rois_dev, r, resized_w, flip)


def tta_boxes_to_aug(boxes, q, resized_w, flip):
    from . import tta as impl
    return impl.boxes_to_aug(boxes, q, resized_w, flip)


def tta_mask_merge(logits, flip):
    from . import tta as impl
    return impl.mask_merge(logits, flip)
```

Measured before the change: 170.0.

## Add 16-tile x 128-channel Winograd F(4x4,3x3) kernel for large single-map convs

Adds a new Winograd F(4x4,3x3) MFMA kernel that works on 16 tiles by 128 output channels per workgroup with 512 threads. Four waves transform the input while all eight do the MFMAs, and weights stream through a register ring of buffer loads. The matching weight packing is added, and the kernel is selected by default for Cout%128 single-map launches with at least two rounds of workgroups (FPN P2). The aim is more weight reuse per input transform and better MFMA utilisation, at the cost of a new, complex code path with occupancy 1 and possible tail imbalance.

```diff
diff --git a/include/upsnet_hip.h b/include/upsnet_hip.h
--- a/include/upsnet_hip.h
+++ b/include/upsnet_hip.h
@@ -185,6 +185,10 @@
                                       const int height[], const int width[], int Cin, const float *wpack, int ldw, const float *bias,
                                       int Cout, int relu);
 int upsnet_conv_pack_weight_winograd36(void *stream, const float *weight, int cout, int cin, int ldw, float *wpack);
+int upsnet_conv2d_winograd36_n128_nhwc_f32(void *stream, int nseg, const float *const x[], const float *const residual[], float *const out[],
+                                           const int batch[], const int height[], const int width[], int Cin, const float *wpack, int ldw,
+                                           const float *bias, int Cout, int relu);
+int upsnet_conv_pack_weight_winograd36_n128(void *stream, const float *weight, int cout, int cin, int ldw, float *wpack);
 size_t upsnet_conv2d_winograd36_splitk_workspace_bytes(int batch, int height, int width, int Cout, int ksplit);
 int upsnet_conv2d_winograd36_nhwc_f32_splitk(void *stream, const float *x, float *out, int batch, int height, int width, int Cin,
                                              const float *wpack, int ldw, const float *bias, int Cout, int relu, int ksplit, void *workspace);
diff --git a/upsnet_amd/_lib.py b/upsnet_amd/_lib.py
--- a/upsnet_amd/_lib.py
+++ b/upsnet_amd/_lib.py
@@ -104,6 +104,8 @@
     "upsnet_conv2d_winograd_nhwc_f32_tail": (c_int, [P, P, P, c_int, c_int, c_int, c_int, c_int, P, c_int, P, c_int, P, c_int, c_int]),
     "upsnet_conv2d_winograd36_nhwc_f32": (c_int, [P, c_int, P, P, P, P, P, c_int, P, c_int, P, c_int, c_int]),
     "upsnet_conv_pack_weight_winograd36": (c_int, [P, P, c_int, c_int, c_int, P]),
+    "upsnet_conv2d_winograd36_n128_nhwc_f32": (c_int, [P, c_int, P, P, P, P, P, P, c_int, P, c_int, P, c_int, c_int]),
+    "upsnet_conv_pack_weight_winograd36_n128": (c_int, [P, P, c_int, c_int, c_int, P]),
     "upsnet_conv2d_nhwc_bf16": (c_int, [P, c_int, P, P, P, P, P, P, c_int, P, P, c_int, P, c_int, c_int, c_int, c_int, c_int, c_int]),
     "upsnet_bottleneck_proj_bf16": (c_int, [P, P, P, c_int, c_int, c_int, c_int, c_int, c_int, P, P, P, P, P, P]),
     "upsnet_conv_bf16_tuning": (c_int, [c_int, c_int]),
diff --git a/upsnet_amd/csrc/conv_params.h b/upsnet_amd/csrc/conv_params.h
--- a/upsnet_amd/csrc/conv_params.h
+++ b/upsnet_amd/csrc/conv_params.h
@@ -35,11 +35,11 @@
 static inline int conv_fill(ConvParams &p, const char *who, int nseg, const float *const x[], const float *const res[],
                      const float *const off[], const float *const mask[], float *const out[], const int batch[],
                      const int height[], const int width[], int Cin, int Cout, const float *wpack, int ldw, const float *bias,
-                     int KH, int KW, int stride, int pad, int dil, int relu)
+                     int KH, int KW, int stride, int pad, int dil, int relu, int cin_mult = CV_BK)
 {
     UPS_REQUIRE(nseg >= 1 && nseg <= CV_MAXSEG, "%s: 1..%d feature maps per launch (got %d)", who, CV_MAXSEG, nseg);
     UPS_REQUIRE(x && out && height && width && wpack, "%s: null pointer", who);
-    UPS_REQUIRE(Cin > 0 && Cin % CV_BK == 0, "%s: Cin must be a multiple of 32 (got %d)", who, Cin);
+    UPS_REQUIRE(Cin > 0 && Cin % cin_mult == 0, "%s: Cin must be a multiple of %d (got %d)", who, cin_mult, Cin);
     UPS_REQUIRE(Cout > 0 && ldw % 32 == 0 && ldw >= Cout, "%s: ldw must be Cout rounded up to 32 (got %d for Cout=%d)", who, ldw, Cout);
     UPS_REQUIRE(KH >= 1 && KW >= 1 && KH * KW <= 49 && stride >= 1 && pad >= 0 && dil >= 1, "%s: bad kernel/stride/pad/dilation", who);
     UPS_REQUIRE((long)KH * KW * Cin * ldw < (1L << 30), "%s: packed weight exceeds 4 GiB", who);
diff --git a/upsnet_amd/csrc/conv_wino36.hip b/upsnet_amd/csrc/conv_wino36.hip
--- a/upsnet_amd/csrc/conv_wino36.hip
+++ b/upsnet_amd/csrc/conv_wino36.hip
@@ -202,12 +202,6 @@
     }
     };
     if (risky) slab_loop(std::false_type{}); else slab_loop(std::true_type{});
-#undef W36_LOADROW_FAST
-#undef W36_LOADROW_SAFE
-#undef W36_ROWOFF
-#undef W36_FIXROW
-#undef W36_ROWPASS
-#undef W36_COLSTASH
 #undef W36_BLOAD
 
     const unsigned crow = (unsigned)p.Cout * 4u;
@@ -262,11 +256,240 @@
     }
 }
 
+#define W36N_TM 16
+#define W36N_TN 128
+#define W36N_VBUF (W36_PTS * 4 * W36N_TM * 16)
+#define W36N_BBLK 1024
+#define W36N_BXI (8 * W36N_BBLK)
+#define W36N_BSLAB (W36_PTS * W36N_BXI)
+#define W36N_XCH (W36N_TM * W36_PTS * 64 * 4)
+#define W36N_RING 4
+#define W36N_SWZ(Q) ((((Q) & 1) << 1) | (((Q) >> 1) * 12))
+
+typedef float w36_floatx4 __attribute__((ext_vector_type(4)));
+
+__global__ void __launch_bounds__(512, 1) conv_wino36_n128_f32_kernel(const ConvParams p)
+{
+    extern __shared__ __attribute__((aligned(16))) unsigned char smem_raw[];
+    const int tid = threadIdx.x, lane = tid & 63;
+    const int wave = __builtin_amdgcn_readfirstlane(tid >> 6);
+    const int cg = wave >> 2, pg = wave & 3;
+    const int kq = lane >> 4, l16 = lane & 15;
+    int m_t, n_t;
+    {
+        const int nt = p.n_tiles;
+        const int per = (p.m_tiles + 7) >> 3;
+        const int bid = (int)blockIdx.x;
+        const int q = bid >> 3;
+        n_t = q % nt;
+        const int local = q / nt;
+        m_t = (bid & 7) * per + local;
+        if (local >= per || m_t >= p.m_tiles) return;
+    }
+    int si = 0;
+#pragma unroll
+    for (int q = 1; q < CV_MAXSEG; ++q) if (q < p.nseg && m_t >= p.seg[q].tile_start) si = q;
+    const ConvSeg sg = p.seg[si];
+    const long p0 = (long)(m_t - sg.tile_start) * W36N_TM;
+    const int nslabs = p.Cin >> 4;
+    const long HoWo = (long)sg.Ho * sg.Wo;
+
+    const int ltile = (tid >> 4) & 15, lch = tid & 15;
+    int hrow0, wcol0, hlo, hhi;
+    unsigned tbase, nrmask = 0, ncmask = 0;
+    bool lane_fix;
+    {
+        const long pp = p0 + ltile;
+        const bool tile_ok = pp < sg.M;
+        const long ppc = tile_ok ? pp : sg.M - 1;
+        const int n = (int)(ppc / HoWo);
+        const int rem = (int)(ppc - (long)n * HoWo);
+        const int ty = rem / sg.Wo, tx = rem - ty * sg.Wo;
+        const int h0 = 4 * ty - 1;
+        hlo = n * sg.H; hhi = tile_ok ? hlo + sg.H : hlo;
+        hrow0 = hlo + h0;
+        wcol0 = 4 * tx - 1;
+#pragma unroll
+        for (int r = 0; r < 6; ++r) nrmask |= (h0 + r >= 0 && h0 + r < sg.H) ? 0u : (1u << r);
+#pragma unroll
+        for (int c = 0; c < 6; ++c) ncmask |= (wcol0 + c >= 0 && wcol0 + c < sg.W) ? 0u : (1u << c);
+        lane_fix = tile_ok && (nrmask | ncmask) != 0;
+        tbase = (unsigned)(hrow0 * sg.W + wcol0) * (4u * (unsigned)p.Cin) + 4u * (unsigned)lch;
+    }
+    const bool fix = __builtin_amdgcn_ballot_w64(lane_fix) != 0ull;
+    bool risky;
+    {
+        const long plast = min(p0 + (long)W36N_TM, sg.M) - 1;
+        const long nl = plast / HoWo;
+        const long tyl = (plast - nl * HoWo) / sg.Wo;
+        risky = (nl * sg.H + 4 * tyl + 4) * (long)sg.W + 4L * sg.Wo >= (long)sg.N * sg.H * sg.W;
+    }
+    const unsigned cin4 = 4u * (unsigned)p.Cin;
+    const unsigned rowpitch = (unsigned)sg.W * cin4;
+    const unsigned cin4_s = __builtin_amdgcn_readfirstlane(cin4);
+    const unsigned rowpitch_s = __builtin_amdgcn_readfirstlane((unsigned)sg.W) * cin4_s;
+    const unsigned cbase = (unsigned)wcol0 * cin4 + 4u * (unsigned)lch;
+    const size_t xaddr = reinterpret_cast<size_t>(sg.x);
+    const unsigned xlo = __builtin_amdgcn_readfirstlane((unsigned)xaddr), xhi = __builtin_amdgcn_readfirstlane((unsigned)(xaddr >> 32));
+    const unsigned xbytes = __builtin_amdgcn_readfirstlane((unsigned)(sg.N * sg.H * sg.W) * 4u * (unsigned)p.Cin);
+    const char *xbase = reinterpret_cast<const char *>(((size_t)xhi << 32) | xlo);
+    const unsigned st_base = (unsigned)((((lch >> 2) * W36N_TM + (ltile ^ W36N_SWZ(lch >> 2))) * 16) + (lch & 3) * 4);
+    constexpr unsigned XI_PITCH = 4 * W36N_TM * 16;
+    const unsigned fr_base = (unsigned)((kq * W36N_TM + (l16 ^ W36N_SWZ(kq))) * 16) + (unsigned)pg * 9u * XI_PITCH;
+    const size_t waddr = reinterpret_cast<size_t>(p.w) + (size_t)n_t * (size_t)nslabs * W36N_BSLAB;
+    const unsigned wlo = __builtin_amdgcn_readfirstlane((unsigned)waddr), whi = __builtin_amdgcn_readfirstlane((unsigned)(waddr >> 32));
+    const __amdgpu_buffer_rsrc_t wrsrc = __builtin_amdgcn_make_buffer_rsrc(reinterpret_cast<void *>(((size_t)whi << 32) | wlo), 0,
+                                                                            nslabs * (int)W36N_BSLAB, 0x00020000);
+    const unsigned b_lane = (unsigned)(pg * 9 * W36N_BXI + cg * 4 * W36N_BBLK + lane * 16);
+
+    w36_floatx4 acc[9][4];
+#pragma unroll
+    for (int i = 0; i < 9; ++i)
+#pragma unroll
+        for (int b = 0; b < 4; ++b)
+#pragma unroll
+            for (int r = 0; r < 4; ++r) acc[i][b][r] = 0.f;
+
+    float ld[36];
+    float4 breg[W36N_RING];
+#define W36N_BLOAD2(S0, SO, U) { const unsigned so_ = (SO) + (unsigned)(((U) >> 1) * W36N_BXI + ((U) & 1) * 2 * W36N_BBLK);                \
+        const w36_uintx4 v0_ = __builtin_amdgcn_raw_buffer_load_b128(wrsrc, b_lane, so_, 0);                                              \
+        const w36_uintx4 v1_ = __builtin_amdgcn_raw_buffer_load_b128(wrsrc, b_lane, so_ + W36N_BBLK, 0);                                           \
+        breg[(S0)] = make_float4(__uint_as_float(v0_.x), __uint_as_float(v0_.y), __uint_as_float(v0_.z), __uint_as_float(v0_.w));         \
+        breg[(S0) + 1] = make_float4(__uint_as_float(v1_.x), __uint_as_float(v1_.y), __uint_as_float(v1_.z), __uint_as_float(v1_.w)); }
+
+#pragma unroll
+    for (int u = 0; u < W36N_RING / 2; ++u) W36N_BLOAD2(2 * u, 0u, u)
+    if (wave < 4) {
+        const __amdgpu_buffer_rsrc_t xr = __builtin_amdgcn_make_buffer_rsrc(const_cast<char *>(xbase), 0, xbytes, 0x00020000);
+#pragma unroll
+        for (int r = 0; r < 6; ++r) { W36_LOADROW_SAFE(r, xr) }
+#pragma unroll
+        for (int r = 0; r < 6; ++r) { W36_ROWPASS(r) }
+#pragma unroll
+        for (int j = 0; j < 6; ++j) { W36_COLSTASH(j, st_base) }
+    }
+    __syncthreads();
+    float4 afr = *reinterpret_cast<const float4 *>(smem_raw + fr_base);
+
+    auto slab_loop = [&](auto mode_tag) __attribute__((always_inline)) {
+    constexpr int MODE = decltype(mode_tag)::value;
+    for (int s = 0; s < nslabs; ++s) {
+        const int sn = min(s + 1, nslabs - 1);
+        const __amdgpu_buffer_rsrc_t xr = __builtin_amdgcn_make_buffer_rsrc(const_cast<char *>(xbase) + (size_t)sn * 64, 0, xbytes - (unsigned)sn * 64u, 0x00020000);
+        const unsigned cur = (s & 1) ? W36N_VBUF : 0u, nxt = W36N_VBUF - cur;
+        const unsigned sb = nxt + st_base;
+        const unsigned wcur = (unsigned)s * W36N_BSLAB, wnxt = (unsigned)sn * W36N_BSLAB;
+#pragma unroll
+        for (int u = 0; u < 18; ++u) {
+            if constexpr (MODE == 1) { if (u < 6) { W36_LOADROW_FAST(u, xr) } }
+            if constexpr (MODE == 2) { if (u < 6) { W36_LOADROW_SAFE(u, xr) } }
+            float4 afn = afr;
+            if (u & 1) {
+                if (u < 17) afn = *reinterpret_cast<const float4 *>(smem_raw + cur + fr_base + (unsigned)((u + 1) >> 1) * XI_PITCH);
+                else afn = *reinterpret_cast<const float4 *>(smem_raw + nxt + fr_base);
+            }
+            if constexpr (MODE != 0) {
+                if (u >= 6 && u <= 11) { if constexpr (MODE == 1) { W36_FIXROW(u - 6) } W36_ROWPASS(u - 6) }
+                if (u >= 11 && u <= 16) { W36_COLSTASH(u - 11, sb) }
+            }
+            const float4 b0 = breg[(2 * u) % W36N_RING], b1 = breg[(2 * u) % W36N_RING + 1];
+            w36_floatx4 &a0 = acc[u >> 1][2 * (u & 1)], &a1 = acc[u >> 1][2 * (u & 1) + 1];
+            a0 = __builtin_amdgcn_mfma_f32_16x16x4f32(afr.x, b0.x, a0, 0, 0, 0);
+            a1 = __builtin_amdgcn_mfma_f32_16x16x4f32(afr.x, b1.x, a1, 0, 0, 0);
+            a0 = __builtin_amdgcn_mfma_f32_16x16x4f32(afr.y, b0.y, a0, 0, 0, 0);
+            a1 = __builtin_amdgcn_mfma_f32_16x16x4f32(afr.y, b1.y, a1, 0, 0, 0);
+            a0 = __builtin_amdgcn_mfma_f32_16x16x4f32(afr.z, b0.z, a0, 0, 0, 0);
+            a1 = __builtin_amdgcn_mfma_f32_16x16x4f32(afr.z, b1.z, a1, 0, 0, 0);
+            a0 = __builtin_amdgcn_mfma_f32_16x16x4f32(afr.w, b0.w, a0, 0, 0, 0);
+            a1 = __builtin_amdgcn_mfma_f32_16x16x4f32(afr.w, b1.w, a1, 0, 0, 0);
+            if (u + W36N_RING / 2 < 18) { W36N_BLOAD2((2 * u) % W36N_RING, wcur, u + W36N_RING / 2) } else { W36N_BLOAD2((2 * u) % W36N_RING, wnxt, u + W36N_RING / 2 - 18) }
+            if (u == 16) __syncthreads();
+            afr = afn;
+            __builtin_amdgcn_sched_barrier(0);
+        }
+    }
+    };
+    if (wave >= 4) slab_loop(std::integral_constant<int, 0>{});
+    else if (risky) slab_loop(std::integral_constant<int, 2>{});
+    else slab_loop(std::integral_constant<int, 1>{});
+#undef W36N_BLOAD2
+
+    const unsigned crow = (unsigned)p.Cout * 4u;
+    const unsigned obytes_ = __builtin_amdgcn_readfirstlane((unsigned)((long)sg.N * sg.OH * sg.OW) * crow);
+    const size_t oaddr_ = reinterpret_cast<size_t>(sg.out);
+    const __amdgpu_buffer_rsrc_t orsrc = __builtin_amdgcn_make_buffer_rsrc(
+        reinterpret_cast<void *>(((size_t)(unsigned)__builtin_amdgcn_readfirstlane((unsigned)(oaddr_ >> 32)) << 32) | (unsigned)__builtin_amdgcn_readfirstlane((unsigned)oaddr_)),
+        0, (int)obytes_, 0x00020000);
+    const bool has_res = sg.res != nullptr;
+    const size_t raddr_ = reinterpret_cast<size_t>(has_res ? sg.res : sg.out);
+    const __amdgpu_buffer_rsrc_t rrsrc = __builtin_amdgcn_make_buffer_rsrc(
+        reinterpret_cast<void *>(((size_t)(unsigned)__builtin_amdgcn_readfirstlane((unsigned)(raddr_ >> 32)) << 32) | (unsigned)__builtin_amdgcn_readfirstlane((unsigned)raddr_)),
+        0, (int)obytes_, 0x00020000);
+    float *xch = reinterpret_cast<float *>(smem_raw);
+#pragma unroll 1
+    for (int bb = 0; bb < 2; ++bb) {
+        __syncthreads();
+        if (cg == bb) {
+#pragma unroll
+            for (int b = 0; b < 4; ++b) {
+                float *dst = xch + (4 * kq * W36_PTS + 9 * pg) * 64 + ((16 * b + 16 * kq + l16) & 63);
+#pragma unroll
+                for (int u = 0; u < 9; ++u)
+#pragma unroll
+                    for (int i = 0; i < 4; ++i) dst[(i * W36_PTS + u) * 64] = acc[u][b][i];
+            }
+        }
+        __syncthreads();
+        const int co_ch = n_t * W36N_TN + 64 * bb + lane;
+        const bool co_ok = co_ch < p.Cout;
+        const float bv = (p.bias != nullptr && co_ok) ? p.bias[co_ch] : 0.f;
+#pragma unroll 1
+        for (int rr = 0; rr < 2; ++rr) {
+            const int tile = 2 * wave + rr;
+            const long pp = p0 + tile;
+            const float *src = xch + tile * W36_PTS * 64 + ((lane + 16 * (tile >> 2)) & 63);
+            float m[36];
+#pragma unroll
+            for (int x = 0; x < 36; ++x) m[x] = src[x * 64];
+            if (!(co_ok && pp < sg.M)) continue;
+            const int n = (int)(pp / HoWo);
+            const int rem = (int)(pp - (long)n * HoWo);
+            const int ty = rem / sg.Wo, tx = rem - ty * sg.Wo;
+            float t[6][4];
+#pragma unroll
+            for (int i = 0; i < 6; ++i) W36_AT(m[6 * i + 0], m[6 * i + 1], m[6 * i + 2], m[6 * i + 3], m[6 * i + 4], m[6 * i + 5], t[i][0], t[i][1], t[i][2], t[i][3])
+#pragma unroll
+            for (int c = 0; c < 4; ++c) {
+                float y[4];
+                W36_AT(t[0][c], t[1][c], t[2][c], t[3][c], t[4][c], t[5][c], y[0], y[1], y[2], y[3])
+                const int ox = 4 * tx + c;
+#pragma unroll
+                for (int a = 0; a < 4; ++a) {
+                    const int oy = 4 * ty + a;
+                    const unsigned off = (oy < sg.OH && ox < sg.OW) ? (unsigned)((n * sg.OH + oy) * sg.OW + ox) * crow + 4u * (unsigned)co_ch : 0x80000000u;
+                    float v = y[a] + bv;
+                    if (has_res) v = v + __uint_as_float(__builtin_amdgcn_raw_buffer_load_b32(rrsrc, off, 0, 0));
+                    if (p.relu) v = fmaxf(v, 0.f);
+                    __builtin_amdgcn_raw_buffer_store_b32(__float_as_uint(v), orsrc, off, 0, 0);
+                }
+            }
+        }
+    }
+}
+#undef W36_LOADROW_FAST
+#undef W36_LOADROW_SAFE
+#undef W36_ROWOFF
+#undef W36_FIXROW
+#undef W36_ROWPASS
+#undef W36_COLSTASH
+
 static int w36_fill(ConvParams &p, const char *who, int nseg, const float *const x[], float *const out[], const int batch[], const int height[],
-                    const int width[], int Cin, int Cout, const float *wpack, int ldw, const float *bias, int relu)
-{
-    UPS_REQUIRE(Cin > 0 && Cin % 32 == 0 && ldw % W36_TN == 0, "%s: Cin %% 32 == 0 and ldw %% 64 == 0 (got %d, %d)", who, Cin, ldw);
-    int rc = conv_fill(p, who, nseg, x, nullptr, nullptr, nullptr, out, batch, height, width, Cin, Cout, wpack, ldw, bias, 3, 3, 1, 1, 1, relu);
+                    const int width[], int Cin, int Cout, const float *wpack, int ldw, const float *bias, int relu,
+                    int tm = W36_TM, int tn = W36_TN, int cin_mult = 32, const float *const residual[] = nullptr)
+{
+    UPS_REQUIRE(Cin > 0 && Cin % cin_mult == 0 && ldw % tn == 0, "%s: Cin %% %d == 0 and ldw %% %d == 0 (got %d, %d)", who, cin_mult, tn, Cin, ldw);
+    int rc = conv_fill(p, who, nseg, x, residual, nullptr, nullptr, out, batch, height, width, Cin, Cout, wpack, ldw, bias, 3, 3, 1, 1, 1, relu, cin_mult);
     if (rc) return rc;
     UPS_REQUIRE((long)W36_PTS * Cin * ldw < (1L << 29), "%s: packed weight exceeds 2 GiB", who);
     int tiles = 0;
@@ -278,10 +501,10 @@
         UPS_REQUIRE((long)s.N * s.H * s.W * Cin < (1L << 28), "%s: feature map %d exceeds 1 GiB; split the batch", who, i);
         UPS_REQUIRE((long)s.N * s.OH * s.OW * Cout < (1L << 29), "%s: output %d exceeds 2 GiB; split the batch", who, i);
         s.tile_start = tiles;
-        tiles += (int)((s.M + W36_TM - 1) / W36_TM);
+        tiles += (int)((s.M + tm - 1) / tm);
     }
     p.m_tiles = tiles;
-    p.n_tiles = ldw / W36_TN;
+    p.n_tiles = ldw / tn;
     return 0;
 }
 
@@ -330,6 +553,24 @@
     return conv_splitk_reduce((hipStream_t)stream, p.partial, ksplit, p.m_total, p.m_total, Cout, bias, nullptr, relu, out);
 }
 
+extern "C" int upsnet_conv2d_winograd36_n128_nhwc_f32(void *stream, int nseg, const float *const x[], const float *const residual[],
+                                                      float *const out[], const int batch[], const int height[], const int width[], int Cin,
+                                                      const float *wpack, int ldw, const float *bias, int Cout, int relu)
+{
+    ConvParams p;
+    int rc = w36_fill(p, "conv2d_winograd36_n128_nhwc_f32", nseg, x, out, batch, height, width, Cin, Cout, wpack, ldw, bias, relu,
+                      W36N_TM, W36N_TN, 16, residual);
+    if (rc) return rc;
+    static std::atomic<unsigned long long> attr_dev{0};
+    UPS_ONCE_PER_DEVICE(attr_dev, UPS_CHECK_HIP(hipFuncSetAttribute(reinterpret_cast<const void *>(&conv_wino36_n128_f32_kernel), hipFuncAttributeMaxDynamicSharedMemorySize, W36N_XCH)));
+    const int grid = 8 * ((p.m_tiles + 7) / 8) * p.n_tiles;
+    hipLaunchKernelGGL(conv_wino36_n128_f32_kernel, dim3(grid), dim3(512), W36N_XCH, (hipStream_t)stream, p);
+    UPS_CHECK_LAUNCH("conv_wino36_n128_f32_kernel");
+    ups_set_form("wino36<%d,%d>", W36N_TM, W36N_TN);
+    return 0;
+}
+
+template <bool N128>
 __global__ void conv_pack_weight_wino36_kernel(const float *__restrict__ w, int cout, int cin, int ldw, float *__restrict__ wp)
 {
     const long total = (long)ldw * cin;
@@ -347,14 +588,15 @@
         for (int i = 0; i < 6; ++i)
 #pragma unroll
             for (int b = 0; b < 3; ++b) t[i][b] = G[i][0] * g[0][b] + G[i][1] * g[1][b] + G[i][2] * g[2][b];
-        const long blk = ((long)(co / W36_TN) * nslabs + (c >> 4)) * W36_PTS;
-        const int q = (c & 15) >> 2, ci = c & 3, cl = co % W36_TN;
+        const long blk = ((long)(co / (N128 ? W36N_TN : W36_TN)) * nslabs + (c >> 4)) * W36_PTS;
+        const int q = (c & 15) >> 2, ci = c & 3, cl = co % W36_TN, cb16 = (co % W36N_TN) >> 4;
 #pragma unroll
         for (int i = 0; i < 6; ++i)
 #pragma unroll
             for (int j = 0; j < 6; ++j) {
                 const double u = t[i][0] * G[j][0] + t[i][1] * G[j][1] + t[i][2] * G[j][2];
-                wp[(((blk + i * 6 + j) * 4 + q) * W36_TN + cl) * 4 + ci] = (float)u;
+                if constexpr (N128) wp[((((blk + i * 6 + j) * 8 + cb16) * 4 + q) * 16 + (co & 15)) * 4 + ci] = (float)u;
+                else wp[(((blk + i * 6 + j) * 4 + q) * W36_TN + cl) * 4 + ci] = (float)u;
             }
     }
 }
@@ -366,7 +608,19 @@
     const long total = (long)ldw * cin;
     int blocks = (int)((total + 255) / 256);
     if (blocks > 65535) blocks = 65535;
-    hipLaunchKernelGGL(conv_pack_weight_wino36_kernel, dim3(blocks), dim3(256), 0, (hipStream_t)stream, weight, cout, cin, ldw, wpack);
+    hipLaunchKernelGGL(conv_pack_weight_wino36_kernel<false>, dim3(blocks), dim3(256), 0, (hipStream_t)stream, weight, cout, cin, ldw, wpack);
     UPS_CHECK_LAUNCH("conv_pack_weight_wino36_kernel");
     return 0;
 }
+
+extern "C" int upsnet_conv_pack_weight_winograd36_n128(void *stream, const float *weight, int cout, int cin, int ldw, float *wpack)
+{
+    UPS_REQUIRE(weight && wpack && cout > 0 && cin > 0 && ldw >= cout, "conv_pack_weight_winograd36_n128: bad args");
+    UPS_REQUIRE(cin % 16 == 0 && ldw % W36N_TN == 0, "conv_pack_weight_winograd36_n128: Cin %% 16 must be 0 and ldw a multiple of 128");
+    const long total = (long)ldw * cin;
+    int blocks = (int)((total + 255) / 256);
+    if (blocks > 65535) blocks = 65535;
+    hipLaunchKernelGGL(conv_pack_weight_wino36_kernel<true>, dim3(blocks), dim3(256), 0, (hipStream_t)stream, weight, cout, cin, ldw, wpack);
+    UPS_CHECK_LAUNCH("conv_pack_weight_wino36_kernel<n128>");
+    return 0;
+}
diff --git a/upsnet_amd/knobs.py b/upsnet_amd/knobs.py
--- a/upsnet_amd/knobs.py
+++ b/upsnet_amd/knobs.py
@@ -63,6 +63,7 @@
     'UPSNET_WINO36_SPLITK': ('0', 'models/hipconv.py', 'res3 / res4 conv2 and FPN P4 on the split-K F(4x4) form (3-5 us per launch; more rounding error)'),
     'UPSNET_WINO36_PREFIX': ('0', 'models/hipconv.py', 'multi-map F(4x4) launches keep only the leading maps that fill whole rounds of workgroups (measured: no gain)'),
     'UPSNET_WINO36_ROI': ('1', 'models/hipconv.py', 'mask head (ROI batches) on the Winograd F(4x4,3x3) kernel (0: F(2x2) with the half-size tail)'),
+    'UPSNET_WINO36_N128': ('1', 'models/hipconv.py', 'Cout % 128 == 0 F(4x4,3x3) single-map launches of two or more rounds of workgroups (FPN P2) on the 16-tile x 128-channel form (0: the 32-tile x 64-channel form everywhere)'),
     'UPSNET_WINO36_MIN_FILL': ('0.65', 'models/hipconv.py', 'F(4x4,3x3) only if its last round of workgroups is at least this full'),
     'UPSNET_WINOGRAD': ('1', 'models/hipconv.py', '3x3 / stride 1 layers on the Winograd kernel'),
     'UPSNET_WINOGRAD_MIN_WG': ('128', 'models/hipconv.py', 'fewest workgroups for the Winograd kernel'),
diff --git a/upsnet_amd/models/hipconv.py b/upsnet_amd/models/hipconv.py
--- a/upsnet_amd/models/hipconv.py
+++ b/upsnet_amd/models/hipconv.py
@@ -350,6 +350,29 @@
     return _pack(m, 'wino36', ops.pack_winograd36_weight)
 
 
+WINO36_N128 = os.environ.get('UPSNET_WINO36_N128', '1') != '0'
+WINO36_N128_MIN_ROUNDS = 2
+
+
+def _winograd36_n128_plan(m):
+    return _pack(m, 'wino36n128', lambda w: ops.pack_winograd36_weight(w, n128=True))
+
+
+def _use_winograd36_n128(m, xs):
+    if not (WINO36_N128 and len(xs) == 1 and m.out_channels % 128 == 0 and m.in_channels % 16 == 0):
+        return False
+    wgs = sum(-(-(x.shape[0] * ((x.shape[2] + 3) // 4) * ((x.shape[3] + 3) // 4)) // 16) for x in xs) * (m.out_channels // 128)
+    return wgs >= WINO36_N128_MIN_ROUNDS * _cus(xs[0].device)
+
+
+def _winograd36_launch(m, xs, relu):
+    if _use_winograd36_n128(m, xs):
+        wp, ldw = _winograd36_n128_plan(m)
+        return ops.conv2d_winograd36_multi(xs, wp, ldw, m.bias, m.out_channels, relu=relu, n128=True), ' n128'
+    wp, ldw = _winograd36_plan(m)
+    return ops.conv2d_winograd36_multi(xs, wp, ldw, m.bias, m.out_channels, relu=relu), ''
+
+
 def _winograd36_shape_ok(m):
     return (tuple(m.kernel_size) == (3, 3) and tuple(m.stride) == (1, 1) and tuple(m.padding) == (1, 1) and tuple(m.dilation) == (1, 1) and
             m.in_channels % 32 == 0 and m.out_channels % 64 == 0)
@@ -472,12 +495,12 @@
             ks = _wino36_ksplit(m, x)
             return ops.conv2d_winograd36_splitk(x, wp, ldw, m.bias, m.out_channels, ks, relu=relu), 'winograd36 splitk%d' % ks
         if winograd is True and not pin and residual is None and _use_winograd36(m, [x]):
-            wp, ldw = _winograd36_plan(m)
-            return ops.conv2d_winograd36_multi([x], wp, ldw, m.bias, m.out_channels, relu=relu)[0], 'winograd36'
+            ys, sfx = _winograd36_launch(m, [x], relu)
+            return ys[0], 'winograd36' + sfx
         if (winograd == 'always' and WINO36 and WINO36_ROI and residual is None and x.dtype == torch.float32 and _winograd36_shape_ok(m) and
                 x.shape[2] * x.shape[3] <= 1024):
-            wp, ldw = _winograd36_plan(m)
-            return ops.conv2d_winograd36_multi([x], wp, ldw, m.bias, m.out_channels, relu=relu)[0], 'winograd36 roi'
+            ys, sfx = _winograd36_launch(m, [x], relu)
+            return ys[0], 'winograd36 roi' + sfx
         if winograd and not residual_up and _use_winograd(m, [x], always=(winograd == 'always')):
             wp, ldw = _winograd_plan(m)
             ks = 1 if winograd == 'always' else _wino_ksplit(m, [x])
@@ -526,7 +549,8 @@
                 for x, y in zip(xs[:k], ys):
                     _trace('conv', module=m, x=x, out=y, relu=relu, residual=None, residual_up=False, form='winograd36 multi')
                 return ys + conv_multi(m, xs[k:], relu=relu)
-            ys, form = ops.conv2d_winograd36_multi(xs, wp, ldw, m.bias, m.out_channels, relu=relu), 'winograd36 multi'
+            ys, sfx = _winograd36_launch(m, xs, relu)
+            form = 'winograd36 multi' + sfx
         elif _use_winograd(m, xs):
             wp, ldw = _winograd_plan(m)
             ys, form = ops.conv2d_winograd_multi(xs, wp, ldw, m.bias, m.out_channels, relu=relu), 'winograd tm%d multi' % _wino_tm(m, xs)
diff --git a/upsnet_amd/ops.py b/upsnet_amd/ops.py
--- a/upsnet_amd/ops.py
+++ b/upsnet_amd/ops.py
@@ -1346,19 +1346,21 @@
     return outs
 
 
-def pack_winograd36_weight(weight):
+def pack_winograd36_weight(weight, n128=False):
     require_cuda(weight)
     weight = f32c(weight)
     Cout, Cin, kh, kw = weight.shape
-    if (kh, kw) != (3, 3) or Cin % 32:
-        raise RuntimeError("pack_winograd36_weight: 3x3 kernel and Cin %% 32 == 0")
-    ldw = (Cout + 63) // 64 * 64
+    if (kh, kw) != (3, 3) or Cin % (16 if n128 else 32):
+        raise RuntimeError("pack_winograd36_weight: 3x3 kernel and Cin %% %d == 0" % (16 if n128 else 32))
+    tn = 128 if n128 else 64
+    ldw = (Cout + tn - 1) // tn * tn
     wp = torch.empty((36 * Cin, ldw), dtype=torch.float32, device=weight.device)
-    check(lib().upsnet_conv_pack_weight_winograd36(stream(), ptr(weight), Cout, Cin, ldw, ptr(wp)), "conv_pack_weight_winograd36")
+    fn = lib().upsnet_conv_pack_weight_winograd36_n128 if n128 else lib().upsnet_conv_pack_weight_winograd36
+    check(fn(stream(), ptr(weight), Cout, Cin, ldw, ptr(wp)), "conv_pack_weight_winograd36")
     return wp, ldw
 
 
-def conv2d_winograd36_multi(xs, wpack, ldw, bias, cout, relu=False, outs=None):
+def conv2d_winograd36_multi(xs, wpack, ldw, bias, cout, relu=False, outs=None, n128=False, residuals=None):
     require_cuda(wpack, *xs)
     assert 1 <= len(xs) <= 5
     xs = [nhwc(x.float()) for x in xs]
@@ -1375,15 +1377,27 @@
             outs.append(o)
         else:
             outs.append(_nhwc_out(N, cout, H, W, x.device))
-    ev0 = _prof_begin()
-    check(lib().upsnet_conv2d_winograd36_nhwc_f32(stream(), len(xs), ptr_array(xs), ptr_array(outs), int_array([x.shape[0] for x in xs]),
-                                                  int_array([x.shape[2] for x in xs]), int_array([x.shape[3] for x in xs]), int(cin), ptr(wpack),
-                                                  int(ldw), ptr(None if bias is None else f32c(bias)), int(cout), int(bool(relu))),
-          "conv2d_winograd36_nhwc_f32")
+    ress = None
+    if residuals is not None:
+        if not n128:
+            raise RuntimeError("conv2d_winograd36_multi: residuals only on the n128 form")
+        ress = [nhwc(r.float()) for r in residuals]
+        for r, o in zip(ress, outs):
+            if tuple(r.shape) != tuple(o.shape):
+                raise RuntimeError("conv2d_winograd36_multi: residual shape %s != %s" % (tuple(r.shape), tuple(o.shape)))
+    ev0 = _prof_begin()
+    geo = (int_array([x.shape[0] for x in xs]), int_array([x.shape[2] for x in xs]), int_array([x.shape[3] for x in xs]), int(cin), ptr(wpack),
+           int(ldw), ptr(None if bias is None else f32c(bias)), int(cout), int(bool(relu)))
+    if n128:
+        check(lib().upsnet_conv2d_winograd36_n128_nhwc_f32(stream(), len(xs), ptr_array(xs), ptr_array(ress) if ress is not None else None,
+                                                           ptr_array(outs), *geo), "conv2d_winograd36_n128_nhwc_f32")
+    else:
+        check(lib().upsnet_conv2d_winograd36_nhwc_f32(stream(), len(xs), ptr_array(xs), ptr_array(outs), *geo), "conv2d_winograd36_nhwc_f32")
     if ev0 is not None:
         npix = sum(o.shape[0] * o.shape[2] * o.shape[3] for o in outs)
-        _prof_end(ev0, 'conv', 2.0 * cout * cin * 9 * npix, 4.0 * (cin * npix + cout * npix + cout * cin * 9),
-                  "winograd36 3x3/1 %d->%d %s" % (cin, cout, [tuple(x.shape[0:1] + x.shape[2:]) for x in xs]))
+        _prof_end(ev0, 'conv', 2.0 * cout * cin * 9 * npix, 4.0 * (cin * npix + cout * npix * (2 if ress is not None else 1) + cout * cin * 9),
+                  "winograd36%s 3x3/1 %d->%d %s%s" % ("n128" if n128 else "", cin, cout, [tuple(x.shape[0:1] + x.shape[2:]) for x in xs],
+                                                    " +res" if ress is not None else ""))
     return outs
 
 
```

New measurement: 169.9. Within noise of the previous version (-0.1%).
